# opteroncx/MoePhoto

Measured on AMD Instinct MI355X. Metric: megapixels/sec (input), 1080p 4x SR (Net4x a4), 256-px tiles with overlap, higher is better.
Workload: dtype fp16; 1 GPU; BASELINE configs[1]: 1 frame(s) 1920x1080 RGB -> 7680x4320, model a4 (Net4x, synthetic weights in zoo format), crop 256 pad 5 align 8 -> 40 tiles/frame, fp16 I/O, fp16 MFMA operands + fp32 accumulate; tiles_per_frame=40, parallelism=single GPU, precision=mixed, exact_blocks=1, input=natural-image-like synthetic frame (tests/golden_defs.natural_image)

## Files before the change

moephoto_amd/csrc/common.h:

```cpp
#pragma once
#include <hip/hip_runtime.h>
#include <stdint.h>

typedef _Float16 half_t;
typedef __attribute__((ext_vector_type(2))) _Float16 half2_t;
typedef __attribute__((ext_vector_type(4))) _Float16 half4_t;
typedef __attribute__((ext_vector_type(8))) _Float16 half8_t;
typedef __attribute__((ext_vector_type(4))) float float4_t;
typedef __attribute__((ext_vector_type(16))) float float16_t;

constexpr int kCB = 64;
constexpr int kTileW = 32;
constexpr int kTileH = 8;
constexpr int kFragBytes = 1024;

struct ConvArgs {
    const half_t* in;
    half_t* out;
    const half_t* res;
    const half_t* wpk;
    const float* bias;
    const float* bias_img;
    const half_t* zero;
    half_t* trash;
    half_t* out_lo;
    const half_t* in_lo;
    int plane_w;
    const half_t* side16;
    const float* tail1_w;
    float* tail1_out;
    const half_t* res_lo;
    float* acc32;
    int acc_mode;
    long long w_batch_stride;
    int B, H, W;
    int in_cs, out_cs;
    int r;
    int nchunks;
    int G;
    int px, py;
    float slope;
    float scale;
    const half_t* tail_w;
    float* tplanes;
    int tail_form;
    int tail_split;
    int dbg;
    float* pool; int pool_slabs;
};

struct ConvForm {
    int B = 0, H = 0, W = 0, in_cs = 64, out_cs = 64, r = 1, nchunks = 1, G = 1, py = 1;
    float slope = 1.f, scale = 1.f;
    int acc_mode = 0, dbg = 0, tail_form = 0, tail_split = 0, pool_slabs = 0;
    bool res = false, res_lo = false, in_lo = false, out_lo = false, side16 = false, tail = false, tail1 = false, pool = false, plane_w = false;
};
inline ConvForm conv_form(const ConvArgs& a)
{
    ConvForm c;
    c.B = a.B; c.H = a.H; c.W = a.W; c.in_cs = a.in_cs; c.out_cs = a.out_cs; c.r = a.r; c.nchunks = a.nchunks; c.G = a.G; c.py = a.py;
    c.slope = a.slope; c.scale = a.scale; c.acc_mode = a.acc_mode; c.dbg = a.dbg; c.tail_form = a.tail_form; c.tail_split = a.tail_split; c.pool_slabs = a.pool_slabs;
    c.res = a.res != nullptr; c.res_lo = a.res_lo != nullptr; c.in_lo = a.in_lo != nullptr; c.out_lo = a.out_lo != nullptr; c.side16 = a.side16 != nullptr;
    c.tail = a.tplanes != nullptr; c.tail1 = a.tail1_w != nullptr; c.pool = a.pool != nullptr; c.plane_w = a.plane_w != 0;
    return c;
}

struct TailSumLayout { unsigned S, RA, CA, CO, total; int py, px; };
__host__ __device__ inline TailSumLayout tailsum_layout(int B, int H, int W)
{
    TailSumLayout l;
    l.py = (H + kTileH - 1) / kTileH; l.px = (W + kTileW - 1) / kTileW;
    auto up = [](unsigned long long n) { return (unsigned)((n + 63) / 64 * 64); };
    l.S = 0;
    l.RA = l.S + up(16ull * B * H * W);
    l.CA = l.RA + up(8ull * B * l.py * W);
    l.CO = l.CA + up(8ull * B * H * l.px);
    l.total = l.CO + up(4ull * B * l.py * l.px);
    return l;
}
inline bool tailsum_fits(int B, int H, int W)
{
    const unsigned long long el = 16ull * B * H * W + 8ull * B * ((H + kTileH - 1) / kTileH) * W + 8ull * B * H * ((W + kTileW - 1) / kTileW) + 4ull * B * ((H + kTileH - 1) / kTileH) * ((W + kTileW - 1) / kTileW) + 4 * 64;
    return el * 4 < (1ull << 32) - (1ull << 17);
}

struct Conv1x1Args {
    const half_t* in_hi; const half_t* in_lo;
    half_t* out_hi; half_t* out_lo;
    const half_t* w_hi; const half_t* w_lo;
    const float* bias;
    const float* tail_w; float* tail_out;
    float slope;
    int B, H, W, r, nchunks, out_cs;
    int nks;
};
struct Conv1x1Form { int B, H, W, r, nchunks, out_cs; float slope; bool x3, tail, out_lo; };
bool conv1x1_applicable(const Conv1x1Form& a, int max_groups);
bool launch_conv1x1(const Conv1x1Args& a, int max_groups, hipStream_t s);
hipError_t conv1x1_init();

struct Conv1x1F2Args {
    const half_t* in_hi; const half_t* in_lo;
    const half_t* wa_hi; const half_t* wa_lo;
    const half_t* wb_hi; const half_t* wb_lo;
    const float* bias_a; const float* bias_b;
    const float* tail_w; float* tail_out;
    float slope_a, slope_b;
    int B, H, W;
};
bool conv1x1_f2_applicable(int B, int H, int W, float slope_a, float slope_b, int max_groups);
bool launch_conv1x1_f2(const Conv1x1F2Args& a, int max_groups, hipStream_t s);
hipError_t conv1x1_f2_init();

void launch_conv_mfma(const ConvArgs& a, int taps, int nseg, hipStream_t s);
int conv_mfma_max_groups();
hipError_t conv_mfma_init();
bool conv3x3_sp_applicable(const ConvForm& c);
bool launch_conv3x3_sp(const ConvArgs& a, hipStream_t s);
hipError_t conv3x3_sp_init();
bool conv3x3_rw_applicable(const ConvForm& c);
bool launch_conv3x3_rw(const ConvArgs& a, hipStream_t s);
hipError_t conv3x3_rw_init();

struct Ps4Args {
    const half_t* in;
    const half_t* wpk;
    const float* bias;
    const half_t* tail_w;
    half_t* out;
    float* plane;
    float* apron;
    float slope;
    int B, H, W;
    int split;
};
bool launch_conv3x3_ps4(const Ps4Args& a, int max_groups, hipStream_t s);
bool ps4_applicable(int B, int H, int W);
inline bool ps4_tail_applicable(int B, int H, int W, float slope) { return slope < 1.f && ps4_applicable(B, H, W); }
bool ps4_store_applicable(int B, int H, int W, float slope);
size_t ps4_plane_bytes(int B, int H, int W);
size_t ps4_apron_bytes(int B, int H, int W);
hipError_t conv3x3_ps4_init();
struct TailAddArgs {
    const float* p0; const float* p1;
    const float* a0; const float* a1;
    void* y; int y_dtype; const long long* y_off;
    int B, H, W, px;
    int vec_ok;
};
void launch_tailadd(const TailAddArgs& a, hipStream_t s);

struct Ps9Args {
    const half_t* in;
    const half_t* wpk;
    const float* bias;
    const half_t* tail_w;
    float* plane;
    float* apron;
    float slope;
    int B, H, W;
    int split;
    int xcd_map;
};
bool launch_conv3x3_ps9(const Ps9Args& a, int max_groups, hipStream_t s);
bool ps9_applicable(int B, int H, int W);
inline bool ps9_tail_applicable(int B, int H, int W, float slope) { return slope < 1.f && ps9_applicable(B, H, W); }
size_t ps9_plane_bytes(int B, int H, int W);
size_t ps9_apron_bytes(int B, int H, int W);
hipError_t conv3x3_ps9_init();
struct TailAdd3Args {
    const float* p0; const float* p1;
    const float* a0; const float* a1;
    void* y; int y_dtype; const long long* y_off;
    int B, H, W, px;
    int vec_ok;
};
void launch_tailadd3(const TailAdd3Args& a, hipStream_t s);

struct ArsbArgs {
    const half_t* x_hi; const half_t* x_lo;
    half_t* y_hi; half_t* y_lo;
    const half_t* w1; const half_t* w2;
    const half_t* zero;
    float slope;
    int B, H, W;
    int px, py;
    int cin;
    int drop_lo;
    unsigned long long* trace;
};
bool arsb32c_applicable(int B, int H, int W, float slope, bool x_lo, bool y_lo, int cin);
bool launch_arsb32c(ArsbArgs a, int max_groups, hipStream_t s);
hipError_t arsb32c_init();

struct ConvX3Args {
    const half_t* in_hi; const half_t* in_lo;
    half_t* out_hi; half_t* out_lo;
    const half_t* res_hi; const half_t* res_lo;
    const half_t* w_hi; const half_t* w_lo;
    const half_t* zero;
    float slope;
    int B, H, W;
    int px, py;
    float* pool; int pool_slabs;
    const float* gate;
    const half_t* wq_hi16; const unsigned char* wq_hi8; const unsigned char* wq_lo8;
    int in8, out8;
};
struct ConvX3Form {
    int B = 0, H = 0, W = 0, pool_slabs = 0;
    float slope = 1.f;
    bool res = false, res_lo = false, pool = false, gate = false, in8 = false, out8 = false;
};
inline ConvX3Form conv_x3_form(const ConvX3Args& a)
{
    ConvX3Form c;
    c.B = a.B; c.H = a.H; c.W = a.W; c.pool_slabs = a.pool_slabs; c.slope = a.slope;
    c.res = a.res_hi != nullptr; c.res_lo = a.res_lo != nullptr; c.pool = a.pool != nullptr; c.gate = a.gate != nullptr; c.in8 = a.in8 != 0; c.out8 = a.out8 != 0;
    return c;
}
bool conv64_x3_applicable(const ConvX3Form& c, int max_groups);
bool launch_conv64_x3(ConvX3Args a, int max_groups, hipStream_t s);
hipError_t conv64_x3_init();
bool conv64_q8_applicable(const ConvX3Form& c);
bool launch_conv64_q8(ConvX3Args a, int max_groups, hipStream_t s);
hipError_t conv64_q8_init();
bool conv64_sq_applicable(const ConvX3Form& c, int max_groups);
bool launch_conv64_sq(ConvX3Args a, int max_groups, hipStream_t s);
hipError_t conv64_sq_init();
bool conv64_s_applicable(const ConvForm& c);
bool launch_conv64_s(const ConvArgs& a, int max_groups, hipStream_t s);
hipError_t conv64_s_init();
struct ArsbSqArgs {
    const half_t* x_hi; const unsigned char* x_lo8;
    half_t* y_hi; void* y_lo;
    const half_t* w16[2]; const unsigned char* wh8[2]; const unsigned char* wl8[2];
    float slope;
    int B, H, W, out8;
};
bool arsb_sq_applicable(int B, int H, int W, float slope);
bool launch_arsb_sq(const ArsbSqArgs& a, int max_groups, hipStream_t s);
hipError_t arsb_sq_init();

inline int pooled_groups(long long P, long long items, int max_groups)
{
    long long G = 1;
    if (P <= max_groups) G = P * (max_groups / P);
    else for (long long d = max_groups; d >= 1; --d) if (P % d == 0) { G = d; break; }
    return (int)(G < items ? G : items);
}
inline bool pooled_groups_ok(long long P, long long items, int max_groups)
{
    const long long full = items < max_groups ? items : max_groups;
    return 2ll * pooled_groups(P, items, max_groups) >= full;
}

struct DirectConvArgs {
    const half_t* in; half_t* out; const half_t* res;
    const float* w;
    const float* bias;
    long long w_batch_stride;
    int B, H, W, in_cs, out_cs, cin, cout, k, r;
    float slope, scale;
};
void launch_conv_direct(const DirectConvArgs& a, hipStream_t s);

struct StemArgs {
    const void* x; int x_dtype;
    const long long* x_off;
    long long sB, sH, sW;
    const float* w;
    float slope;
    half_t* out;
    half_t* out_lo;
    int B, H, W, taps;
    int out_lo8;
    const float* w2; half_t* out2; half_t* out2_lo;
};
void launch_stem(const StemArgs& a, hipStream_t s);

struct TailArgs {
    const half_t* in0; const half_t* in1;
    const half_t* w0; const half_t* w1;
    const half_t* in0_lo; const half_t* in1_lo;
    const half_t* w0_lo; const half_t* w1_lo;
    int in1_lo8;
    const void* skip; int skip_dtype;
    const long long* skip_off; long long skip_sB, skip_sH, skip_sW;
    void* y; int y_dtype;
    const long long* y_off;
    int B, H, W, taps;
};
void launch_tail(const TailArgs& a, hipStream_t s);

struct TapSumArgs {
    const float* t0; const float* t1;
    void* y; int y_dtype; const long long* y_off;
    int B, H, W;
    int r;
    int form;
    int vec_ok;
};
void launch_tapsum(const TapSumArgs& a, hipStream_t s);

struct Tail1SumArgs {
    const float* p0; const float* p1;
    int nparts;
    void* y; int y_dtype; const long long* y_off;
    int B, H, W;
    const float* lut; int r; const void* x; const long long* x_off; long long sB, sH, sW;
    int vec_ok;
};
void launch_tail1sum(const Tail1SumArgs& a, hipStream_t s);

void launch_pool_partial(const half_t* in, const half_t* in_lo, float* partial, int B, long long HW, int C, int nslab, hipStream_t s);

struct SednSeArgs {
    const float* partial; int nslab; long long HW;
    const float* w_down;
    const float* w_up;
    const float* trans_pk32;
    half_t* trans_out;
    half_t* trans_out_lo;
    int B, nfrag;
};
void launch_sedn_se(const SednSeArgs& a, hipStream_t s);

struct SednFuseArgs {
    const half_t* x;
    float* partial;
    const float* pooled; int pooled_slabs;
    int pooled_count;
    int nslab, B, H, W;
    const float* w256t;
    const float* w256;
    const float* wt;
    const float* w_down;
    const float* w_up;
    float* gate;
    half_t* weff;
};
void launch_sedn_fuse(const SednFuseArgs& a, hipStream_t s);

struct FrmArgs {
    const float* partial; int nslab; long long HW;
    const float* w0; const float* b0;
    const float* w2; const float* b2;
    const half_t* t; const half_t* x; half_t* out;
    const half_t* t_lo; const half_t* x_lo; half_t* out_lo;
    float* gate;
    int B;
};
void launch_frm(const FrmArgs& a, hipStream_t s);
struct FrmPreArgs {
    const half_t* m; const half_t* m_lo;
    const float* partial; int nslab;
    const float* c2t;
    const float* w0; const float* b0;
    const float* w2; const float* b2;
    float* gate;
    int B, H, W;
};
void launch_frm_pre(const FrmPreArgs& a, hipStream_t s);

struct StitchArgs {
    const float* tiles; const long long* tile_off;
    const int* row_first; const int* row_cnt;
    const int* col_first; const int* col_cnt;
    const int* row_tab; const int* col_tab;
    const float* ramp;
    void* out; int out_dtype;
    int C, out_h, out_w, step_w;
    int row_lo;
    int y0, rows;
};
void launch_stitch(const StitchArgs& a, hipStream_t s);
struct QuantDither { float S, top; int ordered; };
bool launch_stitch_out(const StitchArgs& a, int canvas_dtype, float quant, hipStream_t s, const QuantDither* dq = nullptr);
void launch_stitch_planes(const StitchArgs& a, int canvas_dtype, int depth, hipStream_t s, const QuantDither* dq = nullptr);
struct StitchMix {
    const void* inp; long long sC, sH, sW;
    const void* alpha; long long aH, aW;
    float sf, tf; int blend;
    float quant;
    int inp_vec, alpha_vec;
    long long once_from; int q_once;
};
bool launch_stitch_mix(const StitchArgs& a, StitchMix m, int canvas_dtype, hipStream_t s, const QuantDither* dq = nullptr);
struct YuvEdge {
    int ky[3], ku[3], kv[3];
    unsigned mul_y, base_y; int mul_c, base_c;
    int depth, f16;
};
void launch_stitch_yuv(const StitchArgs& a, const YuvEdge& y, hipStream_t s, int dither = 0);
void launch_to_output_yuv(const void* src, int src_dtype, int H, int W, const YuvEdge& y, void* dst, hipStream_t s, int dither = 0);
struct LumaCoef { float kr, kg, kb, ib, ir, eb, er, gr, gb; };
struct StitchLuma { const float* c; LumaCoef k; int rp; float quant; };
bool launch_stitch_luma(const StitchArgs& a, const StitchLuma& m, int canvas_dtype, hipStream_t s, const QuantDither* dq = nullptr);
void launch_luma_split(const void* img, int dtype, int C, long long sC, long long sH, long long sW, int H, int W, const LumaCoef& k, int rp, void* dst_y, float* dst_c, hipStream_t s);
void launch_luma_merge(const void* y, int dtype, const float* c, int C, int H, int W, const LumaCoef& k, int rp, float quant, void* dst, int dst_dtype, hipStream_t s,
                       const QuantDither* dq = nullptr);

struct BlendTileArgs {
    const void* r; void* canvas; const void* ramp;
    long long r_sC, r_sH, c_sC, c_sH;
    int C, rh, rw;
    int top_sc, left_sc;
    int r0, c0;
    int lt_h, lt_w;
};
void launch_blend_tile(const BlendTileArgs& a, bool f16, hipStream_t s);

struct SymArgs {
    const void* src; void* dst;
    long long sC, sH, sW;
    int C, Hd, Wd;
    int nR, nC, flipR, flipC;
    int src_vec;
    int div; float inv;
};
void launch_sym(SymArgs a, bool f16, bool fold, bool tr, hipStream_t s);

struct WireRec {
    long long tile_off, wire_off;
    int C, th, tw;
    int ra0, ra1, rb0, rb1;
    int ca0, ca1, cb0, cb1;
    int pad_;
};
long long wire_rec_words(const WireRec& r);
void launch_wire(bool pack, float* tiles, unsigned* wire, const WireRec* recs, int n, long long max_elems, hipStream_t s);

void launch_to_float(const void* src, int src_dtype, float inv_or_div, bool divide, int H, int W, int C, void* dst, int dst_dtype, hipStream_t s);
void launch_to_output(const void* src, int src_dtype, int H, int W, int C, float quant, void* dst, int dst_dtype, hipStream_t s, const QuantDither* dq = nullptr);
void launch_to_float_planes(const void* src, int depth, int H, int W, void* dst_y, void* dst_c, int dst_dtype, hipStream_t s);
struct ChromaTab { short coef[16][4]; signed char off[16]; };
void launch_chroma_resample(const void* src, int src_depth, int h, int w, void* dst, int dst_depth, int scale, int taps, const ChromaTab& tx, const ChromaTab& ty, hipStream_t s);
void launch_chroma_guided(const void* src_c, const void* src_y, int src_depth, int h, int w, void* dst_c, const void* dst_y, int dst_depth, int scale, int left,
                          const unsigned char* cx, const signed char* ox, const unsigned char* cy, const signed char* oy, const unsigned char* range64, hipStream_t s);
constexpr int RGB_FRAC = 20;
struct PlanesRgb { int coef[5]; int yoff, coff, cmax, top, rgb, ordered; };
void launch_planes_rgb(const void* src, int depth, int H, int W, void* dst, int bits, int taps, const ChromaTab& tx, const ChromaTab& ty, const PlanesRgb& k, hipStream_t s);
constexpr int LUT3D_MIN = 2, LUT3D_MAX = 65;
struct Lut3dArgs { const float4* table; const float* vert; int d; float strength, rest; int blend, rgb; };
void launch_lut3d(const void* src, int src_bits, int H, int W, void* dst, int bits, const Lut3dArgs& k, float quant, const QuantDither* dq, hipStream_t s);
constexpr int FIT_TW = 128, FIT_TAPS = 16;
constexpr size_t FIT_LDS_BUDGET = 80 * 1024;
struct FitAxis { const int* off; const short* coef; int taps; };
void launch_fit(const void* src, int src_depth, int h, int w, void* dst, int dst_depth, int oh, int ow, int planes, int th, size_t lds, const FitAxis& ax, const FitAxis& ay, hipStream_t s);
void launch_fit_px(const void* src, int src_depth, int h, int w, void* dst, int dst_depth, int oh, int ow, int channels, int th, size_t lds, const FitAxis& ax, const FitAxis& ay, hipStream_t s);
void launch_resize(const void* src, void* dst, int dtype, int C, int H, int W, int h, int w, int mode, hipStream_t s);
void launch_maxabsdiff(const float* a, const float* b, long long n, unsigned* out, hipStream_t s);
void launch_changed_blocks(const void* cur, void* prev, int n, int rows, long long row_bytes, int block_rows, int block_bytes, unsigned char* map, hipStream_t s);
// ... 3 lines not shown
```

moephoto_amd/csrc/conv3x3_ps4.hip:

```cpp
#include "common.h"
#include "mfma_stream.h"
#include "rowtile.h"
#include "../../include/moephoto_amd.h"
#include <algorithm>

#ifndef PS4_FILL
#define PS4_FILL 5
#endif
#ifndef PS4_ZSKIP
#define PS4_ZSKIP 1
#endif
#ifndef PS4_ABL
#define PS4_ABL 0
#endif

namespace {

constexpr int RB = 4;
constexpr int PW = kTileW + 2;
constexpr int ROWB = PW * 128;
constexpr int BLKB = RB * ROWB;
constexpr int NPIECE = BLKB / 1024;
constexpr int TREC = 36 * 128 + 64;
constexpr int TEXP = 36 * 128;
constexpr int TROWS = 16;
constexpr int OFF_T = 2 * BLKB;
constexpr int OFF_BIAS = OFF_T + TROWS * TREC;
constexpr int OFF_TW = OFF_BIAS + 1024;
constexpr int OFF_DUMP = OFF_TW + 8 * 1024;
constexpr int LDS_BYTES = OFF_DUMP + 1024;

enum OpKind : int { OP_NONE = 0, OP_P, OP_WL, OP_TM, OP_TW, OP_BI, OP_DMA, OP_FA, OP_FR, OP_FS, OP_AR, OP_AS, OP_ST };
constexpr OpList row_ops(int epi)
{
    OpList r;
    if (epi == 0) {
        for (int s = 0; s < 4; ++s) {
            r.push(OP_P, s >> 1, 4 * (s & 1), 2); r.push(OP_P, s >> 1, 4 * (s & 1) + 2, 2);
            r.push(OP_ST, s >> 1, s & 1);
        }
        return r;
    }
    const bool split = epi == 2;
    int nl = 0;
    auto wl = [&](int frag) { r.push(OP_WL, frag, nl & 1); ++nl; };
    int nt = 0;
    wl(0);
    wl(split ? 4 : 1);
    for (int s = 0; s < 4; ++s) {
        if (split) for (int k = 0; k < 4; ++k) r.push(OP_P, s >> 1, 4 * (s & 1) + k, 1);
        else for (int k = 0; k < 4; k += 2) r.push(OP_P, s >> 1, 4 * (s & 1) + k, 2);
        r.push(OP_TM, nt & 1, 0, nt == 0); ++nt;
        if (split) {
            if (s < 3) wl(s + 1);
            r.push(OP_TM, nt & 1, 1, 0); ++nt;
            if (s < 3) wl(4 + s + 1);
        } else if (s + 2 < 4) wl(s + 2);
    }
    for (int k = 0; k < 5; ++k) r.push(OP_TW, k);
    return r;
}
constexpr OpList extra_ops(int e, bool tail)
{
    OpList r;
    if (!tail) {
        if (e == 0) for (int m = 0; m < 3; ++m) { r.push(OP_DMA, m, 0); r.push(OP_DMA, m, 1); }
        if (e == 1) for (int m = 3; m < 5; ++m) { r.push(OP_DMA, m, 0); r.push(OP_DMA, m, 1); }
        return r;
    }
    if (e == 0) {
        r.push(OP_FA);
        for (int dy = 0; dy < 3; ++dy) { r.push(OP_FR, dy, 0); r.push(OP_FR, dy, 1); r.push(OP_FR, dy, 2); }
        r.push(OP_FS);
        r.push(OP_AR); r.push(OP_AS);
        r.push(OP_DMA, 0, 0); r.push(OP_DMA, 0, 1);
    }
    if (e == 1) for (int m = 1; m < 5; ++m) { r.push(OP_DMA, m, 0); r.push(OP_DMA, m, 1); }
    return r;
}

template <int EPI, bool MASK>
__global__ __launch_bounds__(256) void conv3x3_ps4_kernel(Ps4Args a)
{
#if defined(__HIP_DEVICE_COMPILE__)
    constexpr bool TAIL = EPI >= 1, SPLIT = EPI == 2;
    constexpr bool PERM = !TAIL;
    extern __shared__ __attribute__((aligned(1024))) char smem[];
    const unsigned lds0 = (unsigned)(unsigned long long)(__attribute__((address_space(3))) char*)smem;
    const int tid = threadIdx.x, lane = tid & 63;
    const int w4 = __builtin_amdgcn_readfirstlane(tid >> 6);
    const int pi = w4 >> 1, pj = w4 & 1;
    const int j = lane & 31, hh = lane >> 5;
    const int H = a.H, W = a.W;

    const int px = (W + kTileW - 1) / kTileW, nyb = H / RB;
    const int g = blockIdx.x, G = gridDim.x;
    const long long nitems = (long long)a.B * px * nyb;
    int item = (int)(nitems * g / G);
    const int item_end = (int)(nitems * (g + 1) / G);
    if (item >= item_end) return;

    half8_t wf[2][36];
    {
        const half_t* wsrc = a.wpk + (long long)w4 * (72 * 512);
        int src = lane;
        if (PERM) {
            src = weight_row(j, hh);
        }
#pragma unroll
        for (int f = 0; f < 36; ++f) {
            wf[0][f] = *(const half8_t*)(wsrc + ((f * 2 + 0) * 64 + src) * 8);
            wf[1][f] = *(const half8_t*)(wsrc + ((f * 2 + 1) * 64 + src) * 8);
        }
#pragma unroll
        for (int f = 0; f < 36; ++f) asm volatile("" : "+a"(wf[0][f]));
#pragma unroll
        for (int f = 0; f < 28; ++f) asm volatile("" : "+a"(wf[1][f]));
#pragma unroll
        for (int f = 28; f < 36; ++f) asm volatile("" : "+v"(wf[1][f]));
    }
    {
        const int bw = tid >> 6, bcg = (tid >> 5) & 1, bhh = (tid >> 4) & 1, bq = (tid >> 2) & 3, be = tid & 3;
        *(float*)(smem + OFF_BIAS + tid * 4) = a.bias[64 * bw + 32 * bcg + (PERM ? 16 * (bq >> 1) + 8 * bhh + 4 * (bq & 1) + be : 8 * bq + 4 * bhh + be)];
        if (TAIL) {
            const u4_t* tsrc = (const u4_t*)a.tail_w;
            *(u4_t*)(smem + OFF_TW + tid * 16) = tsrc[tid];
            *(u4_t*)(smem + OFF_TW + 4096 + tid * 16) = SPLIT ? tsrc[256 + tid] : u4_t{0u, 0u, 0u, 0u};
            const u4_t z = {0u, 0u, 0u, 0u};
            for (int o = tid * 16; o < TROWS * TREC; o += 256 * 16) *(u4_t*)(smem + OFF_T + o) = z;
        }
    }
    const unsigned bias_ad = lds0 + (unsigned)(OFF_BIAS + ((w4 * 2 + 0) * 2 + hh) * 64);
    const unsigned tw_ad = lds0 + (unsigned)(OFF_TW + lane * 16);

    const unsigned in_pad = (unsigned)(RB * W + 1) * 128u;
    const __amdgpu_buffer_rsrc_t rin = __builtin_amdgcn_make_buffer_rsrc((void*)((const char*)a.in - in_pad), 0, (unsigned)a.B * H * W * 128u + in_pad, 0x00020000);
    const __amdgpu_buffer_rsrc_t rpl = TAIL ? __builtin_amdgcn_make_buffer_rsrc((void*)a.plane, 0, (unsigned)a.B * H * W * 16u, 0x00020000)
                                            : __builtin_amdgcn_make_buffer_rsrc((void*)a.out, 0, (unsigned)a.B * H * W * 512u, 0x00020000);
    const __amdgpu_buffer_rsrc_t rap = __builtin_amdgcn_make_buffer_rsrc((void*)(TAIL ? (void*)a.apron : (void*)a.out), 0, TAIL ? (unsigned)a.B * px * H * 16u : 0u, 0x00020000);
    unsigned d_off = 0, d_r = 0, d_cc = 0;
    auto piece_addr = [&](int m) {
        unsigned q = (unsigned)((m < 4 ? w4 + 4 * m : 16) * 8 + (lane >> 3));
        asm volatile("" : "+v"(q));
        d_r = __umul24(q, 241u) >> 13;
        d_cc = (unsigned)(__mul24((int)d_r, -PW) + (int)q);
        const unsigned sl = (unsigned)(lane & 7) ^ ((d_cc >> 1) & 7u);
        d_off = ((__umul24(d_r, (unsigned)W) + d_cc) << 7) | (sl << 4);
    };
    auto piece_off = [&](int ya, int xa, bool live) {
        const bool ok = ((unsigned)(ya + (int)d_r) < (unsigned)H) & ((unsigned)(xa + (int)d_cc) < (unsigned)W) & live;
        return ok ? d_off : kOOR;
    };

    unsigned fa[3];
#pragma unroll
    for (int dx = 0; dx < 3; ++dx) {
        fa[dx] = frag_addr(lds0, j + dx, hh);
        asm volatile("" : "+v"(fa[dx]));
    }
    unsigned wa[5];
#pragma unroll
    for (int k = 0; k < 5; ++k) {
        const int t = k < 4 ? 4 * hh + k : 8;
        const int dy = t / 3, dx = t - 3 * dy;
        int col = j;
        if (pj == 1 && dx == 0) col = j + 1;
        if (pj == 0 && dx == 2) col = j - 1;
        unsigned o = (unsigned)((w4 * 9 + t) * 128 + col * 4);
        if (col == kTileW) o = (unsigned)(TEXP + ((0 * 2 + pi) * 3 + dy) * 4);
        if (col < 0) o = (unsigned)(TEXP + ((1 * 2 + pi) * 3 + dy) * 4);
        if (k == 4 && hh == 1) o = (unsigned)(TEXP + 48 + w4 * 4);
        wa[k] = lds0 + (unsigned)OFF_T + o;
        asm volatile("" : "+v"(wa[k]));
    }
    const int f_i = (lane >> 4) & 1, f_xp = lane & 15;
    const int a_side = (lane >> 1) & 1, a_i = lane & 1;
    unsigned slope2;
    {
        const half2_t s2 = {(half_t)a.slope, (half_t)a.slope};
        slope2 = __builtin_bit_cast(unsigned, s2);
    }

    float16_t acc[4][2];
    half8_t fr[3];
    half8_t twr[2];
    unsigned hX[4], lX[4];
    float16_t Gt = zero16;

    asm volatile("s_waitcnt lgkmcnt(0)" ::: "memory");
    __builtin_amdgcn_s_barrier();

    while (item < item_end) {
        const int s0 = item % nyb;
        const int t_ = item / nyb;
        const int pxi = t_ % px, b = t_ / px;
        const int s1 = min(nyb, s0 + (item_end - item));
        item += s1 - s0;
        const int x0 = pxi * kTileW;
        const int nblk = s1 - s0 + 3;
        const int kfirst = (PS4_ZSKIP && s0 == 0) ? 1 : 0;
        const int kz = (PS4_ZSKIP && s1 == nyb) ? nblk - 2 : nblk - 1;
        const bool okx = x0 + j < W;
        const int ylo = RB * s0, yhi = RB * s1;

        asm volatile("s_waitcnt lgkmcnt(0)" ::: "memory");
        __builtin_amdgcn_s_barrier();
        asm volatile("" ::: "memory");
        {
            const int ya = RB * (s0 - 1 + kfirst), xa = x0 - 1;
            const unsigned org = (unsigned)((b * H + ya + RB) * W + xa + 1) * 128u;
#pragma unroll
            for (int m = 0; m < 5; ++m) {
                piece_addr(m);
                const bool mine = m < 4 || w4 == 0;
                char* dst = smem + (m < 4 ? (w4 + 4 * m) * 1024 : (mine ? 16 * 1024 : OFF_DUMP));
                __builtin_amdgcn_raw_ptr_buffer_load_lds(rin, (__attribute__((address_space(3))) void*)dst, 16, piece_off(ya, xa, mine), org, 0, 0);
#if PS4_ABL & 128
                if (m < 4) __builtin_amdgcn_raw_ptr_buffer_load_lds(rin, (__attribute__((address_space(3))) void*)(dst + BLKB), 16, piece_off(ya + 4 * RB, xa, mine), org + (unsigned)(4 * RB * W) * 128u, 0, 0);
#endif
            }
#pragma unroll
            for (int s = 0; s < 4; ++s)
#pragma unroll
                for (int cg = 0; cg < 2; ++cg) acc[s][cg] = *(const __attribute__((address_space(3))) float16_t*)(bias_ad + cg * 128);
            asm volatile("s_waitcnt vmcnt(0) lgkmcnt(0)" ::: "memory");
            __builtin_amdgcn_s_barrier();
            asm volatile("" ::: "memory");
            fr[0] = *(lds_h8_t)(fa[0]);
            fr[1] = *(lds_h8_t)(fa[0] ^ 32u);
        }

        auto block = [&](int k, auto BUF_, auto KIND_) __attribute__((always_inline)) {
            constexpr int BUF = decltype(BUF_)::value;
            constexpr bool LAST = decltype(KIND_)::value == 2;
            constexpr bool ZERO = decltype(KIND_)::value == 1;
            const int Rk = RB * (s0 - 1 + k);
            const bool live = k + 1 < kz;
            const int yan = Rk + RB, xan = x0 - 1;
            const unsigned orgn = (unsigned)__builtin_amdgcn_readfirstlane((int)((unsigned)((b * H + yan + RB) * W + xan + 1) * 128u));
            const int yf = Rk - 7 + w4;
            const bool f_ok = (yf >= ylo) & (yf < yhi);
            unsigned fb[3];
            f2_t fs[2] = {{0.f, 0.f}, {0.f, 0.f}};
            f2_t fv[2];
            float av[3];

            auto step = [&](auto E_) __attribute__((always_inline)) {
                constexpr int e = decltype(E_)::value;
                const int orow = Rk + e - 2;
                const unsigned trow = (unsigned)__builtin_amdgcn_readfirstlane((int)((unsigned)((orow + 64) & 15) * (unsigned)TREC));
                const bool rowok = (unsigned)orow < (unsigned)H;
                constexpr int SL = (e + 2) & 3;

                auto op_p = [&](auto CG_, auto K0_, auto N_) __attribute__((always_inline)) {
                    constexpr int cg = decltype(CG_)::value, k0 = decltype(K0_)::value, n = decltype(N_)::value;
#pragma unroll
                    for (int k = k0; k < k0 + n; ++k) {
                        const float s0v = acc[SL][cg][2 * k], s1v = acc[SL][cg][2 * k + 1];
                        unsigned hv, lv = 0;
                        if (SPLIT) {
                            const float t0 = __builtin_fmaxf(s0v, s0v * a.slope), t1 = __builtin_fmaxf(s1v, s1v * a.slope);
                            split2(t0, t1, -2048.f, hv, lv);
                        } else {
                            const half2_t pr = {(half_t)s0v, (half_t)s1v};
                            const half2_t t = pr * __builtin_bit_cast(half2_t, slope2);
                            hv = __builtin_bit_cast(unsigned, __builtin_elementwise_max(pr, t));
                        }
                        hX[k & 3] = hv; lX[k & 3] = lv;
                    }
                };
                auto op_st = [&](auto CG_, auto G_) __attribute__((always_inline)) {
                    constexpr int cg = decltype(CG_)::value, gq = decltype(G_)::value;
                    const bool rok = (orow >= ylo) & (orow < yhi);
                    const unsigned vo = okx ? (unsigned)(2 * j) * 128u + (unsigned)hh * 16u : kOOR;
                    const unsigned so = rok ? ((unsigned)((b * 2 * H + 2 * orow + pi) * 2 * W + 2 * x0 + pj) * 128u + (unsigned)(64 * cg + 32 * gq)) : kOOR;
                    const u4_t d = {hX[0], hX[1], hX[2], hX[3]};
                    __builtin_amdgcn_raw_buffer_store_b128(d, rpl, vo, so, 0);
                };
                auto op_wl = [&](auto F_, auto S_) __attribute__((always_inline)) {
                    constexpr int fg = decltype(F_)::value, st = decltype(S_)::value;
                    twr[st] = *(lds_h8_t)(tw_ad + (unsigned)(fg * 1024));
                };
                auto op_tm = [&](auto S_, auto LO_, auto FIRST_) __attribute__((always_inline)) {
                    constexpr int st = decltype(S_)::value, lo = decltype(LO_)::value, first = decltype(FIRST_)::value;
                    const half8_t bv = lo ? __builtin_bit_cast(half8_t, u4_t{lX[0], lX[1], lX[2], lX[3]}) : __builtin_bit_cast(half8_t, u4_t{hX[0], hX[1], hX[2], hX[3]});
                    Gt = __builtin_amdgcn_mfma_f32_32x32x16_f16(twr[st], bv, first ? zero16 : Gt, 0, 0, 0);
                };
                auto op_tw = [&](auto K_) __attribute__((always_inline)) {
                    constexpr int k = decltype(K_)::value;
                    float t = __builtin_fmaf(Gt[8 + k], 0.00048828125f, Gt[k]);
                    const bool ok = MASK ? (rowok & okx) : rowok;
                    t = ok ? t : 0.f;
                    const unsigned ad = wa[k] + trow;
                    asm volatile("ds_write_b32 %0, %1" ::"v"(ad), "v"(t) : "memory");
                };
                auto op_bi = [&](auto CG_) __attribute__((always_inline)) {
                    constexpr int cg = decltype(CG_)::value;
#pragma unroll
                    for (int q = 0; q < 4; ++q) {
                        const float4_t t = *(const __attribute__((address_space(3))) float4_t*)(bias_ad + (unsigned)(cg * 128 + q * 16));
                        acc[SL][cg][4 * q] = t[0]; acc[SL][cg][4 * q + 1] = t[1]; acc[SL][cg][4 * q + 2] = t[2]; acc[SL][cg][4 * q + 3] = t[3];
                    }
                };
                auto op_dma = [&](auto M_, auto HALF_) __attribute__((always_inline)) {
                    constexpr int m = decltype(M_)::value, half = decltype(HALF_)::value;
                    if constexpr (half == 0) piece_addr(m);
                    else {
                        const bool mine = m < 4 || w4 == 0;
                        const unsigned dsto = (unsigned)__builtin_amdgcn_readfirstlane((int)(m < 4 ? (BUF ^ 1) * BLKB + (w4 + 4 * m) * 1024 : (mine ? (BUF ^ 1) * BLKB + 16 * 1024 : OFF_DUMP)));
                        __builtin_amdgcn_raw_ptr_buffer_load_lds(rin, (__attribute__((address_space(3))) void*)(smem + dsto), 16, piece_off(yan, xan, live & mine), orgn, 0, 0);
                    }
                };
                auto op_fa = [&]() __attribute__((always_inline)) {
#pragma unroll
                    for (int dy = 0; dy < 3; ++dy) {
                        const int isrc = f_i == 0 ? (dy == 1 ? 0 : 1) : (dy == 1 ? 1 : 0);
                        const int dd = f_i == 0 ? (dy == 0 ? -1 : 0) : (dy == 2 ? 1 : 0);
                        fb[dy] = lds0 + (unsigned)OFF_T + (unsigned)((yf + dd + 64) & 15) * (unsigned)TREC + (unsigned)((2 * isrc * 9 + dy * 3) * 128 + f_xp * 8);
                    }
                };
                auto op_fr = [&](auto DY_, auto DX_) __attribute__((always_inline)) {
                    constexpr int dy = decltype(DY_)::value, dx = decltype(DX_)::value;
                    constexpr int j0 = dx == 1 ? 0 : 1, j1 = dx == 1 ? 1 : 0;
                    if constexpr (dx > 0 || dy > 0) { fs[0] = fs[0] + fv[0]; fs[1] = fs[1] + fv[1]; }
                    fv[0] = *(const __attribute__((address_space(3))) f2_t*)(fb[dy] + (unsigned)((j0 * 9 + dx) * 128));
                    fv[1] = *(const __attribute__((address_space(3))) f2_t*)(fb[dy] + (unsigned)((j1 * 9 + dx) * 128));
                };
                auto op_fs = [&]() __attribute__((always_inline)) {
                    fs[0] = fs[0] + fv[0]; fs[1] = fs[1] + fv[1];
                    const float4_t o4 = {fs[0][0], fs[1][0], fs[0][1], fs[1][1]};
                    const bool ok = f_ok & (lane < 32) & (x0 + 2 * f_xp < W);
                    const unsigned vo = ok ? (unsigned)(f_i * 2 * W + 4 * f_xp) * 4u : kOOR;
                    const unsigned so = (unsigned)(((b * 2 * H + 2 * yf) * 2 * W) + 2 * x0) * 4u;
                    __builtin_amdgcn_raw_buffer_store_b128(__builtin_bit_cast(u4_t, o4), rpl, vo, f_ok ? so : 0u, 0);
                };
                auto op_ar = [&]() __attribute__((always_inline)) {
#pragma unroll
                    for (int dy = 0; dy < 3; ++dy) {
                        const int isrc = a_i == 0 ? (dy == 1 ? 0 : 1) : (dy == 1 ? 1 : 0);
                        const int dd = a_i == 0 ? (dy == 0 ? -1 : 0) : (dy == 2 ? 1 : 0);
                        const unsigned ad = lds0 + (unsigned)OFF_T + (unsigned)((yf + dd + 64) & 15) * (unsigned)TREC + (unsigned)(TEXP + ((a_side * 2 + isrc) * 3 + dy) * 4);
                        av[dy] = *(const __attribute__((address_space(3))) float*)ad;
                    }
                };
                auto op_as = [&]() __attribute__((always_inline)) {
                    const float v = (av[0] + av[1]) + av[2];
                    const bool ok = f_ok & (lane >= 32) & (lane < 36);
                    const unsigned vo = ok ? (unsigned)(((a_side * a.B) * px) * 2 * H + a_i) * 4u : kOOR;
                    const unsigned so = (unsigned)((b * px + pxi) * 2 * H + 2 * yf) * 4u;
                    __builtin_amdgcn_raw_buffer_store_b32(__builtin_bit_cast(unsigned, v), rap, vo, f_ok ? so : 0u, 0);
                };

                if constexpr (LAST) {
                    if constexpr (e == 0 && !(PS4_ABL & 2)) {
                        op_fa();
                        op_fr(std::integral_constant<int, 0>{}, std::integral_constant<int, 0>{}); op_fr(std::integral_constant<int, 0>{}, std::integral_constant<int, 1>{}); op_fr(std::integral_constant<int, 0>{}, std::integral_constant<int, 2>{});
                        op_fr(std::integral_constant<int, 1>{}, std::integral_constant<int, 0>{}); op_fr(std::integral_constant<int, 1>{}, std::integral_constant<int, 1>{}); op_fr(std::integral_constant<int, 1>{}, std::integral_constant<int, 2>{});
                        op_fr(std::integral_constant<int, 2>{}, std::integral_constant<int, 0>{}); op_fr(std::integral_constant<int, 2>{}, std::integral_constant<int, 1>{}); op_fr(std::integral_constant<int, 2>{}, std::integral_constant<int, 2>{});
                        op_fs();
                        op_ar(); op_as();
                    }
                    return;
                }
                auto chunk = [&](auto F_) __attribute__((always_inline)) {
                    constexpr int f = decltype(F_)::value;
                    constexpr int dx = f >> 2, ks = f & 3;
                    if (e == 3 && f == 10 && !(PS4_ABL & 16)) {
                        asm volatile("s_waitcnt vmcnt(0) lgkmcnt(0)" ::: "memory");
                        __builtin_amdgcn_s_barrier();
                        asm volatile("" ::: "memory");
                    }
                    constexpr OpList LM = row_ops(EPI);
                    constexpr OpList LX = extra_ops(e, TAIL);
                    auto half = [&](auto HC_) __attribute__((always_inline)) {
                        constexpr int hc = decltype(HC_)::value;
                        if constexpr (!ZERO) {
#pragma unroll
                            for (int u = 3 * hc; u < 3 * hc + 3; ++u) {
                                const int dy = u >> 1, cg = u & 1;
                                const int sl = (e + 1 - dy + 4) & 3;
                                acc[sl][cg] = __builtin_amdgcn_mfma_f32_32x32x16_f16(wf[cg][(dy * 3 + dx) * 4 + ks], fr[f % 3], acc[sl][cg], 0, 0, 0);
                            }
                        }
                        if constexpr (hc == 0 && !ZERO) {
                            constexpr int f2 = (f + 2) % 12;
                            constexpr int rowsel = f + 2 < 12 ? BUF * RB + e : (e < 3 ? BUF * RB + e + 1 : (BUF ^ 1) * RB);
                            if (!(PS4_ABL & 8)) fr[(f + 2) % 3] = *(lds_h8_t)((fa[f2 >> 2] ^ (unsigned)((f2 & 3) * 32)) + (unsigned)(rowsel * ROWB));
                        }
                        constexpr int h = 2 * f + hc;
                        constexpr int MH = TAIL ? 20 : 10;
                        constexpr int m_lo = h < MH ? h * LM.n / MH : LM.n, m_hi = h < MH ? (h + 1) * LM.n / MH : LM.n;
                        constexpr int x_lo = TAIL ? h * LX.n / 24 : (h < 12 ? 0 : (h - 12) * LX.n / 12), x_hi = TAIL ? (h + 1) * LX.n / 24 : (h < 12 ? 0 : (h - 11) * LX.n / 12);
                        auto runm = [&](auto I_) __attribute__((always_inline)) {
                            constexpr int I = decltype(I_)::value;
                            if constexpr (I >= m_lo && I < m_hi && !(PS4_ABL & 1)) {
                                constexpr Op o = LM.op[I];
                                if constexpr (o.kind == OP_P) op_p(std::integral_constant<int, o.a>{}, std::integral_constant<int, o.b>{}, std::integral_constant<int, o.c>{});
                                if constexpr (o.kind == OP_WL) op_wl(std::integral_constant<int, o.a>{}, std::integral_constant<int, o.b>{});
                                if constexpr (o.kind == OP_TM && !(PS4_ABL & 32)) op_tm(std::integral_constant<int, o.a>{}, std::integral_constant<int, o.b>{}, std::integral_constant<int, o.c>{});
                                if constexpr (o.kind == OP_TW) op_tw(std::integral_constant<int, o.a>{});
                                if constexpr (o.kind == OP_ST) op_st(std::integral_constant<int, o.a>{}, std::integral_constant<int, o.b>{});
                            }
                        };
                        auto runx = [&](auto I_) __attribute__((always_inline)) {
                            constexpr int I = decltype(I_)::value;
                            if constexpr (I >= x_lo && I < x_hi) {
                                constexpr Op o = LX.op[I];
                                if constexpr (o.kind != OP_DMA && (PS4_ABL & 2)) return;
                                if constexpr (o.kind == OP_DMA && (PS4_ABL & 64)) return;
                                if constexpr (o.kind == OP_DMA) op_dma(std::integral_constant<int, o.a>{}, std::integral_constant<int, o.b>{});
                                if constexpr (o.kind == OP_FA) op_fa();
                                if constexpr (o.kind == OP_FR) op_fr(std::integral_constant<int, o.a>{}, std::integral_constant<int, o.b>{});
                                if constexpr (o.kind == OP_FS) op_fs();
                                if constexpr (o.kind == OP_AR) op_ar();
                                if constexpr (o.kind == OP_AS) op_as();
                            }
                        };
                        static_for<LM.n>(runm);
                        static_for<LX.n>(runx);
                        if (f == 10 && hc == 1 && !(PS4_ABL & 4)) op_bi(std::integral_constant<int, 0>{});
                        if (f == 11 && hc == 1 && !(PS4_ABL & 4)) op_bi(std::integral_constant<int, 1>{});
                    };
                    half(std::integral_constant<int, 0>{});
                    half(std::integral_constant<int, 1>{});
#ifndef PS4_NOPIN
                    static_for<ZERO ? 0 : 2>([&](auto HC_) __attribute__((always_inline)) {
                        constexpr int hc = decltype(HC_)::value, h = 2 * f + hc, MH = TAIL ? 20 : 10;
                        constexpr int m_lo = h < MH ? h * LM.n / MH : LM.n, m_hi = h < MH ? (h + 1) * LM.n / MH : LM.n;
                        pin_mfmas<3, hc == 0 ? 1 : 0, PS4_FILL>();
                        pin_mfmas<(!TAIL || (PS4_ABL & 33)) ? 0 : count_kind(LM, m_lo, m_hi, OP_TM), 0, PS4_FILL>();
                    });
#endif
                    __builtin_amdgcn_sched_barrier(0);
                };
#if PS4_ABL
                if constexpr (!LAST) asm volatile("" ::"v"(acc[SL][0]), "v"(acc[SL][1]), "v"(Gt));
#endif
                static_for<12>(chunk);
            };
            step(std::integral_constant<int, 0>{});
            step(std::integral_constant<int, 1>{});
            step(std::integral_constant<int, 2>{});
            step(std::integral_constant<int, 3>{});
        };

        typedef std::integral_constant<int, 0> Run;
        typedef std::integral_constant<int, 1> Zero;
        typedef std::integral_constant<int, 2> Last;
        int k = kfirst;
        for (; k + 1 < kz; k += 2) {
            block(k, std::integral_constant<int, 0>{}, Run{});
            block(k + 1, std::integral_constant<int, 1>{}, Run{});
        }
        if (k < kz) { block(k, std::integral_constant<int, 0>{}, Run{}); ++k; }
        if (k < nblk - 1) { block(k, std::integral_constant<int, 0>{}, Zero{}); ++k; }
        if (TAIL) block(k, std::integral_constant<int, 0>{}, Last{});
    }
#endif
}

template <bool VEC>
__global__ __launch_bounds__(256) void tailadd_kernel(TailAddArgs a)
{
    const int nq = a.W >> 3;
    const long long idx = (long long)blockIdx.x * 256 + threadIdx.x;
    if (idx >= (long long)a.B * a.H * nq) return;
    const int xq = (int)(idx % nq);
    const int Y = (int)((idx / nq) % a.H), b = (int)(idx / ((long long)nq * a.H));
    const int X0 = xq * 8;
    const long long po = ((long long)b * a.H + Y) * a.W + X0;
    float v[8];
    {
        const float4 r0 = *(const float4*)(a.p0 + po), r1 = *(const float4*)(a.p0 + po + 4);
        v[0] = r0.x; v[1] = r0.y; v[2] = r0.z; v[3] = r0.w; v[4] = r1.x; v[5] = r1.y; v[6] = r1.z; v[7] = r1.w;
        if (a.p1) {
            const float4 u0 = *(const float4*)(a.p1 + po), u1 = *(const float4*)(a.p1 + po + 4);
            v[0] += u0.x; v[1] += u0.y; v[2] += u0.z; v[3] += u0.w; v[4] += u1.x; v[5] += u1.y; v[6] += u1.z; v[7] += u1.w;
        }
    }
    const int c = X0 >> 6, in = X0 & 63;
    const long long as = (long long)a.B * a.px * a.H;
    if (in == 0 && c >= 1) {
        const long long o = ((long long)b * a.px + (c - 1)) * a.H + Y;
        float t = a.a0[o];
        if (a.a1) t += a.a1[o];
        v[0] += t;
    }
    if (in == 56 && c + 1 < a.px) {
        const long long o = as + ((long long)b * a.px + (c + 1)) * a.H + Y;
        float t = a.a0[o];
        if (a.a1) t += a.a1[o];
        v[7] += t;
    }
    const long long yo = (a.y_off ? a.y_off[b] : (long long)b * a.H * a.W) + (long long)Y * a.W + X0;
    if (a.y_dtype == MOE_F16) {
        if (VEC) {
            half8_t h;
#pragma unroll
            for (int k = 0; k < 8; ++k) h[k] = (half_t)v[k];
            *(half8_t*)((half_t*)a.y + yo) = h;
        } else {
#pragma unroll
            for (int k = 0; k < 8; ++k) ((half_t*)a.y)[yo + k] = (half_t)v[k];
        }
    } else {
        float* yp = (float*)a.y + yo;
        if (VEC) {
            *(float4*)yp = make_float4(v[0], v[1], v[2], v[3]);
            *(float4*)(yp + 4) = make_float4(v[4], v[5], v[6], v[7]);
        } else {
#pragma unroll
            for (int k = 0; k < 8; ++k) yp[k] = v[k];
        }
    }
}

template <int EPI, bool MASK>
hipError_t set_limit()
{
    return hipFuncSetAttribute((const void*)conv3x3_ps4_kernel<EPI, MASK>, hipFuncAttributeMaxDynamicSharedMemorySize, LDS_BYTES);
}

}

hipError_t conv3x3_ps4_init()
{
    hipError_t e;
    if ((e = set_limit<0, true>()) != hipSuccess) return e;
    if ((e = set_limit<1, false>()) != hipSuccess) return e;
    if ((e = set_limit<1, true>()) != hipSuccess) return e;
    if ((e = set_limit<2, false>()) != hipSuccess) return e;
    return set_limit<2, true>();
}

size_t ps4_plane_bytes(int B, int H, int W) { return (size_t)B * H * W * 16; }
size_t ps4_apron_bytes(int B, int H, int W) { return (size_t)2 * B * ((W + kTileW - 1) / kTileW) * 2 * H * 4; }

bool ps4_applicable(int B, int H, int W)
{
    if (H % RB != 0 || W % 4 != 0 || H < RB) return false;
    if ((long long)B * H * W * 128 + (long long)(RB * W + 1) * 128 >= (1ll << 32) - 65536) return false;
    return (long long)B * ((W + kTileW - 1) / kTileW) * (H / RB) < (1ll << 31) / 4;
}

bool ps4_store_applicable(int B, int H, int W, float slope)
{
    return ps4_tail_applicable(B, H, W, slope) && (long long)B * H * W * 512 < (1ll << 32) - 65536;
}

bool launch_conv3x3_ps4(const Ps4Args& a, int max_groups, hipStream_t s)
{
    if (!(a.out ? ps4_store_applicable(a.B, a.H, a.W, a.slope) : ps4_tail_applicable(a.B, a.H, a.W, a.slope))) return false;
    const int px = (a.W + kTileW - 1) / kTileW;
    const long long items = (long long)a.B * px * (a.H / RB);
    const int G = (int)std::min<long long>(items, max_groups);
    const bool ragged = a.W % kTileW != 0;
    if (a.out) {
        if (a.plane) return false;
        conv3x3_ps4_kernel<0, true><<<dim3(G), dim3(256), LDS_BYTES, s>>>(a);
        return true;
    }
    if (a.split) {
        if (ragged) conv3x3_ps4_kernel<2, true><<<dim3(G), dim3(256), LDS_BYTES, s>>>(a);
        else conv3x3_ps4_kernel<2, false><<<dim3(G), dim3(256), LDS_BYTES, s>>>(a);
    } else {
        if (ragged) conv3x3_ps4_kernel<1, true><<<dim3(G), dim3(256), LDS_BYTES, s>>>(a);
        else conv3x3_ps4_kernel<1, false><<<dim3(G), dim3(256), LDS_BYTES, s>>>(a);
    }
    return true;
}

void launch_tailadd(const TailAddArgs& a, hipStream_t s)
{
    const long long n = (long long)a.B * a.H * (a.W / 8);
    if (a.vec_ok) tailadd_kernel<true><<<dim3((unsigned)((n + 255) / 256)), dim3(256), 0, s>>>(a);
    else tailadd_kernel<false><<<dim3((unsigned)((n + 255) / 256)), dim3(256), 0, s>>>(a);
}
```

moephoto_amd/csrc/forward.cpp:

```cpp
#include "net.h"

using namespace moe;

namespace moe {

const char* kernel_name(ConvKernel k)
{
    static const char* const names[] = {"no kernel", "conv_direct", "conv1x1", "conv_mfma", "conv3x3_sp", "conv3x3_rw", "conv3x3_ps4 (store form)", "conv3x3_sp (hi + lo residual)",
                                        "conv_mfma (three products)", "conv64_x3", "conv64_q8", "conv64_sq", "conv3x3_sp (three launches)", "conv_mfma (fp32 side buffer)"};
    return names[(int)k];
}

static bool fast_layer(const moe_net& n, const ConvLayer& L) { return L.taps == 9 && L.nseg == 1 && !L.per_plane && n.opt.conv_impl == 2; }

ConvForm Fwd::form(const ConvLayer& L, int H, int W) const
{
    ConvForm c;
    c.B = B; c.H = H; c.W = W; c.in_cs = 64 * L.nseg; c.out_cs = L.r > 1 ? 64 : 64 * L.nchunks; c.r = L.r; c.nchunks = L.nchunks;
    c.py = (H + kTileH - 1) / kTileH;
    const long long items = (long long)B * ((W + kTileW - 1) / kTileW) * c.py;
    const int per_xcd = groups / 8;
    int G = per_xcd >= L.nchunks ? 8 * (per_xcd / L.nchunks) : groups / L.nchunks;
    if (G < 1) G = 1;
    if (G > items) G = (int)items;
// ... 82 lines not shown
        DirectConvArgs d{};
        d.in = in.hi; d.out = out.hi; d.res = res ? res->hi : nullptr;
        d.w = blob<float>(L.w_plain);
        d.bias = L.has_bias ? blob<float>(L.bias_plain) : nullptr;
        d.w_batch_stride = 0;
        d.B = B; d.H = H; d.W = W; d.in_cs = c.in_cs; d.out_cs = c.out_cs; d.cin = L.cin; d.cout = L.cout; d.k = L.k; d.r = L.r;
        d.slope = L.slope; d.scale = L.scale;
        if (L.per_plane) { d.w = (const float*)e.plane_w; d.w_batch_stride = (long long)L.cout * L.cin; }
        launch_conv_direct(d, s);
        return MOE_OK;
    }
    ConvArgs a{};
    a.in = in.hi; a.out = out.hi; a.res = res ? res->hi : nullptr;
    a.wpk = L.per_plane ? e.plane_w : blob<half_t>(L.w_hi);
    a.bias = L.has_bias ? blob<float>(L.bias) : small<float>("zero_bias");
    a.zero = small<half_t>("zero");
    a.bias_img = blob<float>(L.bias_img);
    a.trash = small<half_t>("trash");
    a.w_batch_stride = L.per_plane ? (long long)L.nchunks * L.nfrag() * 512 : 0;
    a.B = B; a.H = H; a.W = W; a.in_cs = c.in_cs; a.out_cs = c.out_cs; a.r = c.r; a.nchunks = c.nchunks;
    a.px = (W + kTileW - 1) / kTileW; a.py = c.py; a.G = c.G;
    a.slope = c.slope; a.scale = c.scale; a.dbg = c.dbg;
    a.tail_w = e.tail_w; a.tplanes = e.tplanes; a.tail_form = c.tail_form; a.tail_split = c.tail_split;
    a.tail1_w = e.tail1_w; a.tail1_out = e.tail1_out;
    if (c.pool) { a.pool = e.pool_out; a.pool_slabs = c.pool_slabs; }
    const bool x3 = this->x3 || e.exact;
    const bool timed = r.kernel != ConvKernel::mfma_x3 && r.kernel != ConvKernel::sp_three && r.kernel != ConvKernel::acc32;
    const int rec = timed ? prof_begin(key, (x3 ? 3 : 1) * 2.0 * (double)B * H * W * L.cout * L.cin * L.taps) : -1;
    bool ok = true;
    auto single = [&](const ConvArgs& ca) {
        if (r.kernel == ConvKernel::rw) return launch_conv3x3_rw(ca, s);
        if (r.kernel == ConvKernel::sp) return launch_conv3x3_sp(ca, s);
        if (r.kernel == ConvKernel::ps4_store) {
            Ps4Args q{};
            q.in = ca.in; q.wpk = ca.wpk; q.bias = ca.bias; q.out = ca.out; q.slope = ca.slope; q.B = ca.B; q.H = ca.H; q.W = ca.W;
            return launch_conv3x3_ps4(q, groups, s);
        }
        launch_conv_mfma(ca, L.taps, L.nseg, s);
        return true;
    };
    switch (r.kernel) {
    case ConvKernel::conv1x1: {
        Conv1x1Args q{};
        q.in_hi = in.hi; q.in_lo = x3 ? in.lo : nullptr; q.out_hi = out.hi; q.out_lo = x3 ? out.lo : nullptr;
        q.w_hi = blob<half_t>(L.w_hi); q.w_lo = x3 ? blob<half_t>(L.w_lo) : nullptr; q.bias = a.bias;
        q.tail_w = e.tail1_w; q.tail_out = e.tail1_out; q.slope = L.slope;
        q.B = B; q.H = H; q.W = W; q.r = L.r; q.nchunks = L.nchunks; q.out_cs = c.out_cs;
        q.nks = (L.cin <= 48 && n.opt.k48) ? 3 : 4;
        ok = launch_conv1x1(q, groups, s);
        break;
    }
    case ConvKernel::mfma: case ConvKernel::sp: case ConvKernel::rw: case ConvKernel::ps4_store: {
        unsigned long long* tr = nullptr;
        const size_t nb = 8 * 32 * 4 * 16 * 8;
        if (!x3 && (c.dbg & 64) && fast_layer(n, L) && key == n.opt.trace_key && hipMalloc((void**)&tr, nb) == hipSuccess) {
            (void)hipMemsetAsync(tr, 0, nb, s);
            ConvArgs t = a; t.acc32 = (float*)tr;
            ok = single(t);
            std::vector<unsigned long long> host(nb / 8);
            (void)hipStreamSynchronize(s);
            (void)hipMemcpy(host.data(), tr, nb, hipMemcpyDeviceToHost);
            if (FILE* f = fopen("/tmp/moe_trace.bin", "wb")) { fwrite(host.data(), 1, nb, f); fclose(f); }
            (void)hipFree(tr);
        } else
            ok = single(a);
        break;
    }
    case ConvKernel::sp_res_lo: {
        ConvArgs q = a; q.acc_mode = 3; q.side16 = res->lo; q.out_lo = out.lo; q.res_lo = nullptr;
        ok = launch_conv3x3_sp(q, s);
        break;
    }
    case ConvKernel::mfma_x3: {
        ConvArgs f4 = a; f4.wpk = blob<half_t>(L.w_x3); f4.acc_mode = 4; f4.in_lo = in.lo; f4.out_lo = out.lo; f4.res_lo = res ? res->lo : nullptr;
        launch_conv_mfma(f4, 1, 3, s);
        break;
    }
    case ConvKernel::x3: case ConvKernel::q8: case ConvKernel::sq: {
        ConvX3Args q{};
        q.in_hi = in.hi; q.in_lo = in.lo; q.out_hi = out.hi; q.out_lo = out.lo;
        q.res_hi = res ? res->hi : nullptr; q.res_lo = res ? res->lo : nullptr;
        q.w_hi = blob<half_t>(L.w_arsb); q.w_lo = blob<half_t>(L.w_arsb_lo); q.zero = small<half_t>("zero");
        q.slope = L.slope; q.B = B; q.H = H; q.W = W;
        if (r.x3.pool) { q.pool = e.pool_out; q.pool_slabs = e.pool_slabs; }
        if (r.x3.gate) q.gate = e.gate_in;
        if (r.kernel == ConvKernel::x3) { ok = launch_conv64_x3(q, groups, s); break; }
        q.wq_hi16 = blob<half_t>(L.w_hi); q.wq_hi8 = blob<unsigned char>(L.wq_hi8); q.wq_lo8 = blob<unsigned char>(L.wq_lo8);
        q.in8 = r.x3.in8; q.out8 = r.x3.out8;
        ok = r.kernel == ConvKernel::sq ? launch_conv64_sq(q, groups, s) : launch_conv64_q8(q, groups, s);
        break;
    }
    case ConvKernel::sp_three: {
        ConvArgs q1 = a; q1.wpk = blob<half_t>(L.w_lo); q1.out = side16; q1.res = (res && res->has_lo) ? res->lo : nullptr; q1.bias = small<float>("zero_bias");
        q1.bias_img = small<float>("zero_bias_img"); q1.slope = 1.f; q1.scale = 1.f; q1.acc_mode = 0; q1.tail_w = nullptr; q1.tplanes = nullptr;
        ConvArgs q2 = q1; q2.in = in.lo; q2.wpk = blob<half_t>(L.w_hi); q2.res = side16;
        ConvArgs q3 = a; q3.acc_mode = 3; q3.side16 = side16; q3.out_lo = out.lo; q3.res_lo = nullptr;
        ok = launch_conv3x3_sp(q1, s) && launch_conv3x3_sp(q2, s) && launch_conv3x3_sp(q3, s);
        break;
    }
    case ConvKernel::acc32: {
        a.acc32 = acc32;
        ConvArgs p1 = a; p1.wpk = L.per_plane ? e.plane_w_lo : blob<half_t>(L.w_lo); p1.acc_mode = 1; p1.res = nullptr; p1.bias = nullptr;
        launch_conv_mfma(p1, L.taps, L.nseg, s);
        ConvArgs p2 = a; p2.in = in.lo; p2.acc_mode = 2; p2.res = nullptr; p2.bias = nullptr;
        launch_conv_mfma(p2, L.taps, L.nseg, s);
        ConvArgs p3 = a; p3.acc_mode = 3; p3.out_lo = out.lo; p3.res_lo = res ? res->lo : nullptr;
        launch_conv_mfma(p3, L.taps, L.nseg, s);
        break;
    }
    default: ok = false;
    }
    prof_end(rec);
    if (!ok) return fail(MOE_EINVAL, "internal error: layer %s (%d planes of %dx%d) was routed to %s, and that launcher refused it", key.c_str(), B, H, W, kernel_name(r.kernel));
    return MOE_OK;
}

ConvDone Fwd::conv(const std::string& key, const Act& in, const Act& out, const Act* res, int H, int W, const ConvExtra& e)
{
    const ConvRoute r = route(key, in, out, res, H, W, e);
    if (r.done.ok && !dry()) {
        rc = launch(r, key, in, out, res, e);
        if (rc) ar.base = nullptr;
    }
    return r.done;
}

void Fwd::stem(const Act& out, const Act* out2)
{
    if (dry()) return;
    StemArgs a{};
    if (out2) { a.w2 = small<float>("stem.p2"); a.out2 = out2->hi; a.out2_lo = out2->lo; }
    a.x = io.x; a.x_dtype = io.x_dtype; a.x_off = io.x_off; a.sB = io.sB; a.sH = io.sH; a.sW = io.sW;
    a.w = small<float>("stem"); a.slope = n.scalars.at("stem_slope");
    a.out = out.hi; a.out_lo = out.lo; a.out_lo8 = out.lo8; a.B = B; a.H = h; a.W = w; a.taps = (int)n.scalars.at("stem_taps");
    launch_stem(a, s);
}

void Fwd::gate() { if (ctx.gate_event && !dry()) (void)hipStreamWaitEvent(s, ctx.gate_event, 0); }

void Fwd::tail(const Act* r, const Act* u, int H, int W, bool skip)
{
    gate();
    if (dry()) return;
    TailArgs a{};
    a.in0 = r->hi; a.w0 = small<half_t>("tail_r");
    if (u) { a.in1 = u->hi; a.w1 = small<half_t>("tail_u"); }
    if (r->has_lo && (!u || u->has_lo)) {
        a.in0_lo = r->lo; a.w0_lo = small<half_t>("tail_r.lo");
        if (u) { a.in1_lo = u->lo; a.w1_lo = small<half_t>("tail_u.lo"); a.in1_lo8 = u->lo8; }
    }
    if (skip) { a.skip = io.x; a.skip_dtype = io.x_dtype; a.skip_off = io.x_off; a.skip_sB = io.sB; a.skip_sH = io.sH; a.skip_sW = io.sW; }
    a.y = io.y; a.y_dtype = io.y_dtype; a.y_off = io.y_off; a.B = B; a.H = H; a.W = W; a.taps = (int)n.scalars.at("tail_taps");
    launch_tail(a, s);
}

static size_t acc32_need(const moe_net& n, int B, int h, int w)
{
    size_t best = 0;
    long long HW = (long long)h * w;
    if (n.arch == MOE_ARCH_SEDN) return (size_t)B * (size_t)HW * 256;
    int rr = 1;
    best = (size_t)B * (size_t)HW * 64;
    for (int s = 0; s < n.stages; ++s) {
        best = std::max<size_t>(best, (size_t)B * (size_t)HW * rr * rr * 64 * n.r * n.r);
        rr *= n.r;
    }
    return best;
}

int exact_blocks_of(const moe_net& n)
{
    if (n.exact_blocks >= 0) return n.exact_blocks > 6 ? 6 : n.exact_blocks;
    const int env = n.opt.exact_blocks_env;
    if (env >= 0) return env > 6 ? 6 : env;
    if (n.calib_valid && n.calib_blocks >= 0) return n.calib_blocks;
    return default_exact_blocks(n.arch);
}

int default_exact_blocks(int arch)
{
    switch (arch) {
        case MOE_ARCH_NET2X: return 4;
        case MOE_ARCH_NET3X: return 2;
        case MOE_ARCH_NET4X: return 1;
        case MOE_ARCH_NETDN: return 1;
        default: return 0;
    }
}

long long sp_bytes_per_pixel(const moe_net& n)
{
    long long per = 128;
    if (n.arch == MOE_ARCH_SEDN) per = 512;
    if (n.arch == MOE_ARCH_LITE) {
        for (int st = 0; st + 1 < n.stages; ++st) per *= 4;
    }
    if (n.arch == MOE_ARCH_NET2X || n.arch == MOE_ARCH_NET3X || n.arch == MOE_ARCH_NET4X) {
        long long rr = 1;
        for (int st = 0; st < n.stages; ++st) {
            rr *= (long long)n.r * n.r;
            per = std::max(per, st == n.stages - 1 ? 36 * rr : 128 * rr);
        }
    }
    return per;
}

static int run_forward(const moe_net& n, Fwd& f, const FwdIO& io)
{
    const int B = f.B, h = f.h, w = f.w;
    const long long P = (long long)B * h * w;
    f.io = io;
    if (f.x3) {
        f.acc32_elems = acc32_need(n, B, h, w);
        f.acc32 = (float*)f.ar.take(f.acc32_elems * 4);
        f.side16 = (half_t*)f.ar.take(f.acc32_elems * 2 + 4096);
    } else if (f.mixed) {
        f.side16 = (half_t*)f.ar.take((size_t)P * 64 * 2 + 4096);
        bool steep = false;
        for (int i = 1; i <= exact_blocks_of(n); ++i) steep = steep || n.convs[n.conv_index.at("c1_" + std::to_string(i))].slope > 1.f;
        if (steep) { f.acc32_elems = (size_t)P * 64; f.acc32 = (float*)f.ar.take(f.acc32_elems * 4); }
    }
    int rc = MOE_OK;
    switch (n.arch) {
        case MOE_ARCH_SEDN: rc = forward_sedn(n, f); break;
        case MOE_ARCH_LITE: rc = forward_lite(n, f); break;
        default: rc = forward_arsb(n, f);
    }
    return rc ? rc : f.rc;
}

static Fwd make_fwd(const moe_net& n, const FwdCtx& ctx, NetRuntime* rt, hipStream_t s, int B, int h, int w, Arena ar)
{
    Fwd f{n, ctx, rt, s, B, h, w, ar, ctx.groups, n.precision == MOE_PREC_FP16X3, n.precision == MOE_PREC_DEBUG_DIRECT};
    f.mixed = n.precision == MOE_PREC_MIXED;
    return f;
}

static size_t workspace_need(const moe_net& n, const FwdCtx& ctx, int B, int h, int w)
{
    Fwd f = make_fwd(n, ctx, nullptr, nullptr, B, h, w, Arena{});
    run_forward(n, f, FwdIO{});
    return f.ar.off + 4096;
}

static bool plan_matches(const Fwd& f, size_t planned)
{
    if (f.ar.overflow) return false;
    return f.skips_planned_work ? f.ar.off <= planned : f.ar.off == planned;
}

static int forward_dev_chunk(moe_net& n, const FwdIO& io, int B, int h, int w, hipStream_t s, bool y_off_mult8, const FwdCtx& ctx);

static void build_lite_lut_on_device(moe_net& n, hipStream_t s, const FwdCtx& ctx)
{
    const int r = n.scale;
    std::vector<unsigned short> pat(65536);
    for (int i = 0; i < 65536; ++i) pat[(size_t)i] = (unsigned short)i;
    half_t* in = nullptr;
    float* scratch = nullptr;
    int rc = MOE_ENOMEM;
    if (hipMalloc((void**)&in, 65536 * 2) == hipSuccess && hipMalloc((void**)&n.lut, (size_t)65536 * r * r * 4) == hipSuccess && hipMalloc((void**)&scratch, (size_t)65536 * r * r * 4) == hipSuccess &&
        hipMemcpyAsync(in, pat.data(), 65536 * 2, hipMemcpyHostToDevice, s) == hipSuccess && hipStreamSynchronize(s) == hipSuccess) {
        FwdCtx capture = ctx;
        capture.lut_capture = n.lut;
        rc = forward_dev_chunk(n, FwdIO{in, MOE_F16, 65536, 256, 1, nullptr, scratch, MOE_F32, nullptr}, 1, 256, 256, s, true, capture);
        (void)hipStreamSynchronize(s);
    }
    if (in) (void)hipFree(in);
    if (scratch) (void)hipFree(scratch);
    if (rc != MOE_OK) { (void)hipGetLastError(); drop_lut(n); }
    n.lut_state = rc == MOE_OK ? 1 : -1;
}

static void build_lite_lut(moe_net& n, hipStream_t s, const FwdCtx& ctx)
{
    n.lut_state = -1;
    if (n.arch != MOE_ARCH_LITE || !n.opt.lite_lut || n.debug || !n.opt.fuse_tail || n.precision == MOE_PREC_DEBUG_DIRECT) return;
    hipStreamCaptureStatus cs = hipStreamCaptureStatusNone;
    if (hipStreamIsCapturing(s, &cs) != hipSuccess || cs != hipStreamCaptureStatusNone) { (void)hipGetLastError(); n.lut_state = 0; return; }
    int cur = -1;
    if (hipGetDevice(&cur) != hipSuccess || (cur != n.device && hipSetDevice(n.device) != hipSuccess)) { (void)hipGetLastError(); n.lut_state = 0; return; }
    build_lite_lut_on_device(n, s, ctx);
    if (cur != n.device) (void)hipSetDevice(cur);
}

int forward_dev(moe_net& n, const FwdIO& io, int B, int h, int w, hipStream_t s, bool y_off_mult8, const FwdCtx& ctx)
{
    if (!n.finalized) return fail(MOE_ESTATE, "moe_net_forward: net is not finalized (load_state_dict + to(device) first)");
    if (B < 1 || h < 1 || w < 1) return fail(MOE_EINVAL, "moe_net_forward: bad shape B=%d h=%d w=%d", B, h, w);
    if ((io.x_dtype != MOE_F32 && io.x_dtype != MOE_F16) || (io.y_dtype != MOE_F32 && io.y_dtype != MOE_F16))
        return fail(MOE_EINVAL, "moe_net_forward: x/y dtype must be MOE_F32 or MOE_F16");
    const long long bmax = kSpRange / (sp_bytes_per_pixel(n) * (long long)h * w);
    if (bmax < 1)
        return fail(MOE_ENOMEM, "a %dx%d tile exceeds the convolution kernels' addressing range (%lld pixels per plane at most for this net): use a smaller cropsize",
                    h, w, kSpRange / sp_bytes_per_pixel(n));
    if (n.arch == MOE_ARCH_LITE && io.x_dtype == MOE_F16 && n.lut_state == 0 && n.opt.lite_lut) build_lite_lut(n, s, ctx);
    if (B <= bmax) return forward_dev_chunk(n, io, B, h, w, s, y_off_mult8, ctx);
    const size_t xe = io.x_dtype == MOE_F32 ? 4 : 2, ye = io.y_dtype == MOE_F32 ? 4 : 2;
    const long long yplane = (long long)h * n.scale * w * n.scale;
    for (int b0 = 0; b0 < B; b0 += (int)bmax) {
        const int cnt = (int)std::min<long long>(bmax, B - b0);
        FwdIO c = io;
        if (io.x_off) c.x_off += b0; else c.x = (const char*)io.x + (size_t)b0 * io.sB * xe;
        if (io.y_off) c.y_off += b0; else c.y = (char*)io.y + (size_t)b0 * yplane * ye;
        const bool al = y_off_mult8 && (io.y_off || ((size_t)b0 * yplane * ye) % 16 == 0);
        if (int rc = forward_dev_chunk(n, c, cnt, h, w, s, al, ctx)) return rc;
    }
    return MOE_OK;
}

static int forward_dev_chunk(moe_net& n, const FwdIO& io, int B, int h, int w, hipStream_t s, bool y_off_mult8, const FwdCtx& ctx)
{
    int cur = -1;
    HIP_TRY(hipGetDevice(&cur));
    if (cur != n.device) HIP_TRY(hipSetDevice(n.device));
    const size_t need = workspace_need(n, ctx, B, h, w);
    StreamSet& set = *ctx.set;
    if (int rc = set.ws.grow(need, s, "workspace of %zu bytes for %d planes of %dx%d does not fit", need, B, h, w)) return rc;
    const size_t planned = need - 4096;
    Fwd f = make_fwd(n, ctx, &n.rt, s, B, h, w, Arena{(char*)set.ws.p, 0, planned});
    f.y_vec = y_off_mult8 && ((uintptr_t)io.y % 16 == 0);
    int rc = run_forward(n, f, io);
    if (rc) return rc;
    if (!plan_matches(f, planned))
        return fail(MOE_EINVAL, "internal error: the launching pass took %zu bytes of workspace%s, the planning pass %zu (%d planes of %dx%d)", f.ar.off,
                    f.ar.overflow ? " (beyond the plan: the launches behind that point were not issued)" : "", planned, B, h, w);
    hipError_t e = hipGetLastError();
    if (e != hipSuccess) return fail(MOE_EHIP, "kernel launch failed: %s", hipGetErrorString(e));
    return MOE_OK;
}

void free_set(StreamSet& set)
{
    if (set.side) { (void)hipStreamSynchronize(set.side); (void)hipStreamDestroy(set.side); }
    for (hipEvent_t e : {set.ev_fork, set.ev_join}) if (e) (void)hipEventDestroy(e);
    set.ws.release();
    set = StreamSet{};
}

void free_records(NetRuntime& rt)
{
    for (auto& ev : rt.prof_ev) { (void)hipEventDestroy(ev.e0); (void)hipEventDestroy(ev.e1); }
    for (auto& sl : rt.off_ring) {
        if (sl.host) (void)hipHostFree(sl.host);
        if (sl.dev) (void)hipFree(sl.dev);
        if (sl.done) (void)hipEventDestroy(sl.done);
    }
    for (auto& t : rt.taps) if (t.second.dev) (void)hipFree(t.second.dev);
    rt = NetRuntime{};
}

void pipe_destroy(moe_net& n)
{
    for (auto& ps : n.pipe) {
        if (ps.main) { (void)hipStreamSynchronize(ps.main); (void)hipStreamDestroy(ps.main); }
        for (hipEvent_t e : {ps.entry, ps.done}) if (e) (void)hipEventDestroy(e);
        free_set(ps);
        ps = PipeSet{};
    }
    n.pipe_prev_valid = false;
    n.pipe_last_stream = nullptr;
}

static bool overlap_eligible(const moe_net& n, int B, int h, int w)
{
    const bool sr = n.arch == MOE_ARCH_NET2X || n.arch == MOE_ARCH_NET3X || n.arch == MOE_ARCH_NET4X;
    return sr && n.finalized && n.opt.overlap_calls && !n.debug && n.opt.conv_impl == 2 && (n.precision == MOE_PREC_MIXED || n.precision == MOE_PREC_FP16) &&
           (long long)B * h * w <= 4ll * 65536 && n.prof_keys.empty() && n.opt.repeat_key.empty();
}

static int forward_pipelined(moe_net* n, const void* x, int x_dtype, int B, int h, int w, int64_t sB, int64_t sH, int64_t sW, void* y, int y_dtype, hipStream_t s, unsigned flags)
{
    HIP_TRY(hipSetDevice(n->device));
    PipeSet& ps = n->pipe[n->pipe_next];
    PipeSet& prev = n->pipe[n->pipe_next ^ 1];
    if (!ps.main) {
        HIP_TRY(hipStreamCreateWithFlags(&ps.main, hipStreamNonBlocking));
        HIP_TRY(hipEventCreateWithFlags(&ps.entry, hipEventDisableTiming));
        HIP_TRY(hipEventCreateWithFlags(&ps.done, hipEventDisableTiming));
    }
    HIP_TRY(hipEventRecord(ps.entry, s));
    const bool since_prev = (flags & MOE_FWD_INPUT_SINCE_PREV) && n->pipe_prev_valid && n->pipe_last_stream == s && prev.entry;
    HIP_TRY(hipStreamWaitEvent(ps.main, since_prev ? prev.entry : ps.entry, 0));
    n->pipe_next ^= 1;
    const int groups = n->opt.overlap_groups > 0 ? std::max(16, std::min(n->opt.overlap_groups, n->max_groups)) : std::max(16, n->max_groups / 2);
    const FwdCtx ctx{&ps, groups, n->opt.overlap_fork && n->opt.branch_streams, since_prev ? ps.entry : nullptr, nullptr};
    const int rc = forward_dev(*n, FwdIO{x, x_dtype, sB, sH, sW, nullptr, y, y_dtype, nullptr}, B, h, w, ps.main, true, ctx);
    if (hipEventRecord(ps.done, ps.main) != hipSuccess || hipStreamWaitEvent(s, ps.done, 0) != hipSuccess) { (void)hipGetLastError(); (void)hipStreamSynchronize(ps.main); }
    n->pipe_prev_valid = rc == MOE_OK;
    n->pipe_last_stream = s;
    return rc;
}

}

extern "C" {

int moe_net_forward_ex(moe_net* n, const void* x, int x_dtype, int B, int h, int w, int64_t sB, int64_t sH, int64_t sW,
                       const int64_t* x_off, void* y, int y_dtype, const int64_t* y_off, void* stream, unsigned flags)
{
    if (!n || !x || !y) return fail(MOE_EINVAL, "moe_net_forward: NULL argument");
    if (flags & ~(unsigned)MOE_FWD_INPUT_SINCE_PREV) return fail(MOE_EINVAL, "moe_net_forward_ex: unknown flags 0x%x", flags);
    if ((flags & MOE_FWD_INPUT_SINCE_PREV) && !x_off && !y_off && B >= 1 && h >= 1 && w >= 1 && overlap_eligible(*n, B, h, w)) {
        hipStreamCaptureStatus cs = hipStreamCaptureStatusNone;
        if (hipStreamIsCapturing((hipStream_t)stream, &cs) == hipSuccess && cs == hipStreamCaptureStatusNone)
            return forward_pipelined(n, x, x_dtype, B, h, w, sB, sH, sW, y, y_dtype, (hipStream_t)stream, flags);
        (void)hipGetLastError();
    }
    n->pipe_prev_valid = false;
    return moe_net_forward(n, x, x_dtype, B, h, w, sB, sH, sW, x_off, y, y_dtype, y_off, stream);
}

int moe_net_forward(moe_net* n, const void* x, int x_dtype, int B, int h, int w, int64_t sB, int64_t sH, int64_t sW,
                    const int64_t* x_off, void* y, int y_dtype, const int64_t* y_off, void* stream)
{
    if (!n || !x || !y) return fail(MOE_EINVAL, "moe_net_forward: NULL argument");
    hipStream_t s = (hipStream_t)stream;
    long long* xo = nullptr;
    long long* yo = nullptr;
    NetRuntime::OffSlot* slot = nullptr;
    if (x_off || y_off) {
        HIP_TRY(hipSetDevice(n->device >= 0 ? n->device : 0));
        NetRuntime::OffSlot& sl = n->rt.off_ring[n->rt.off_next];
        n->rt.off_next = (n->rt.off_next + 1) % 4;
        if (sl.used) HIP_TRY(hipEventSynchronize(sl.done));
        const size_t need = (size_t)B * 2;
        if (need > sl.cap) {
            if (sl.host) { (void)hipHostFree(sl.host); sl.host = nullptr; }
            if (sl.dev) { (void)hipFree(sl.dev); sl.dev = nullptr; }
            sl.cap = 0;
            const size_t cap = std::max<size_t>(need, 256);
            HIP_TRY(hipHostMalloc((void**)&sl.host, cap * 8, hipHostMallocDefault));
            HIP_TRY(hipMalloc((void**)&sl.dev, cap * 8));
            sl.cap = cap;
        }
        if (!sl.done) HIP_TRY(hipEventCreateWithFlags(&sl.done, hipEventDisableTiming));
        for (int i = 0; i < B; ++i) { sl.host[i] = x_off ? x_off[i] : 0; sl.host[B + i] = y_off ? y_off[i] : 0; }
        HIP_TRY(hipMemcpyAsync(sl.dev, sl.host, need * 8, hipMemcpyHostToDevice, s));
        sl.used = true;
        slot = &sl;
        if (x_off) xo = sl.dev;
        if (y_off) yo = sl.dev + B;
    }
    bool mult8 = true;
    if (y_off) for (int i = 0; i < B; ++i) mult8 = mult8 && (y_off[i] % 8 == 0);
    const int rc = forward_dev(*n, FwdIO{x, x_dtype, sB, sH, sW, xo, y, y_dtype, yo}, B, h, w, s, mult8, own_ctx(*n, &n->set));
    if (slot && hipEventRecord(slot->done, s) != hipSuccess) { (void)hipGetLastError(); (void)hipStreamSynchronize(s); }
    return rc;
}

int64_t moe_net_workspace_bytes(const moe_net* n, int B, int h, int w)
{
    if (!n || B < 1 || h < 1 || w < 1) return fail(MOE_EINVAL, "moe_net_workspace_bytes: bad argument");
    if (!n->finalized) return fail(MOE_ESTATE, "moe_net_workspace_bytes: net is not finalized");
    return (int64_t)workspace_need(*n, own_ctx(*n, nullptr), B, h, w);
}

int moe_net_set_profile(moe_net* n, const char* layer_substrings)
{
    if (!n) return fail(MOE_EINVAL, "moe_net_set_profile: NULL net");
    n->prof_keys.clear();
    std::string all = layer_substrings ? layer_substrings : "";
    size_t pos = 0;
    while (pos <= all.size() && !all.empty()) {
        const size_t c = all.find(',', pos);
        const std::string k = all.substr(pos, c == std::string::npos ? std::string::npos : c - pos);
        if (!k.empty()) n->prof_keys.push_back(k);
        if (c == std::string::npos) break;
        pos = c + 1;
    }
    n->rt.prof_used = 0;
    return MOE_OK;
}

int moe_net_get_profile_at(moe_net* n, int index, double* total_ms, int64_t* launches, double* flops)
{
    if (!n || !total_ms || !launches || !flops) return fail(MOE_EINVAL, "moe_net_get_profile: NULL argument");
    double ms = 0, fl = 0;
    int64_t cnt = 0;
    for (size_t i = 0; i < n->rt.prof_used; ++i) {
        const NetRuntime::ProfRec& r = n->rt.prof_ev[i];
        if (r.key != index) continue;
        HIP_TRY(hipEventSynchronize(r.e1));
        float t = 0.f;
        HIP_TRY(hipEventElapsedTime(&t, r.e0, r.e1));
        ms += t; fl += r.flops; ++cnt;
    }
    *total_ms = ms; *launches = cnt; *flops = fl;
    return MOE_OK;
}

int moe_net_get_profile(moe_net* n, double* total_ms, int64_t* launches, double* flops)
{
    int rc = moe_net_get_profile_at(n, 0, total_ms, launches, flops);
    if (rc == MOE_OK) n->rt.prof_used = 0;
    return rc;
}

int64_t moe_net_max_tile_pixels(const moe_net* n)
{
    if (!n) return fail(MOE_EINVAL, "moe_net_max_tile_pixels: NULL net");
    return (int64_t)(kSpRange / sp_bytes_per_pixel(*n));
}

int moe_net_set_debug(moe_net* n, int enable)
{
    if (!n) return fail(MOE_EINVAL, "moe_net_set_debug: NULL net");
    if (enable == 2 && n->arch == MOE_ARCH_LITE)
        return fail(MOE_EINVAL, "moe_net_set_debug: value 2 (taps of the production forward) is defined for SEDN, Net2x / Net3x / Net4x and NetDN; 1 taps lite's unfused forward");
    n->debug = enable != 0 && enable != 2;
    n->tap_only = enable == 2;
    return MOE_OK;
}

int64_t moe_net_debug_tap(moe_net* n, const char* tap, float* host, int64_t capacity, int64_t shape[4], void* stream)
{
    if (!n || !tap) return fail(MOE_EINVAL, "moe_net_debug_tap: NULL argument");
    auto it = n->rt.taps.find(tap);
    if (it == n->rt.taps.end() || !it->second.dev) return fail(MOE_EINVAL, "no tap named \"%s\" (enable moe_net_set_debug before the forward)", tap);
    const auto& t = it->second;
    const int64_t nel = t.shape[0] * t.shape[1] * t.shape[2] * t.shape[3];
    if (shape) for (int d = 0; d < 4; ++d) shape[d] = t.shape[d];
    if (!host) return nel;
    if (capacity < nel) return fail(MOE_EINVAL, "moe_net_debug_tap: capacity %lld < %lld", (long long)capacity, (long long)nel);
    HIP_TRY(hipStreamSynchronize((hipStream_t)stream));
    HIP_TRY(hipMemcpy(host, t.dev, (size_t)nel * 4, hipMemcpyDeviceToHost));
    return nel;
}

}
```

moephoto_amd/csrc/forward_arsb.cpp:

```cpp
#include "net.h"

using namespace moe;

namespace {

const ConvLayer* last_up(const moe_net& n, int br)
{
    const auto it = n.conv_index.find(std::string(br == 0 ? "convt_R1" : "u") + ".up" + std::to_string(n.stages - 1));
    return it == n.conv_index.end() ? nullptr : &n.convs[it->second];
}

bool can_fuse_tail(const moe_net& n, const Fwd& f)
{
    const int B = f.B, h = f.h, w = f.w;
    if (!n.opt.fuse_tail || f.x3 || f.direct || n.debug || n.opt.conv_impl != 2 || n.stages < 1) return false;
    if (!(n.arch == MOE_ARCH_NET2X || n.arch == MOE_ARCH_NET3X || n.arch == MOE_ARCH_NET4X)) return false;
    if (sp_bytes_per_pixel(n) * B * h * w > kSpRange) return false;
    int hl = h, wl = w;
    for (int st = 0; st + 1 < n.stages; ++st) { hl *= n.r; wl *= n.r; }
    for (int br = 0; br < 2; ++br) {
        const ConvLayer* L = last_up(n, br);
        if (!L) return false;
        ConvForm c = f.form(*L, hl, wl);
        c.tail = true;
        if (!conv3x3_sp_applicable(c)) return false;
    }
    return true;
}

struct ArsbRun {
    const moe_net& n;
    Fwd& f;
    const int B, h, w;
    bool mixed = false;
    int nx = 0;
    Act A, Bb, Cc;
    bool chain8 = false;
    half_t* lo16x = nullptr;
    bool sr = false, fuse = false, ps4 = false, ps9 = false;
    int H = 0, W = 0;
    Act fin[2];
    float* tp[2] = {nullptr, nullptr};
    float* ps_plane[2] = {nullptr, nullptr};
    float* ps_apron[2] = {nullptr, nullptr};

    void plan_tail_form();
    template <typename Args, typename Launch>
    int ps_stage(int br, const std::string& key, const Act& cur, size_t plane_bytes, size_t apron_bytes, const char* name, Launch launch);
    int run_branch(int br, Act cur);
    int trunk_conv(const std::string& key, const Act& in, const Act& out, const Act* res, bool exact);
    int run_trunk();
    template <typename Args, typename Launch> void tail_add(Launch launch);
    int branch_sum();
    int run();
};

void ArsbRun::plan_tail_form()
{
    sr = n.arch != MOE_ARCH_NETDN;
    fuse = sr && can_fuse_tail(n, f);
    if (sr) {
        int hl = h, wl = w;
        for (int st = 0; st + 1 < n.stages; ++st) { hl *= n.r; wl *= n.r; }
        bool ok = fuse && n.opt.tail_form == 1;
        bool ps4_ok = true;
        bool ps9_ok = true;
        for (int br = 0; br < 2; ++br) {
            const ConvLayer* L = last_up(n, br);
            if (ok) {
                ConvForm c = f.form(*L, hl, wl);
                c.tail = true; c.tail_form = 1;
                ok = conv3x3_rw_applicable(c);
            }
            ps4_ok = ps4_ok && L && ps4_tail_applicable(B, hl, wl, L->slope);
            ps9_ok = ps9_ok && L && ps9_tail_applicable(B, hl, wl, L->slope);
        }
        f.tail_form = ok ? 1 : 0;
        ps4 = ok && n.opt.up_impl == 1 && ps4_ok && (2 * wl) % 8 == 0;
        ps9 = fuse && n.opt.up_impl == 1 && n.r == 3 && f.groups >= 3 && ps9_ok;
    }
}

template <typename Args, typename Launch>
int ArsbRun::ps_stage(int br, const std::string& key, const Act& cur, size_t plane_bytes, size_t apron_bytes, const char* name, Launch launch)
{
    ps_plane[br] = (float*)f.ar.take(plane_bytes + 4096);
    ps_apron[br] = (float*)f.ar.take(apron_bytes + 4096);
    if (!f.dry()) {
        const ConvLayer& L = n.convs[n.conv_index.at(key)];
        Args q{};
        q.in = cur.hi; q.wpk = f.blob<half_t>(L.w_hi); q.bias = L.has_bias ? f.blob<float>(L.bias) : f.small<float>("zero_bias");
        q.tail_w = f.small<half_t>(br == 0 ? "tail_r.frag" : "tail_u.frag");
        q.plane = ps_plane[br]; q.apron = ps_apron[br]; q.slope = L.slope; q.B = B; q.H = H; q.W = W;
        q.split = (f.mixed && f.tail_split_for(key)) ? 1 : 0;
        const int rec = f.prof_begin(key, 2.0 * (double)B * H * W * L.cout * L.cin * L.taps);
        bool done = false;
        for (int rep = f.repeats(key); rep > 0; --rep) done = launch(q, f.groups, f.s);
        f.prof_end(rec);
        if (!done) return fail(MOE_EINVAL, "fused tail kernel (%s) rejected layer %s", name, key.c_str());
    }
    H *= n.r; W *= n.r;
    return (int)MOE_OK;
}

int ArsbRun::run_branch(int br, Act cur)
{
    if (f.mixed) { cur.drop_lo(); cur.lo8 = false; }
    H = h; W = w;
    for (int st = 0; st < n.stages; ++st) {
        const std::string key = std::string(br == 0 ? "convt_R1" : "u") + ".up" + std::to_string(st);
        if (ps4 && st == n.stages - 1) {
            if (int rc = ps_stage<Ps4Args>(br, key, cur, ps4_plane_bytes(B, H, W), ps4_apron_bytes(B, H, W), "ps4", launch_conv3x3_ps4)) return rc;
            continue;
        }
        if (ps9 && st == n.stages - 1) {
            if (int rc = ps_stage<Ps9Args>(br, key, cur, ps9_plane_bytes(B, H, W), ps9_apron_bytes(B, H, W), "ps9", launch_conv3x3_ps9)) return rc;
            continue;
        }
        if (fuse && st == n.stages - 1) {
            tp[br] = (float*)f.ar.take(f.tail_form == 1 ? (size_t)tailsum_layout(B, H, W).total * 4 + 4096 : (size_t)9 * B * H * n.r * W * n.r * 4 + 4096);
            ConvExtra tail;
            tail.fuse_tail = true; tail.tail_w = f.small<half_t>(br == 0 ? "tail_r.frag" : "tail_u.frag"); tail.tplanes = tp[br];
            if (!f.conv(key, cur, Act{}, nullptr, H, W, tail))
                return fail(MOE_EINVAL, "fused tail kernel rejected layer %s", key.c_str());
            H *= n.r; W *= n.r;
            continue;
        }
        Act nxt = f.act((long long)B * H * n.r * W * n.r);
        f.conv(key, cur, nxt, nullptr, H, W);
        H *= n.r; W *= n.r;
        f.tap(std::string(br == 0 ? "r" : "u") + ".up" + std::to_string(st), nxt, H, W, 64, 64);
        cur = nxt;
    }
    fin[br] = cur;
    return (int)MOE_OK;
}

int ArsbRun::trunk_conv(const std::string& key, const Act& in, const Act& out, const Act* res, bool exact)
{
    ConvExtra e;
    e.exact = exact;
    if (!f.conv(key, in, out, res, h, w, e))
        return fail(MOE_EINVAL, "layer %s: %d planes of %dx%d exceed the conv kernel's addressing range (use smaller tiles)", key.c_str(), B, h, w);
    return (int)MOE_OK;
}

int ArsbRun::run_trunk()
{
    if (int rc = trunk_conv("input2", A, Bb, nullptr, mixed)) return rc;
    f.tap("input2", Bb, h, w, 64, n.C);
    const bool arsb_fuse = n.opt.arsb_fuse && !f.x3 && !f.direct && n.opt.conv_impl == 2;
    hipStream_t s = f.s;
    Act cur = Bb, oth = Cc;
    for (int i = 1; i <= 6; ++i) {
        const bool ex = mixed && i <= nx;
        const std::string k1 = "c1_" + std::to_string(i), k2 = "c2_" + std::to_string(i);
        const ConvLayer& L1 = n.convs[n.conv_index.at(k1)];
        const ConvLayer& L2 = n.convs[n.conv_index.at(k2)];
        const bool trunk64 = L1.w_arsb != 0;
        const int cin = (L1.cin == 48 && L2.cin == 48 && n.opt.k48) ? 48 : 64;
        const bool drop6 = mixed && i == 6 && n.arch != MOE_ARCH_NETDN && !n.debug;
        if (arsb_fuse && !ex && (!mixed || (cur.has_lo && oth.has_lo)) && trunk64 && arsb32c_applicable(B, h, w, L1.slope, mixed, mixed, cin)) {
            if (!f.dry()) {
                ArsbArgs q{};
                q.x_hi = cur.hi; q.x_lo = mixed ? cur.lo : nullptr; q.y_hi = oth.hi; q.y_lo = mixed ? oth.lo : nullptr;
                q.w1 = f.blob<half_t>(L1.w_hi); q.w2 = f.blob<half_t>(L2.w_hi); q.zero = f.small<half_t>("zero");
                q.slope = L1.slope; q.B = B; q.H = h; q.W = w; q.cin = cin;
                q.drop_lo = drop6 ? 1 : 0;
                const bool trace = n.opt.arsb_trace;
                const size_t tb = 8 * 16 * 4 * 40 * 8;
                if (trace && i == 3 && hipMalloc((void**)&q.trace, tb) == hipSuccess) (void)hipMemsetAsync(q.trace, 0, tb, s);
                const int rec = f.prof_begin("arsb" + std::to_string(i), 2.0 * 2.0 * (double)B * h * w * L1.cout * L1.cin * 9);
                bool done = false;
                for (int rep = f.repeats("arsb" + std::to_string(i)); rep > 0; --rep) done = launch_arsb32c(q, f.groups, s);
                f.prof_end(rec);
                if (q.trace) {
                    std::vector<unsigned long long> host(tb / 8);
                    (void)hipStreamSynchronize(s);
                    (void)hipMemcpy(host.data(), q.trace, tb, hipMemcpyDeviceToHost);
                    if (FILE* fp = fopen("/tmp/arsb_trace.bin", "wb")) { fwrite(host.data(), 1, tb, fp); fclose(fp); }
                    (void)hipFree(q.trace);
                }
                if (!done) return fail(MOE_EINVAL, "internal error: arsb32c rejected layer %s its predicate took", k1.c_str());
            }
            std::swap(cur, oth); cur.lo8 = oth.lo8 = false;
            Act seen = cur;
            if (drop6) seen.drop_lo();
            f.tap("arsb" + std::to_string(i), seen, h, w, 64, n.C);
            continue;
        }
        if (ex && chain8 && n.opt.exact_fuse && n.opt.q8_impl == 1 && cur.lo8 && cur.has_lo && oth.has_lo && L1.wq_hi8 && L2.wq_hi8 && !L1.has_bias && !L2.has_bias && L2.slope == 1.f &&
            arsb_sq_applicable(B, h, w, L1.slope)) {
            if (!f.dry()) {
                ArsbSqArgs q{};
                q.x_hi = cur.hi; q.x_lo8 = (const unsigned char*)cur.lo; q.y_hi = oth.hi; q.y_lo = oth.lo;
                q.w16[0] = f.blob<half_t>(L1.w_hi); q.wh8[0] = f.blob<unsigned char>(L1.wq_hi8); q.wl8[0] = f.blob<unsigned char>(L1.wq_lo8);
                q.w16[1] = f.blob<half_t>(L2.w_hi); q.wh8[1] = f.blob<unsigned char>(L2.wq_hi8); q.wl8[1] = f.blob<unsigned char>(L2.wq_lo8);
                q.slope = L1.slope; q.B = B; q.H = h; q.W = w; q.out8 = i < nx;
                const int rec = f.prof_begin("xpair" + std::to_string(i), 2.0 * 2.0 * 3.0 * (double)B * h * w * L1.cout * L1.cin * 9);
                const bool done = launch_arsb_sq(q, f.groups, s);
                f.prof_end(rec);
                if (!done) return fail(MOE_EINVAL, "internal error: arsb_sq rejected layer %s its predicate took", k1.c_str());
            }
            std::swap(cur, oth);
            cur.lo8 = i < nx;
            oth.lo8 = false;
            f.tap("arsb" + std::to_string(i), cur, h, w, 64, n.C);
            continue;
        }
        Act m = oth;
        if (mixed && !ex) m.drop_lo();
        m.lo8 = ex && chain8;
        Act bin = cur;
        if (mixed && !ex) bin.drop_lo();
        if (int rc = trunk_conv(k1, bin, m, nullptr, ex)) return rc;
        const Act resid = cur;
        if (ex && chain8 && i == nx) { cur.lo = lo16x ? lo16x : A.lo; cur.lo8 = false; }
        if (int rc = trunk_conv(k2, m, cur, &resid, ex)) return rc;
        f.tap("arsb" + std::to_string(i), cur, h, w, 64, n.C);
    }
    Bb = cur;
    return (int)MOE_OK;
}

template <typename Args, typename Launch>
void ArsbRun::tail_add(Launch launch)
{
    if (f.dry()) return;
    Args t{};
    t.p0 = ps_plane[0]; t.p1 = ps_plane[1]; t.a0 = ps_apron[0]; t.a1 = ps_apron[1];
    t.y = f.io.y; t.y_dtype = f.io.y_dtype; t.y_off = f.io.y_off; t.B = B; t.H = H; t.W = W; t.px = (W / n.r + kTileW - 1) / kTileW;
    t.vec_ok = f.y_vec;
    const int rec = f.prof_begin("tailadd", 0.0);
    f.gate();
    launch(t, f.s);
    f.prof_end(rec);
}

int ArsbRun::branch_sum()
{
    if (ps4) { tail_add<TailAddArgs>(launch_tailadd); return MOE_OK; }
    if (ps9) { tail_add<TailAdd3Args>(launch_tailadd3); return MOE_OK; }
    if (fuse) {
        if (!f.dry()) {
            TapSumArgs t{};
            t.t0 = tp[0]; t.t1 = tp[1]; t.y = f.io.y; t.y_dtype = f.io.y_dtype; t.y_off = f.io.y_off; t.B = B; t.H = H; t.W = W; t.r = n.r;
            t.form = f.tail_form;
            t.vec_ok = n.r == 2 && f.y_vec && W % 8 == 0;
            f.gate();
            launch_tapsum(t, f.s);
        }
        return MOE_OK;
    }
    f.tail(&fin[0], &fin[1], H, W, false);
    return MOE_OK;
}

int ArsbRun::run()
{
    const long long P = (long long)B * h * w;
    hipStream_t s = f.s;
    mixed = f.mixed;
    nx = mixed ? exact_blocks_of(n) : 0;
    f.drop_taps();
    A = f.act(P, 64, mixed); Bb = f.act(P, 64, mixed); Cc = f.act(P, 64, mixed);
    if (mixed && n.opt.conv_impl != 2)
        return fail(MOE_EINVAL, "precision 'mixed' runs on the fast 3x3 kernels only: conv_impl=v1 (MOE_CONV_IMPL=v1) is a debugging switch for 'fp16' / 'fp16x3'");
    const bool dn = n.arch == MOE_ARCH_NETDN;
    chain8 = mixed && f.use_q8() && n.opt.lo8 && !n.debug && !f.direct && nx >= 1 && A.has_lo && Bb.has_lo && Cc.has_lo;
    if (dn && (int)n.scalars.at("tail_taps") != 9) chain8 = false;
    for (int i = 0; chain8 && i <= nx; ++i)
        for (int j = (i == 0 ? 2 : 1); chain8 && j <= 2; ++j)
            chain8 = f.q8_capable(n.convs[n.conv_index.at(i == 0 ? std::string("input2") : "c" + std::to_string(j) + "_" + std::to_string(i))]);
    lo16x = (dn && chain8) ? (half_t*)f.ar.take((size_t)P * 64 * 2 + 2048) : nullptr;
    A.lo8 = Bb.lo8 = chain8;
    f.stem(A);
    f.tap("stem", A, h, w, 64, n.C);
    plan_tail_form();
    const bool forked = sr && f.ctx.fork && !n.debug && !f.direct && !f.x3 && n.opt.conv_impl == 2 && (long long)B * h * w <= 4ll * 65536;
    struct ForkGuard {
        StreamSet* set; hipStream_t s; bool armed = false;
        ~ForkGuard()
        {
            if (!armed) return;
            if (hipEventRecord(set->ev_join, set->side) != hipSuccess || hipStreamWaitEvent(s, set->ev_join, 0) != hipSuccess) (void)hipStreamSynchronize(set->side);
        }
    } fork_guard{f.ctx.set, s};
    const int all = f.groups;
    int g_side = 0;
    if (forked && all >= 32) {
        g_side = n.opt.branch_groups > 0 ? n.opt.branch_groups : (n.stages >= 2 ? 5 * all / 16 : 3 * all / 16);
        g_side = std::max(8, std::min(g_side, all - 8) / 8 * 8);
    }
    if (forked) {
        if (g_side) f.groups = g_side;
        if (!f.dry()) {
            StreamSet& set = *f.ctx.set;
            if (!set.side) {
                HIP_TRY(hipStreamCreateWithFlags(&set.side, hipStreamNonBlocking));
                HIP_TRY(hipEventCreateWithFlags(&set.ev_fork, hipEventDisableTiming));
                HIP_TRY(hipEventCreateWithFlags(&set.ev_join, hipEventDisableTiming));
            }
            HIP_TRY(hipEventRecord(set.ev_fork, s));
            HIP_TRY(hipStreamWaitEvent(set.side, set.ev_fork, 0));
            f.s = set.side;
            fork_guard.armed = true;
        }
        const int rc = run_branch(1, A);
        if (g_side) f.groups = all - g_side;
        if (!f.dry()) {
            f.s = s;
            if (!rc) HIP_TRY(hipEventRecord(f.ctx.set->ev_join, f.ctx.set->side));
        }
        if (rc) return rc;
    }
    if (int rc = run_trunk()) return rc;
    if (n.arch == MOE_ARCH_NETDN) { f.tail(&Bb, &A, h, w, false); return MOE_OK; }
    if (mixed) { A.drop_lo(); Bb.drop_lo(); A.lo8 = Bb.lo8 = false; }
    if (!forked) { if (int rc = run_branch(0, Bb)) return rc; if (int rc = run_branch(1, A)) return rc; }
    else {
        if (int rc = run_branch(0, Bb)) return rc;
        if (!f.dry()) { HIP_TRY(hipStreamWaitEvent(s, f.ctx.set->ev_join, 0)); fork_guard.armed = false; }
        f.groups = all;
    }
    return branch_sum();
}

}

int moe::forward_arsb(const moe_net& n, Fwd& f)
{
    ArsbRun r{n, f, f.B, f.h, f.w};
    return r.run();
}
```

moephoto_amd/csrc/net.h:

```cpp
#pragma once
#include "engine.h"

#include <algorithm>
#include <cmath>
#include <cstdarg>
#include <cstdio>
#include <cstdlib>
#include <cstring>
#include <map>
#include <memory>
#include <utility>

namespace moe {

int fail(int code, const char* fmt, ...);
int launched(const char* who);

inline bool plane_depth(int depth) { return depth == 8 || depth == 10 || depth == 12 || depth == 16; }

#define HIP_TRY(expr)                                                                                    \
    do {                                                                                                 \
        hipError_t e_ = (expr);                                                                          \
        if (e_ != hipSuccess) return fail(e_ == hipErrorOutOfMemory ? MOE_ENOMEM : MOE_EHIP, "%s: %s", #expr, hipGetErrorString(e_)); \
    } while (0)

struct DevBuf {
    void* p = nullptr;
    size_t bytes = 0;
    template <typename... A> int grow(size_t need, hipStream_t s, const char* does_not_fit, A... a)
    {
        if (need <= bytes) return MOE_OK;
        if (p) { HIP_TRY(hipStreamSynchronize(s)); HIP_TRY(hipFree(p)); p = nullptr; bytes = 0; }
        if (hipMalloc(&p, need) != hipSuccess) { (void)hipGetLastError(); p = nullptr; return fail(MOE_ENOMEM, does_not_fit, a...); }
        bytes = need;
        return MOE_OK;
    }
    void release() { if (p) (void)hipFree(p); p = nullptr; bytes = 0; }
};

struct Param {
    std::string name;
    std::vector<int64_t> shape;
    std::vector<float> data;
    bool set = false;
    int64_t numel() const { int64_t n = 1; for (auto d : shape) n *= d; return n; }
};

struct ConvLayer {
    int taps = 9, nseg = 1, nchunks = 1, r = 1;
    int cin = 64, cout = 64, k = 3;
    float slope = 1.f, scale = 1.f;
    bool per_plane = false;
    size_t w_hi = 0, w_lo = 0, bias = 0, bias_img = 0, w_plain = 0, bias_plain = 0, w_pk32 = 0;
    size_t w_arsb_lo = 0;
    size_t wq_hi8 = 0, wq_lo8 = 0;
    size_t w_arsb = 0;
    size_t w_x3 = 0;
    bool has_x3 = false;
    bool has_bias = false;
    int nfrag() const { return nseg * taps * 8; }
};

struct Act {
    half_t* hi = nullptr; half_t* lo = nullptr; bool lo8 = false; bool has_lo = false;
    void drop_lo() { lo = nullptr; has_lo = false; }
};

struct Arena {
    char* base = nullptr;
    size_t off = 0;
    size_t limit = 0;
    bool overflow = false;
    void* take(size_t bytes)
    {
        const size_t a = (off + 255) & ~(size_t)255;
        off = a + bytes;
        if (base && off > limit) { overflow = true; base = nullptr; }
        return base ? base + a : nullptr;
    }
};

struct NetOptions {
    int conv_impl = 2;
    int sp_impl = 1;
    int tail_split = 1;
    int tail_form = 1;
    int up_fuse2 = 1;
    int up_impl = 1;
    int conv1x1 = 1;
    int x3_fuse = 1;
    int arsb_fuse = 1;
    int lo8 = 1;
    int x3_impl = 0;
    int k48 = 1;
    int s64 = 1;
    int branch_streams = 1;
    int branch_groups = 0;
    int exact_fuse = 1;
    int q8_impl = 1;
    int fuse_tail = 1;
    int sedn_fuse = 1;
    int pool_fuse = 1;
    int lite_lut = 1;
    int stem2 = 1;
    int frm_pre = 1;
    int overlap_calls = 1;
    int overlap_fork = 0;
    int overlap_groups = 0;
    int calib_log = 0;
    int auto_calibrate = 1;
    int exact_blocks_env = -1;
    int tiles_per_batch = 0;
    int max_groups = 0;
    int dbg = 0;
    std::string trace_key = "convt_R1.up1";
    bool arsb_trace = false;
    std::string repeat_key;
    int repeat_n = 1;


    bool set(const std::string& key, const char* v);
    void from_env();
};

struct StreamSet { DevBuf ws; hipStream_t side = nullptr; hipEvent_t ev_fork = nullptr, ev_join = nullptr; };
struct PipeSet : StreamSet { hipStream_t main = nullptr; hipEvent_t entry = nullptr, done = nullptr; };

struct NetRuntime {
    struct ProfRec { hipEvent_t e0 = nullptr, e1 = nullptr; int key = 0; double flops = 0; };
    std::vector<ProfRec> prof_ev;
    size_t prof_used = 0;
    struct Tap { float* dev = nullptr; int64_t shape[4] = {0, 0, 0, 0}; };
    std::map<std::string, Tap> taps;
    struct OffSlot { long long* host = nullptr; long long* dev = nullptr; size_t cap = 0; hipEvent_t done = nullptr; bool used = false; };
    OffSlot off_ring[4];
    int off_next = 0;
};

}

struct moe_net {
    int arch = 0, scale = 1;
    moe::NetOptions opt;
    int C = 64;
    int stages = 1, r = 2;
    std::vector<moe::Param> params;
    std::map<std::string, int> index;
    bool finalized = false;
    int device = -1, precision = MOE_PREC_FP16;
    int exact_blocks = -1;
    bool calib_valid = false;
    float* lut = nullptr; int lut_state = 0;
    int calib_blocks = -1;
    double calib_err = 0.0;
    int auto_resolved = -1;
    char* blob = nullptr;
    size_t blob_bytes = 0;
    std::vector<moe::ConvLayer> convs;
    std::map<std::string, int> conv_index;
    std::map<std::string, size_t> small;
    std::map<std::string, float> scalars;
    int max_groups = 256;
    std::vector<std::string> prof_keys;
    bool debug = false;
    bool tap_only = false;
    bool tapping() const { return debug || tap_only; }
    moe::StreamSet set;
    moe::PipeSet pipe[2];
    int pipe_next = 0;
    bool pipe_prev_valid = false;
    hipStream_t pipe_last_stream = nullptr;
    moe::NetRuntime rt;
    moe::DevBuf ens_pad, ens_canvas;

    const moe::Param* get(const std::string& n) const
    {
        auto it = index.find(n);
        return it == index.end() ? nullptr : &params[it->second];
    }
    void add(const std::string& n, std::vector<int64_t> shape)
    {
        index[n] = (int)params.size();
        moe::Param p; p.name = n; p.shape = std::move(shape);
        params.push_back(std::move(p));
    }
};

namespace moe {

struct FwdIO {
    const void* x = nullptr; int x_dtype = MOE_F32; long long sB = 0, sH = 0, sW = 0; const long long* x_off = nullptr;
    void* y = nullptr; int y_dtype = MOE_F32; const long long* y_off = nullptr;
};

struct FwdCtx {
    StreamSet* set = nullptr;
    int groups = 0;
    bool fork = false;
    hipEvent_t gate_event = nullptr;
    float* lut_capture = nullptr;
};
inline FwdCtx own_ctx(const moe_net& n, StreamSet* set) { return FwdCtx{set, n.max_groups, n.opt.branch_streams != 0, nullptr, nullptr}; }

struct ConvExtra {
    const half_t* plane_w = nullptr;
    const half_t* plane_w_lo = nullptr;
    const half_t* tail_w = nullptr;
    float* tplanes = nullptr;
    const float* tail1_w = nullptr;
    float* tail1_out = nullptr;
    bool exact = false;
    float* pool_out = nullptr;
    int pool_slabs = 0;
    bool pool_act = false;
    const float* gate_in = nullptr;
    bool fuse_tail = false, fuse_tail1 = false, pool = false, gate = false;
};
struct ConvDone {
    bool ok = true;
    bool pooled = false;
    bool gated = false;
    int tail1_parts = 0;
    explicit operator bool() const { return ok; }
};
enum class ConvKernel {
    none, direct, conv1x1,
    mfma, sp, rw, ps4_store,
    sp_res_lo,
    mfma_x3,
    x3, q8, sq,
    sp_three, acc32,
};
struct ConvRoute {
    ConvKernel kernel = ConvKernel::none;
    ConvDone done;
    ConvForm form;
    ConvX3Form x3;
};
const char* kernel_name(ConvKernel k);

struct Fwd {
    const moe_net& n;
    const FwdCtx& ctx;
    NetRuntime* rt;
    hipStream_t s;
    int B, h, w;
    Arena ar;
    int groups;
    bool x3, direct;
    bool mixed = false;
    bool y_vec = false;
    float* acc32 = nullptr;
    size_t acc32_elems = 0;
    half_t* side16 = nullptr;
    bool dry() const { return ar.base == nullptr; }
    int rc = 0;
    bool skips_planned_work = false;
    int tail_form = 0;
    FwdIO io;

    Act act(long long pixels, int ch = 64, bool want_lo = false)
    {
        Act a;
        a.hi = (half_t*)ar.take((size_t)pixels * ch * 2 + 2048);
        if (x3 || want_lo) { a.lo = (half_t*)ar.take((size_t)pixels * ch * 2 + 2048); a.has_lo = true; }
        return a;
    }
    template <typename T> T* blob(size_t off) const { return (T*)(n.blob + off); }
    template <typename T> T* small(const std::string& k) const { return (T*)(n.blob + n.small.at(k)); }

    void tap(const std::string& name, const Act& a, int H, int W, int cs, int C)
    {
        if (!n.tapping() || dry()) return;
        auto forget = [&](const std::string& k) {
            auto it = rt->taps.find(k);
            if (it != rt->taps.end()) { if (it->second.dev) (void)hipFree(it->second.dev); rt->taps.erase(it); }
        };
        if (a.lo && a.lo8) {
            float* v = tap_alloc(name, H, W, C);
            float* w8 = tap_alloc(name + ".w8", H, W, C);
            if (v && w8) launch_nhwc8_to_nchw_f32(a.hi, (const unsigned char*)a.lo, v, w8, B, H, W, cs, C, s);
            else { forget(name); forget(name + ".w8"); }
        } else {
            tap_part(name, a.hi, a.lo, H, W, cs, C);
            forget(name + ".w8");
        }
        if (a.lo) tap_part(name + ".hi", a.hi, nullptr, H, W, cs, C);
        else forget(name + ".hi");
    }
    float* tap_alloc(const std::string& name, int H, int W, int C)
    {
        auto& t = rt->taps[name];
        if (t.dev) { (void)hipFree(t.dev); t.dev = nullptr; }
        if (hipMalloc((void**)&t.dev, (size_t)B * C * H * W * 4) != hipSuccess) { t.dev = nullptr; return nullptr; }
        t.shape[0] = B; t.shape[1] = C; t.shape[2] = H; t.shape[3] = W;
        return t.dev;
    }
    void tap_part(const std::string& name, const half_t* hi, const half_t* lo, int H, int W, int cs, int C)
    {
        auto& t = rt->taps[name];
        if (t.dev) { (void)hipFree(t.dev); t.dev = nullptr; }
        const size_t nel = (size_t)B * C * H * W;
        if (hipMalloc((void**)&t.dev, nel * 4) != hipSuccess) return;
        t.shape[0] = B; t.shape[1] = C; t.shape[2] = H; t.shape[3] = W;
        launch_nhwc_to_nchw_f32(hi, lo, t.dev, B, H, W, cs, C, s);
    }
    void drop_taps()
    {
        if (!n.tapping() || dry()) return;
        for (auto& t : rt->taps) if (t.second.dev) (void)hipFree(t.second.dev);
        rt->taps.clear();
    }
    void tap_raw16(const std::string& name, const half_t* p, long long per)
    {
        if (!n.tapping() || dry()) return;
        tap_part(name, p, nullptr, 1, 1, (int)per, (int)per);
    }
    void tap_f32(const std::string& name, const float* p, long long per)
    {
        if (!n.tapping() || dry()) return;
        auto& t = rt->taps[name];
        if (t.dev) { (void)hipFree(t.dev); t.dev = nullptr; }
        if (hipMalloc((void**)&t.dev, (size_t)B * per * 4) != hipSuccess) return;
        t.shape[0] = B; t.shape[1] = per; t.shape[2] = 1; t.shape[3] = 1;
        if (hipMemcpyAsync(t.dev, p, (size_t)B * per * 4, hipMemcpyDeviceToDevice, s) != hipSuccess) { (void)hipGetLastError(); (void)hipFree(t.dev); t.dev = nullptr; }
    }

    bool tail_split_for(const std::string& key) const
    {
        const int mode = n.opt.tail_split;
        return mode == 2 || (mode == 1 && key.compare(0, 8, "convt_R1") == 0);
    }

    int prof_begin(const std::string& key, double flops)
    {
        for (size_t i = 0; i < n.prof_keys.size(); ++i) {
            if (key.find(n.prof_keys[i]) == std::string::npos) continue;
            if (rt->prof_used == rt->prof_ev.size()) {
                NetRuntime::ProfRec r;
                if (hipEventCreate(&r.e0) != hipSuccess || hipEventCreate(&r.e1) != hipSuccess) return -1;
                rt->prof_ev.push_back(r);
            }
            NetRuntime::ProfRec& r = rt->prof_ev[rt->prof_used];
            r.key = (int)i; r.flops = flops;
            (void)hipEventRecord(r.e0, s);
            return (int)rt->prof_used++;
        }
        return -1;
    }
    void prof_end(int rec) { if (rec >= 0) (void)hipEventRecord(rt->prof_ev[rec].e1, s); }
    int repeats(const std::string& key) const { return (!n.opt.repeat_key.empty() && key.find(n.opt.repeat_key) != std::string::npos) ? n.opt.repeat_n : 1; }

    bool use_q8() const { return mixed && (n.opt.x3_impl == 2 || (n.opt.x3_impl == 0 && (n.scale > 1 || n.arch == MOE_ARCH_NETDN))); }
    bool q8_capable(const ConvLayer& L) const
    {
        ConvX3Form c;
        c.B = B; c.H = h; c.W = w; c.slope = L.slope; c.in8 = c.out8 = true;
        return n.opt.x3_fuse && n.opt.conv_impl == 2 && L.k == 3 && L.r == 1 && L.nchunks == 1 && L.nseg == 1 && !L.per_plane && L.wq_hi8 && L.w_arsb_lo && !L.has_bias && conv64_q8_applicable(c);
    }

    ConvDone conv(const std::string& key, const Act& in, const Act& out, const Act* res, int H, int W, const ConvExtra& extra = ConvExtra{});
    ConvRoute route(const std::string& key, const Act& in, const Act& out, const Act* res, int H, int W, const ConvExtra& extra = ConvExtra{}) const;
    ConvForm form(const ConvLayer& L, int H, int W) const;
    int launch(const ConvRoute& r, const std::string& key, const Act& in, const Act& out, const Act* res, const ConvExtra& extra);
    void stem(const Act& out, const Act* out2 = nullptr);
    void tail(const Act* r, const Act* u, int H, int W, bool skip);
    void gate();
};

int forward_arsb(const moe_net& n, Fwd& f);
int forward_sedn(const moe_net& n, Fwd& f);
int forward_lite(const moe_net& n, Fwd& f);

int exact_blocks_of(const moe_net& n);
int default_exact_blocks(int arch);
long long sp_bytes_per_pixel(const moe_net& n);
constexpr long long kSpRange = (1ll << 32) - (1ll << 16);
int forward_dev(moe_net& n, const FwdIO& io, int B, int h, int w, hipStream_t s, bool y_off_mult8, const FwdCtx& ctx);
void free_set(StreamSet& set);
void pipe_destroy(moe_net& n);
void free_records(NetRuntime& rt);
inline void free_ens_scratch(moe_net& n) { n.ens_pad.release(); n.ens_canvas.release(); }
int build_device_weights(moe_net& n, int precision);
void drop_lut(moe_net& n);
bool calibratable(const moe_net& n);
int calibrate_blocks(moe_net& n, double target, hipStream_t s);
int calibrate_sedn(moe_net& n, double target, hipStream_t s, bool adopt);

}
```

moephoto_amd/csrc/options.cpp:

```cpp
#include "net.h"

using namespace moe;

namespace {

enum OptionKind {
    kFlag,
    kWords,
    kCount,
    kInt,
    kText,
    kRepeat,
};
struct OptionWord { const char* word; int value; };
struct OptionRow {
    const char* key;
    const char* env;
    OptionKind kind;
    int NetOptions::*num;
    std::string NetOptions::*text;
    OptionWord words[3];
};
constexpr OptionWord kOnOff[] = {{"0", 0}, {"off", 0}, {"1", 1}, {"on", 1}};

const OptionRow kOptionTable[] = {
    {"conv_impl", "MOE_CONV_IMPL", kWords, &NetOptions::conv_impl, nullptr, {{"sp", 2}, {"v1", 0}}},
    {"sp_impl", "MOE_SP_IMPL", kWords, &NetOptions::sp_impl, nullptr, {{"sp", 0}, {"auto", 1}, {"rw", 2}}},
    {"tail_split", "MOE_TAIL_SPLIT", kWords, &NetOptions::tail_split, nullptr, {{"0", 0}, {"r", 1}, {"ru", 2}}},
    {"tail_form", "MOE_TAIL_FORM", kWords, &NetOptions::tail_form, nullptr, {{"planes", 0}, {"sums", 1}}},
    {"up_impl", "MOE_UP_IMPL", kWords, &NetOptions::up_impl, nullptr, {{"rw", 0}, {"ps4", 1}}},
    {"up_fuse2", "MOE_UP_FUSE2", kFlag, &NetOptions::up_fuse2},
    {"conv1x1", "MOE_CONV1X1", kFlag, &NetOptions::conv1x1},
    {"q8_impl", "MOE_Q8_IMPL", kWords, &NetOptions::q8_impl, nullptr, {{"s", 1}, {"p", 0}}},
    {"exact_fuse", "MOE_EXACT_FUSE", kFlag, &NetOptions::exact_fuse},
    {"branch_streams", "MOE_BRANCH_STREAMS", kFlag, &NetOptions::branch_streams},
    {"branch_groups", "MOE_BRANCH_GROUPS", kCount, &NetOptions::branch_groups},
    {"auto_calibrate", "MOE_AUTO_CALIBRATE", kFlag, &NetOptions::auto_calibrate},
    {"overlap_calls", "MOE_OVERLAP_CALLS", kFlag, &NetOptions::overlap_calls},
    {"overlap_groups", "MOE_OVERLAP_GROUPS", kCount, &NetOptions::overlap_groups},
    {"overlap_fork", "MOE_OVERLAP_FORK", kFlag, &NetOptions::overlap_fork},
    {"s64", "MOE_S64", kFlag, &NetOptions::s64},
    {"k48", "MOE_K48", kFlag, &NetOptions::k48},
    {"x3_impl", "MOE_X3_IMPL", kWords, &NetOptions::x3_impl, nullptr, {{"auto", 0}, {"x3", 1}, {"q8", 2}}},
    {"lo8", "MOE_LO8", kFlag, &NetOptions::lo8},
    {"x3_fuse", "MOE_X3_FUSE", kFlag, &NetOptions::x3_fuse},
    {"arsb_fuse", "MOE_ARSB_FUSE", kFlag, &NetOptions::arsb_fuse},
    {"fuse_tail", "MOE_FUSE_TAIL", kFlag, &NetOptions::fuse_tail},
    {"sedn_fuse", "MOE_SEDN_FUSE", kFlag, &NetOptions::sedn_fuse},
    {"pool_fuse", "MOE_POOL_FUSE", kFlag, &NetOptions::pool_fuse},
    {"frm_pre", "MOE_FRM_PRE", kFlag, &NetOptions::frm_pre},
    {"stem2", "MOE_STEM2", kFlag, &NetOptions::stem2},
    {"lite_lut", "MOE_LITE_LUT", kFlag, &NetOptions::lite_lut},
    {"dbg", "MOE_DBG", kInt, &NetOptions::dbg},
    {"trace_key", "MOE_TRACE_KEY", kText, nullptr, &NetOptions::trace_key},
    {"tiles_per_batch", "MOE_TILES_PER_BATCH", kCount, &NetOptions::tiles_per_batch},
    {"max_groups", "MOE_MAX_GROUPS", kCount, &NetOptions::max_groups},
    {"calib_log", nullptr, kFlag, &NetOptions::calib_log},
    {"repeat", nullptr, kRepeat},
};

bool word_value(const OptionWord* words, size_t n, const char* v, int& out)
{
    for (size_t i = 0; i < n; ++i)
        if (words[i].word && !strcmp(v, words[i].word)) { out = words[i].value; return true; }
    return false;
}

}

bool NetOptions::set(const std::string& key, const char* v)
{
    if (!v) return false;
    for (const OptionRow& r : kOptionTable) {
        if (key != r.key) continue;
        int t = 0;
        switch (r.kind) {
            case kFlag: if (!word_value(kOnOff, 4, v, t)) return false; break;
            case kWords: if (!word_value(r.words, 3, v, t)) return false; break;
            case kCount: if ((t = atoi(v)) < 0) return false; break;
            case kInt: t = atoi(v); break;
            case kText: this->*r.text = v; return true;
            case kRepeat: {
                const char* c = strrchr(v, ':');
                if (!c) {
                    if (*v && strcmp(v, "0")) return false;
                    repeat_key.clear(); repeat_n = 1;
                    return true;
                }
                const int cnt = atoi(c + 1);
                if (cnt < 1 || c == v) return false;
                repeat_key.assign(v, c - v); repeat_n = cnt;
                return true;
            }
        }
        this->*r.num = t;
        return true;
    }
    return false;
}

void NetOptions::from_env()
{
    for (const OptionRow& r : kOptionTable)
        if (const char* e = r.env ? getenv(r.env) : nullptr)
            if (!set(r.key, e)) fprintf(stderr, "moephoto_amd: %s=\"%s\" is not a value of option %s -- ignored\n", r.env, e, r.key);

    if (const char* e = getenv("MOE_EXACT_BLOCKS")) exact_blocks_env = atoi(e);
    arsb_trace = getenv("MOE_ARSB_TRACE") != nullptr;
}

extern "C" int moe_net_set_option(moe_net* n, const char* key, const char* value)
{
    if (!n || !key || !value) return fail(MOE_EINVAL, "moe_net_set_option: NULL argument");
    if (!n->opt.set(key, value)) return fail(MOE_EINVAL, "moe_net_set_option: unknown option or value \"%s\" = \"%s\"", key, value);
    drop_lut(*n);
    if (!strcmp(key, "max_groups") && n->finalized) n->max_groups = n->opt.max_groups > 0 ? n->opt.max_groups : conv_mfma_max_groups();
    return MOE_OK;
}
```

moephoto_amd/csrc/plan_run.cpp:

```cpp
#include "net.h"

using namespace moe;

struct TileTable {
    int device = -1, n_frames = 0;
    int64_t sC = 0, sH = 0, sW = 0, frame_stride = 0;
    std::vector<int64_t> tile_dst;
    bool y_mult8 = false;
    std::vector<int> group_first, group_count;
    void* dev = nullptr;
    const long long *x_off = nullptr, *y_off = nullptr;
};

struct StitchTables {
    int device = -1, C = 0;
    void* dev = nullptr;
    long long* tile_off = nullptr;
    int *row_first = nullptr, *row_cnt = nullptr, *col_first = nullptr, *col_cnt = nullptr, *row_tab = nullptr, *col_tab = nullptr;
    float* ramp = nullptr;
    std::vector<std::pair<int, int*>> strip_tabs;
};

struct UploadedOffsets { int device; std::vector<int64_t> host; void* dev; };

struct TableRing {
    static constexpr int kSlots = 32;
    int device = -1;
    size_t slot_bytes = 0;
    char *host = nullptr, *dev = nullptr;
    hipEvent_t done[kSlots] = {};
    bool used[kSlots] = {};
    int next = 0;
};

struct PlanDevice {
    static constexpr size_t kCached = 16;
    std::vector<TileTable> tables;
    std::vector<StitchTables> stitch;
    std::vector<UploadedOffsets> uploaded;
    std::vector<TableRing> rings;
    DevBuf pool;
    ~PlanDevice()
    {
        for (auto& t : tables) (void)hipFree(t.dev);
        for (auto& t : stitch) { (void)hipFree(t.dev); for (auto& e : t.strip_tabs) (void)hipFree(e.second); }
        for (auto& u : uploaded) (void)hipFree(u.dev);
        for (auto& r : rings) {
            for (hipEvent_t e : r.done) if (e) (void)hipEventDestroy(e);
            (void)hipHostFree(r.host);
            (void)hipFree(r.dev);
        }
        pool.release();
    }
    template <typename V> static int make_room(V& v, hipStream_t s)
    {
        if (v.size() < kCached) return MOE_OK;
        HIP_TRY(hipStreamSynchronize(s));
        (void)hipFree(v.front().dev);
        v.erase(v.begin());
        return MOE_OK;
    }
};

static int upload(const void* host, size_t bytes, void** dev)
{
    HIP_TRY(hipMalloc(dev, bytes));
    const hipError_t e = hipMemcpy(*dev, host, bytes, hipMemcpyHostToDevice);
    if (e != hipSuccess) { (void)hipFree(*dev); *dev = nullptr; }
    HIP_TRY(e);
    return MOE_OK;
}

struct moe_plan { Plan p; mutable PlanDevice dev; };

static void table_rows(const Plan& p, int64_t frame_stride, int64_t sC, int64_t sH, int64_t sW, int n_frames, const int64_t* tile_dst, TileTable& d,
                       std::vector<long long>& off, std::vector<long long>& yo)
{
    int slot = 0;
    for (const auto& g : p.groups) {
        d.group_first.push_back(slot);
        const long long plane = (long long)(g.th * p.sc) * (g.tw * p.sc);
        for (int f = 0; f < n_frames; ++f)
            for (int k : g.tiles) {
                const long long at = tile_dst[(size_t)f * p.tiles.size() + k];
                if (at < 0) continue;
                const TileRect& t = p.tiles[k];
                for (int c = 0; c < p.C; ++c) {
                    off.push_back((long long)f * frame_stride + (long long)c * sC + (long long)t.top * sH + (long long)t.left * sW);
                    yo.push_back(at + (long long)c * plane);
                }
                ++slot;
            }
        d.group_count.push_back(slot - d.group_first.back());
    }
    if (off.empty()) { off.push_back(0); yo.push_back(0); }
    d.y_mult8 = true;
    for (long long v : yo) d.y_mult8 = d.y_mult8 && (v % 8 == 0);
}

static int tile_table(const moe_plan& pl, int device, int64_t frame_stride, int64_t sC, int64_t sH, int64_t sW, int n_frames, const int64_t* tile_dst,
                      hipStream_t s, const TileTable** out)
{
    const Plan& p = pl.p;
    const size_t n = p.tiles.size() * (size_t)n_frames;
    for (const TileTable& c : pl.dev.tables)
        if (c.device == device && c.sC == sC && c.sH == sH && c.sW == sW && c.frame_stride == frame_stride && c.n_frames == n_frames &&
            std::equal(c.tile_dst.begin(), c.tile_dst.end(), tile_dst)) { *out = &c; return MOE_OK; }
    int rc = PlanDevice::make_room(pl.dev.tables, s);
    if (rc) return rc;
    TileTable d;
    std::vector<long long> off, yo;
    table_rows(p, frame_stride, sC, sH, sW, n_frames, tile_dst, d, off, yo);
    off.insert(off.end(), yo.begin(), yo.end());
    rc = upload(off.data(), off.size() * 8, &d.dev);
    if (rc) return rc;
    d.x_off = (const long long*)d.dev; d.y_off = d.x_off + yo.size();
    d.device = device; d.sC = sC; d.sH = sH; d.sW = sW; d.frame_stride = frame_stride; d.n_frames = n_frames;
    d.tile_dst.assign(tile_dst, tile_dst + n);
    pl.dev.tables.push_back(std::move(d));
    *out = &pl.dev.tables.back();
    return MOE_OK;
}

static int run_sets(moe_net& n, const Plan& p, const TileTable& d, const void* img, int img_dtype, int64_t sH, int64_t sW, float* dst, int max_tiles, hipStream_t s)
{
    if (max_tiles <= 0) {
        max_tiles = n.opt.tiles_per_batch > 0 ? n.opt.tiles_per_batch : 32;
    }
    for (size_t gi = 0; gi < p.groups.size(); ++gi) {
        const auto& g = p.groups[gi];
        const int nt = d.group_count[gi];
        if (nt < 1) continue;
        const long long px = (long long)g.th * g.tw;
        const int per = (int)std::max<long long>(1, std::min<long long>(nt, (long long)max_tiles * 65536 / std::max<long long>(px, 1)));
        for (int t0 = 0; t0 < nt; t0 += per) {
            const int cnt = std::min(per, nt - t0);
            const long long slot = (long long)(d.group_first[gi] + t0) * p.C;
            int rc = forward_dev(n, FwdIO{img, img_dtype, 0, sH, sW, d.x_off + slot, dst, MOE_F32, d.y_off + slot}, cnt * p.C, g.th, g.tw, s, d.y_mult8, own_ctx(n, &n.set));
            if (rc) return rc;
        }
    }
    return MOE_OK;
}

static int stitch_tables(const moe_plan& pl, int device, int C, StitchTables** out)
{
    for (StitchTables& c : pl.dev.stitch)
        if (c.device == device && c.C == C) { *out = &c; return MOE_OK; }
    const Plan& p = pl.p;
    std::vector<long long> toff(p.tiles.size());
    for (size_t k = 0; k < toff.size(); ++k) toff[k] = p.tile_off[k] / p.C * C;
    std::vector<char> host;
    auto put = [&](const void* src, size_t bytes) { const size_t a = (host.size() + 255) & ~(size_t)255; host.resize(a + bytes); memcpy(host.data() + a, src, bytes); return a; };
    const size_t o_t = put(toff.data(), toff.size() * 8);
    const size_t o_rf = put(p.row_first.data(), p.row_first.size() * 4), o_rc = put(p.row_cnt.data(), p.row_cnt.size() * 4);
    const size_t o_cf = put(p.col_first.data(), p.col_first.size() * 4), o_cc = put(p.col_cnt.data(), p.col_cnt.size() * 4);
    const size_t o_rt = put(p.row_tab.data(), p.row_tab.size() * 4), o_ct = put(p.col_tab.data(), p.col_tab.size() * 4);
    const float zero = 0.f;
    const size_t o_rp = put(p.ramp.empty() ? &zero : p.ramp.data(), std::max<size_t>(4, p.ramp.size() * 4));
    StitchTables d;
    int rc = upload(host.data(), host.size(), &d.dev);
    if (rc) return rc;
    char* b = (char*)d.dev;
    d.device = device; d.C = C; d.tile_off = (long long*)(b + o_t);
    d.row_first = (int*)(b + o_rf); d.row_cnt = (int*)(b + o_rc); d.col_first = (int*)(b + o_cf); d.col_cnt = (int*)(b + o_cc);
    d.row_tab = (int*)(b + o_rt); d.col_tab = (int*)(b + o_ct); d.ramp = (float*)(b + o_rp);
    pl.dev.stitch.push_back(std::move(d));
    *out = &pl.dev.stitch.back();
    return MOE_OK;
}

struct OutEdge { int canvas_dtype; float quant; const StitchMix* mix = nullptr; const YuvEdge* yuv = nullptr; int planes_depth = 0; const StitchLuma* luma = nullptr;
                 const QuantDither* dq = nullptr; int yuv_dither = 0; };

struct QuantReq {
    int low = 0, dither = 0; bool unit = false; QuantDither d{};
    const QuantDither* dq() { return dither ? &d : nullptr; }
    void fill() { const float top = (float)((1 << low) - 1); d = QuantDither{unit ? top : top + 1.f, top, dither == 2}; }
};
static int quant_flags(const char* who, int arg, bool unit_ok, QuantReq* q)
{
    const int known = MOE_Q_ROUND | MOE_Q_ORDERED | MOE_Q_UNIT, flags = arg & ~0xff;
    *q = QuantReq{};
    q->low = arg;
    if (arg < 0 || (flags & ~known)) return MOE_OK;
    q->low = arg & 0xff;
    if ((flags & MOE_Q_ROUND) && (flags & MOE_Q_ORDERED)) return fail(MOE_EINVAL, "%s: MOE_Q_ROUND and MOE_Q_ORDERED are both set (one mode at most)", who);
    if ((flags & MOE_Q_UNIT) && !(flags & (MOE_Q_ROUND | MOE_Q_ORDERED))) return fail(MOE_EINVAL, "%s: MOE_Q_UNIT without MOE_Q_ROUND or MOE_Q_ORDERED (the truncating quantiser has no unit scale)", who);
    if ((flags & MOE_Q_UNIT) && !unit_ok) return fail(MOE_EINVAL, "%s: MOE_Q_UNIT does not apply to the Y'CbCr edge (its samples are quantised in integers)", who);
    if (flags && q->low == 0) return fail(MOE_EINVAL, "%s: MOE_Q_* flags beside bits = 0 (the canvas form quantises nothing)", who);
    q->dither = flags & MOE_Q_ROUND ? 1 : flags & MOE_Q_ORDERED ? 2 : 0;
    q->unit = (flags & MOE_Q_UNIT) != 0;
    return MOE_OK;
}
static int stitch(const moe_plan& pl, int device, const float* tiles, const int64_t* tile_off, bool off_on_host, int C, void* out, int out_dtype, const int* band, hipStream_t s,
                  const OutEdge* edge = nullptr)
{
    const Plan& p = pl.p;
    HIP_TRY(hipSetDevice(device));
    StitchTables* d = nullptr;
    int rc = stitch_tables(pl, device, C, &d);
    if (rc) return rc;
    const long long* toff = tile_off ? (const long long*)tile_off : d->tile_off;
    if (tile_off && off_on_host) {
        const size_t nt = p.tiles.size();
        toff = nullptr;
        for (auto& c : pl.dev.uploaded)
            if (c.device == device && std::equal(c.host.begin(), c.host.end(), tile_off)) { toff = (const long long*)c.dev; break; }
        if (!toff) {
            void* up = nullptr;
            rc = PlanDevice::make_room(pl.dev.uploaded, s);
            if (!rc) rc = upload(tile_off, nt * 8, &up);
            if (rc) return rc;
            pl.dev.uploaded.push_back(UploadedOffsets{device, std::vector<int64_t>(tile_off, tile_off + nt), up});
            toff = (const long long*)up;
        }
    }
    StitchArgs a{};
    a.tiles = tiles; a.tile_off = toff;
    a.row_first = d->row_first; a.row_cnt = d->row_cnt; a.col_first = d->col_first; a.col_cnt = d->col_cnt;
    a.row_tab = d->row_tab; a.col_tab = d->col_tab; a.ramp = d->ramp;
    a.out = out; a.out_dtype = out_dtype; a.C = C; a.out_h = p.out_h; a.out_w = p.out_w; a.step_w = p.aw.step;
    a.y0 = 0; a.rows = p.out_h; a.row_lo = 0;
    if (band) {
        const int row0 = band[0], row1 = band[1], nrow = p.ah.step;
        a.row_lo = row0;
        a.y0 = p.row_tab[row0 * 4 + 1];
        a.rows = (row1 < nrow ? p.row_tab[row1 * 4 + 1] : p.out_h) - a.y0;
        if (band[2] && row1 < nrow) {
            int* tab = nullptr;
            for (auto& e : d->strip_tabs) if (e.first == row1) tab = e.second;
            if (!tab) {
                std::vector<int> rt(p.row_tab);
                rt[row1 * 4 + 2] = rt[row1 * 4 + 0];
                rt[row1 * 4 + 3] = rt[row1 * 4 + 1] - rt[row1 * 4 + 0];
                rc = upload(rt.data(), rt.size() * 4, (void**)&tab);
                if (rc) return rc;
                d->strip_tabs.push_back({row1, tab});
            }
            a.row_tab = tab;
        }
    }
    if (edge && edge->yuv) {
        launch_stitch_yuv(a, *edge->yuv, s, edge->yuv_dither);
        return launched("stitch_yuv");
    }
    if (edge && edge->planes_depth) {
        launch_stitch_planes(a, edge->canvas_dtype, edge->planes_depth, s, edge->dq);
        return launched("stitch_planes");
    }
    if (edge && edge->luma) {
        if (!launch_stitch_luma(a, *edge->luma, edge->canvas_dtype, s, edge->dq)) return fail(MOE_EINVAL, "moe_stitch_luma: %d pool planes (1 or 2 are supported)", C);
        return launched("stitch_luma");
    }
    if (edge && edge->mix) {
        if (!launch_stitch_mix(a, *edge->mix, edge->canvas_dtype, s, edge->dq)) return fail(MOE_EINVAL, "moe_stitch_mix: %d planes (1 to 4 are supported)", C + (edge->mix->alpha ? 1 : 0));
        return launched("stitch_mix");
    }
    if (edge) {
        if (!launch_stitch_out(a, edge->canvas_dtype, edge->quant, s, edge->dq)) return fail(MOE_EINVAL, "moe_stitch_out: %d planes (1 to 4 are supported)", C);
        return launched("stitch_out");
    }
    launch_stitch(a, s);
    return launched("stitch");
}

static int out_edge_args(const char* who, int planes, int canvas_dtype, int bits, const void* dst, int dst_dtype)
{
    if (!dst) return fail(MOE_EINVAL, "%s: NULL argument", who);
    if (planes < 1 || planes > 4) return fail(MOE_EINVAL, "%s: %d planes (1 to 4 are supported)", who, planes);
    if (canvas_dtype != MOE_F32 && canvas_dtype != MOE_F16) return fail(MOE_EINVAL, "%s: canvas dtype must be MOE_F32 or MOE_F16", who);
    if (bits != 8 && bits != 16) return fail(MOE_EINVAL, "%s: %d bits (8 or 16)", who, bits);
    if (dst_dtype != MOE_U8 && dst_dtype != MOE_U16) return fail(MOE_EINVAL, "%s: dst dtype must be MOE_U8 or MOE_U16", who);
    if (dst_dtype == MOE_U8 && bits > 8) return fail(MOE_EINVAL, "%s: %d bits do not fit MOE_U8", who, bits);
    return MOE_OK;
}

static int plane_edge_args(const char* who, int planes, int canvas_dtype, int depth, const void* dst, OutEdge* edge)
{
    if (!dst) return fail(MOE_EINVAL, "%s: NULL argument", who);
    if (planes < 1 || planes > 4) return fail(MOE_EINVAL, "%s: %d planes (1 to 4 are supported)", who, planes);
    if (canvas_dtype != MOE_F32 && canvas_dtype != MOE_F16) return fail(MOE_EINVAL, "%s: canvas dtype must be MOE_F32 or MOE_F16", who);
    if (!plane_depth(depth)) return fail(MOE_EINVAL, "%s: depth %d (8, 10, 12 or 16)", who, depth);
    if (depth > 8 && ((uintptr_t)dst & 1)) return fail(MOE_EINVAL, "%s: dst is not 2-byte aligned (depth %d: uint16 samples)", who, depth);
    *edge = OutEdge{canvas_dtype, (float)(1 << depth)};
    edge->planes_depth = depth;
    return MOE_OK;
}

static int yuv_edge_args(const char* who, int planes, int dtype, int depth, int matrix, int order, const void* dst, YuvEdge* y)
{
    static const int tab[3][3][3] = {{{3483, 11718, 1183}, {-1877, -6315, 8192}, {8192, -7441, -751}},
                                     {{4899, 9617, 1868}, {-2765, -5427, 8192}, {8192, -6860, -1332}},
                                     {{4304, 11108, 972}, {-2288, -5904, 8192}, {8192, -7533, -659}}};
    if (!dst) return fail(MOE_EINVAL, "%s: NULL argument", who);
    if (planes != 3) return fail(MOE_EINVAL, "%s: the plan has %d planes (C must be 3)", who, planes);
    if (dtype != MOE_F32 && dtype != MOE_F16) return fail(MOE_EINVAL, "%s: canvas dtype must be MOE_F32 or MOE_F16", who);
    if (depth != 8 && depth != 10 && depth != 12 && depth != 16) return fail(MOE_EINVAL, "%s: depth %d (8, 10, 12 or 16)", who, depth);
    if (matrix < MOE_YUV_BT709 || matrix > MOE_YUV_BT2020NC) return fail(MOE_EINVAL, "%s: unknown matrix %d", who, matrix);
    if (order != MOE_ORDER_BGR && order != MOE_ORDER_RGB) return fail(MOE_EINVAL, "%s: unknown order %d", who, order);
    for (int p = 0; p < 3; ++p) {
        const int colour = order == MOE_ORDER_BGR ? 2 - p : p;
        y->ky[p] = tab[matrix][0][colour]; y->ku[p] = tab[matrix][1][colour]; y->kv[p] = tab[matrix][2][colour];
    }
    y->mul_y = 219u << (depth - 6); y->base_y = 16u << (depth - 8);
    y->mul_c = 224 << (depth - 8); y->base_c = 128 << (depth - 8);
    y->depth = depth; y->f16 = dtype == MOE_F16;
    return MOE_OK;
}

static int mix_edge_args(const char* who, const Plan& p, int planes, const void* inp, int inp_dtype, int64_t sC, int64_t sH, int64_t sW, const void* alpha, int64_t aH, int64_t aW,
                         double strength, int bits, const void* dst, int dst_dtype, StitchMix* m)
{
    if (!inp || !dst) return fail(MOE_EINVAL, "%s: NULL argument", who);
    if (p.sc != 1) return fail(MOE_EINVAL, "%s: plan scale %d (the blend with the input needs a plan of scale 1)", who, p.sc);
    if (bits != 0 && bits != 8 && bits != 16) return fail(MOE_EINVAL, "%s: %d bits (0 = the canvas, 8 or 16)", who, bits);
    if (inp_dtype != MOE_F32 && inp_dtype != MOE_F16) return fail(MOE_EINVAL, "%s: canvas dtype (the input's) must be MOE_F32 or MOE_F16", who);
    if (bits == 0 && dst_dtype != inp_dtype) return fail(MOE_EINVAL, "%s: dst dtype must be the input's for the canvas form (bits = 0)", who);
    if (bits != 0 && dst_dtype != MOE_U8 && dst_dtype != MOE_U16) return fail(MOE_EINVAL, "%s: dst dtype must be MOE_U8 or MOE_U16 for %d bits", who, bits);
    if (bits > 8 && dst_dtype == MOE_U8) return fail(MOE_EINVAL, "%s: %d bits do not fit MOE_U8", who, bits);
    if (planes < 1 || planes + (alpha ? 1 : 0) > 4) return fail(MOE_EINVAL, "%s: %d planes%s (1 to 4 in all are supported)", who, planes, alpha ? " + alpha" : "");
    if (!std::isfinite(strength)) return fail(MOE_EINVAL, "%s: strength must be finite", who);
    *m = StitchMix{inp, sC, sH, sW, alpha, aH, aW, (float)strength, (float)(1.0 - strength), strength != 1.0, bits ? (float)(1 << bits) : 0.f, 0, 0, 0, 0};
    return MOE_OK;
}

static LumaCoef luma_coef(int matrix)
{
    static const double K[3][2] = {{0.2126, 0.0722}, {0.299, 0.114}, {0.2627, 0.0593}};
    const double kr = K[matrix][0], kb = K[matrix][1], kg = 1 - kr - kb;
    const double eb = 2 * (1 - kb), er = 2 * (1 - kr);
    return LumaCoef{(float)kr, (float)kg, (float)kb, (float)(1 / eb), (float)(1 / er), (float)eb, (float)er, (float)(kr * er / kg), (float)(kb * eb / kg)};
}

static int luma_edge_args(const char* who, int planes, int dtype, const void* c, int matrix, int order, int bits, const void* dst, int dst_dtype, StitchLuma* m)
{
    if (!c || !dst) return fail(MOE_EINVAL, "%s: NULL argument", who);
    if (planes != 3 && planes != 4) return fail(MOE_EINVAL, "%s: %d colour planes (3, or 4 with alpha)", who, planes);
    if (dtype != MOE_F32 && dtype != MOE_F16) return fail(MOE_EINVAL, "%s: canvas dtype must be MOE_F32 or MOE_F16", who);
    if (matrix < MOE_YUV_BT709 || matrix > MOE_YUV_BT2020NC) return fail(MOE_EINVAL, "%s: unknown matrix %d", who, matrix);
    if (order != MOE_ORDER_BGR && order != MOE_ORDER_RGB) return fail(MOE_EINVAL, "%s: unknown order %d", who, order);
    if (bits != 0 && bits != 8 && bits != 16) return fail(MOE_EINVAL, "%s: %d bits (0 = the canvas, 8 or 16)", who, bits);
    if (bits == 0 && dst_dtype != dtype) return fail(MOE_EINVAL, "%s: dst dtype must be the canvas dtype for the canvas form (bits = 0)", who);
    if (bits != 0 && dst_dtype != MOE_U8 && dst_dtype != MOE_U16) return fail(MOE_EINVAL, "%s: dst dtype must be MOE_U8 or MOE_U16 for %d bits", who, bits);
    if (bits > 8 && dst_dtype == MOE_U8) return fail(MOE_EINVAL, "%s: %d bits do not fit MOE_U8", who, bits);
    if ((uintptr_t)c & 3) return fail(MOE_EINVAL, "%s: c is not 4-byte aligned (fp32 planes)", who);
    const uintptr_t es = dst_dtype == MOE_F32 ? 4 : dst_dtype == MOE_U8 ? 1 : 2;
    if ((uintptr_t)dst & (es - 1)) return fail(MOE_EINVAL, "%s: dst is not aligned to its %d-byte elements", who, (int)es);
    *m = StitchLuma{(const float*)c, luma_coef(matrix), order == MOE_ORDER_RGB ? 0 : 2, bits ? (float)(1 << bits) : 0.f};
    return MOE_OK;
}

static int run_plan(const char* who, moe_net* n, const moe_plan* pl, const void* img, int img_dtype, int64_t sC, int64_t sH, int64_t sW,
                    void* out, int out_dtype, int max_tiles, float* pool, int shard_index, int shard_count, int do_stitch, void* stream, const OutEdge* edge)
{
    if (!n || !pl || !img || (do_stitch && !out)) return fail(MOE_EINVAL, "%s: NULL argument", who);
    if (!n->finalized) return fail(MOE_ESTATE, "%s: net is not finalized", who);
    const Plan& p = pl->p;
    if (p.sc != n->scale) return fail(MOE_EINVAL, "%s: plan scale %d != net scale %d", who, p.sc, n->scale);
    if (shard_count < 1) { shard_count = 1; shard_index = 0; }
    if (shard_index < 0 || shard_index >= shard_count) return fail(MOE_EINVAL, "%s: shard %d of %d", who, shard_index, shard_count);
    hipStream_t s = (hipStream_t)stream;
    HIP_TRY(hipSetDevice(n->device));
    std::vector<int64_t> at(p.tile_off.begin(), p.tile_off.end());
    for (size_t k = 0; k < at.size(); ++k) if ((int)(k % shard_count) != shard_index) at[k] = -1;
    const TileTable* d = nullptr;
    int rc = tile_table(*pl, n->device, 0, sC, sH, sW, 1, at.data(), s, &d);
    if (rc) return rc;
    if (!pool) {
        rc = pl->dev.pool.grow(p.pool_elems_per_plane_set * 4, s, "tile pool of %zu bytes does not fit", p.pool_elems_per_plane_set * 4);
        if (rc) return rc;
        pool = (float*)pl->dev.pool.p;
    }
    rc = run_sets(*n, p, *d, img, img_dtype, sH, sW, pool, max_tiles, s);
    if (rc || !do_stitch) return rc;
    return stitch(*pl, n->device, pool, nullptr, false, p.C, out, out_dtype, nullptr, s, edge);
}

static int ring_slot(const moe_plan& pl, int device, TableRing** ring, int* slot)
{
    TableRing* r = nullptr;
    for (TableRing& c : pl.dev.rings) if (c.device == device) r = &c;
    if (!r) {
        TableRing t;
        t.device = device;
        t.slot_bytes = (std::max<size_t>(1, pl.p.tiles.size() * (size_t)pl.p.C) * 16 + 255) & ~(size_t)255;
        HIP_TRY(hipMalloc((void**)&t.dev, t.slot_bytes * TableRing::kSlots));
        hipError_t e = hipHostMalloc((void**)&t.host, t.slot_bytes * TableRing::kSlots, hipHostMallocDefault);
        for (int i = 0; i < TableRing::kSlots && e == hipSuccess; ++i) e = hipEventCreateWithFlags(&t.done[i], hipEventDisableTiming);
        if (e != hipSuccess) {
            for (hipEvent_t ev : t.done) if (ev) (void)hipEventDestroy(ev);
            if (t.host) (void)hipHostFree(t.host);
            (void)hipFree(t.dev);
        }
        HIP_TRY(e);
        pl.dev.rings.push_back(t);
        r = &pl.dev.rings.back();
    }
    const int i = r->next;
    if (r->used[i]) {
        const hipError_t e = hipEventQuery(r->done[i]);
        if (e == hipErrorNotReady) HIP_TRY(hipEventSynchronize(r->done[i]));
        else HIP_TRY(e);
    }
    r->next = (i + 1) % TableRing::kSlots;
    *ring = r; *slot = i;
    return MOE_OK;
}

extern "C" {

int moe_plan_create(const int64_t shape[3], double ram, double ram_coef, int pad, int scale, int align, int cropsize, moe_plan** out)
{
    if (!shape || !out) return fail(MOE_EINVAL, "moe_plan_create: NULL argument");
    auto p = std::make_unique<moe_plan>();
    std::string err;
    int rc = build_plan(p->p, shape, ram, ram_coef, pad, scale, align, cropsize, err);
    if (rc) return fail(rc, "%s", err.c_str());
    *out = p.release();
    return MOE_OK;
}

void moe_plan_destroy(moe_plan* p)
{
    delete p;
}

int moe_plan_info(const moe_plan* p, int64_t info[12])
{
    if (!p || !info) return fail(MOE_EINVAL, "moe_plan_info: NULL argument");
    const Plan& q = p->p;
    const int64_t v[12] = {(int64_t)q.tiles.size(), q.ah.step, q.aw.step, q.out_h, q.out_w, q.pad_h_to, q.pad_w_to, q.pad_sc,
                           q.tile_h, q.tile_w, q.ah.clip, q.aw.clip};
    memcpy(info, v, sizeof v);
    return MOE_OK;
}

int moe_plan_rows(const moe_plan* p, int32_t* rows)
{
    if (!p || !rows) return fail(MOE_EINVAL, "moe_plan_rows: NULL argument");
    memcpy(rows, p->p.row_tab.data(), p->p.row_tab.size() * 4);
    return MOE_OK;
}

static void axis_seams(const std::vector<int>& tab, int i, int out[4])
{
    const int n = (int)tab.size() / 4;
    const int o = tab[i * 4 + 2], ext = tab[i * 4 + 3];
    std::vector<std::pair<int, int>> iv;
    for (int k = 0; k < n; ++k) {
        const int a = std::max(tab[k * 4 + 0] - o, 0), b = std::min(tab[k * 4 + 1] - o, ext);
        if (b > a) iv.push_back({a, b});
    }
    std::sort(iv.begin(), iv.end());
    std::vector<std::pair<int, int>> m;
    for (auto& v : iv) {
        if (!m.empty() && v.first <= m.back().second) m.back().second = std::max(m.back().second, v.second);
        else m.push_back(v);
    }
    while (m.size() > 2) { m[1].second = m.back().second; m.pop_back(); }
    out[0] = out[1] = out[2] = out[3] = 0;
    if (m.size() >= 1) { out[0] = m[0].first; out[1] = m[0].second; out[2] = out[3] = m[0].second; }
    if (m.size() == 2) { out[2] = m[1].first; out[3] = m[1].second; }
}

int moe_plan_seams(const moe_plan* p, int32_t* seams)
{
    if (!p || !seams) return fail(MOE_EINVAL, "moe_plan_seams: NULL argument");
    const Plan& q = p->p;
    for (int i = 0; i < q.ah.step; ++i)
        for (int j = 0; j < q.aw.step; ++j) {
            int r[4], c[4];
            axis_seams(q.row_tab, i, r);
            axis_seams(q.col_tab, j, c);
            int32_t* o = seams + ((size_t)i * q.aw.step + j) * 8;
            for (int e = 0; e < 4; ++e) { o[e] = r[e]; o[4 + e] = c[e]; }
        }
    return MOE_OK;
}

static_assert(sizeof(moe_wire_rec) == sizeof(WireRec) && sizeof(WireRec) == 64, "moe_wire_rec layout");

int64_t moe_wire_words(const moe_wire_rec* rec)
{
    if (!rec) return -1;
    WireRec r;
    memcpy(&r, rec, sizeof r);
    return wire_rec_words(r);
}

static int wire_call(bool pack, float* tiles, void* wire, const moe_wire_rec* recs_dev, int n, int64_t max_elems, void* stream)
{
    if (n < 0 || (n > 0 && (!tiles || !wire || !recs_dev))) return fail(MOE_EINVAL, "moe_wire_%s: bad argument", pack ? "pack" : "unpack");
    launch_wire(pack, tiles, (unsigned*)wire, (const WireRec*)recs_dev, n, max_elems, (hipStream_t)stream);
    return launched("wire kernel");
}

int moe_wire_pack(const float* tiles_dev, void* wire_dev, const moe_wire_rec* recs_dev, int n, int64_t max_elems, void* stream)
{
    return wire_call(true, (float*)tiles_dev, wire_dev, recs_dev, n, max_elems, stream);
}

int moe_wire_unpack(float* tiles_dev, const void* wire_dev, const moe_wire_rec* recs_dev, int n, int64_t max_elems, void* stream)
{
    return wire_call(false, tiles_dev, (void*)wire_dev, recs_dev, n, max_elems, stream);
}

int moe_plan_tiles(const moe_plan* p, int32_t* tiles)
{
    if (!p || !tiles) return fail(MOE_EINVAL, "moe_plan_tiles: NULL argument");
    for (size_t k = 0; k < p->p.tiles.size(); ++k) {
        const TileRect& t = p->p.tiles[k];
        const int32_t v[8] = {t.top, t.bottom, t.left, t.right, t.top_t, t.left_t, t.bsc, t.rsc};
        memcpy(tiles + k * 8, v, sizeof v);
    }
    return MOE_OK;
}

int moe_plan_ramp(const moe_plan* p, float* ramp)
{
    if (!p || !ramp) return fail(MOE_EINVAL, "moe_plan_ramp: NULL argument");
    memcpy(ramp, p->p.ramp.data(), p->p.ramp.size() * 4);
    return MOE_OK;
}

int64_t moe_plan_pool_elems(const moe_plan* p, int C)
{
    if (!p || C < 1) return fail(MOE_EINVAL, "moe_plan_pool_elems: bad argument");
    return (int64_t)(p->p.pool_elems_per_plane_set / p->p.C * C);
}

int moe_plan_tile_offsets(const moe_plan* p, int C, int64_t* off)
{
    if (!p || !off || C < 1) return fail(MOE_EINVAL, "moe_plan_tile_offsets: bad argument");
    for (size_t k = 0; k < p->p.tiles.size(); ++k) off[k] = p->p.tile_off[k] / p->p.C * C;
    return MOE_OK;
}

int moe_stitch(const moe_plan* p, int device, const float* tiles_dev, const int64_t* tile_off, int C, void* out, int out_dtype, void* stream)
{
    if (!p || !tiles_dev || !out || C < 1) return fail(MOE_EINVAL, "moe_stitch: bad argument");
    return stitch(*p, device, tiles_dev, tile_off, true, C, out, out_dtype, nullptr, (hipStream_t)stream);
}

int moe_stitch_dev(const moe_plan* p, int device, const float* tiles_dev, const int64_t* tile_off_dev, int C, void* out, int out_dtype, void* stream)
{
    if (!p || !tiles_dev || !tile_off_dev || !out || C < 1) return fail(MOE_EINVAL, "moe_stitch_dev: bad argument");
    return stitch(*p, device, tiles_dev, tile_off_dev, false, C, out, out_dtype, nullptr, (hipStream_t)stream);
}

int moe_stitch_band(const moe_plan* p, int device, const float* tiles_dev, const int64_t* tile_off_dev, int C, void* out, int out_dtype,
                    int row0, int row1, int strip, void* stream)
{
    if (!p || !tiles_dev || !tile_off_dev || !out || C < 1) return fail(MOE_EINVAL, "moe_stitch_band: bad argument");
    const int nrow = p->p.ah.step;
    if (row0 < 0 || row1 <= row0 || row1 > nrow) return fail(MOE_EINVAL, "moe_stitch_band: tile rows [%d, %d) of %d", row0, row1, nrow);
    const int band[3] = {row0, row1, strip};
    return stitch(*p, device, tiles_dev, tile_off_dev, false, C, out, out_dtype, band, (hipStream_t)stream);
}

int moe_stitch_out(const moe_plan* p, int device, const float* tiles_dev, const int64_t* tile_off_dev, int C, int canvas_dtype, int bits, void* dst, int dst_dtype, void* stream)
{
    if (!p || !tiles_dev || C < 1) return fail(MOE_EINVAL, "moe_stitch_out: bad argument");
    QuantReq q;
    if (int rc = quant_flags("moe_stitch_out", bits, true, &q)) return rc;
    bits = q.low;
    const int rc = out_edge_args("moe_stitch_out", C, canvas_dtype, bits, dst, dst_dtype);
    if (rc) return rc;
    q.fill();
    OutEdge edge{canvas_dtype, (float)(1 << bits)};
    edge.dq = q.dq();
    return stitch(*p, device, tiles_dev, tile_off_dev, false, C, dst, dst_dtype, nullptr, (hipStream_t)stream, &edge);
}

int moe_stitch_planes(const moe_plan* p, int device, const float* tiles_dev, const int64_t* tile_off_dev, int C, int canvas_dtype, int depth, void* dst, void* stream)
{
    if (!p || !tiles_dev) return fail(MOE_EINVAL, "moe_stitch_planes: NULL argument");
    OutEdge edge{};
    QuantReq q;
    if (int rc = quant_flags("moe_stitch_planes", depth, true, &q)) return rc;
    depth = q.low;
    const int rc = plane_edge_args("moe_stitch_planes", C, canvas_dtype, depth, dst, &edge);
    if (rc) return rc;
    q.fill();
    edge.dq = q.dq();
    return stitch(*p, device, tiles_dev, tile_off_dev, false, C, dst, depth == 8 ? MOE_U8 : MOE_U16, nullptr, (hipStream_t)stream, &edge);
}

int moe_stitch_mix(const moe_plan* p, int device, const float* tiles_dev, const int64_t* tile_off_dev, int C, const void* inp, int inp_dtype, int64_t sC, int64_t sH, int64_t sW,
                   const void* alpha, int64_t aH, int64_t aW, double strength, int bits, void* dst, int dst_dtype, void* stream)
{
    if (!p || !tiles_dev) return fail(MOE_EINVAL, "moe_stitch_mix: NULL argument");
    StitchMix m{};
    QuantReq q;
    if (int rc = quant_flags("moe_stitch_mix", bits, true, &q)) return rc;
    bits = q.low;
    const int rc = mix_edge_args("moe_stitch_mix", p->p, C, inp, inp_dtype, sC, sH, sW, alpha, aH, aW, strength, bits, dst, dst_dtype, &m);
    if (rc) return rc;
    q.fill();
    OutEdge edge{inp_dtype, m.quant, &m};
    edge.dq = q.dq();
    return stitch(*p, device, tiles_dev, tile_off_dev, false, C, dst, dst_dtype, nullptr, (hipStream_t)stream, &edge);
}

int moe_stitch_yuv(const moe_plan* p, int device, const float* tiles_dev, const int64_t* tile_off_dev, int canvas_dtype, int depth, int matrix, int order, void* dst, void* stream)
{
    if (!p || !tiles_dev) return fail(MOE_EINVAL, "moe_stitch_yuv: NULL argument");
    YuvEdge y{};
    QuantReq q;
    if (int rc = quant_flags("moe_stitch_yuv", depth, false, &q)) return rc;
    depth = q.low;
    const int rc = yuv_edge_args("moe_stitch_yuv", p->p.C, canvas_dtype, depth, matrix, order, dst, &y);
    if (rc) return rc;
    OutEdge edge{canvas_dtype, 0.f};
    edge.yuv = &y;
    edge.yuv_dither = q.dither;
    return stitch(*p, device, tiles_dev, tile_off_dev, false, 3, dst, depth == 8 ? MOE_U8 : MOE_U16, nullptr, (hipStream_t)stream, &edge);
}

int moe_stitch_luma(const moe_plan* p, int device, const float* tiles_dev, const int64_t* tile_off_dev, int P, int canvas_dtype, const void* c, int matrix, int order,
                    int bits, void* dst, int dst_dtype, void* stream)
{
    if (!p || !tiles_dev) return fail(MOE_EINVAL, "moe_stitch_luma: NULL argument");
    if (P != 1 && P != 2) return fail(MOE_EINVAL, "moe_stitch_luma: %d pool planes (1: Y', or 2: Y' and alpha)", P);
    StitchLuma m{};
    QuantReq q;
    if (int rc = quant_flags("moe_stitch_luma", bits, true, &q)) return rc;
    bits = q.low;
    const int rc = luma_edge_args("moe_stitch_luma", P + 2, canvas_dtype, c, matrix, order, bits, dst, dst_dtype, &m);
    if (rc) return rc;
    q.fill();
    if ((uintptr_t)tiles_dev & 3) return fail(MOE_EINVAL, "moe_stitch_luma: tiles_dev is not 4-byte aligned (fp32 pool)");
    OutEdge edge{canvas_dtype, m.quant};
    edge.luma = &m;
    edge.dq = q.dq();
    return stitch(*p, device, tiles_dev, tile_off_dev, false, P, dst, dst_dtype, nullptr, (hipStream_t)stream, &edge);
}

int moe_blend_tile(const void* r, int64_t r_sC, int64_t r_sH, void* canvas, int64_t c_sC, int64_t c_sH, int dtype, int C,
                   int top_sc, int left_sc, int bsc, int rsc, int topT, int leftT, int pad_sc, const void* ramp, void* stream)
{
    if (!r || !canvas || C < 1) return fail(MOE_EINVAL, "moe_blend_tile: NULL argument");
    if (dtype != MOE_F32 && dtype != MOE_F16) return fail(MOE_EINVAL, "moe_blend_tile: dtype must be MOE_F32 or MOE_F16");
    const int rh = bsc - top_sc, rw = rsc - left_sc;
    if (rh < 1 || rw < 1 || top_sc < 0 || left_sc < 0 || pad_sc < 0) return fail(MOE_EINVAL, "moe_blend_tile: empty or negative window (%d..%d, %d..%d)", top_sc, bsc, left_sc, rsc);
    auto band = [&](int lt, int l, int& first, int& solid) {
        if (lt < 0) lt += l;
        if (lt < 1) { first = solid = 0; return true; }
        first = lt - pad_sc; solid = lt;
        return first >= 0 && lt <= l;
    };
    BlendTileArgs a{};
    if (!band(topT, rh, a.r0, a.lt_h) || !band(leftT, rw, a.c0, a.lt_w))
        return fail(MOE_EINVAL, "moe_blend_tile: blend band outside the window (topT %d, leftT %d, pad_sc %d, window %d x %d)", topT, leftT, pad_sc, rh, rw);
    if ((a.lt_h > a.r0 || a.lt_w > a.c0) && !ramp) return fail(MOE_EINVAL, "moe_blend_tile: ramp is NULL");
    a.r = r; a.canvas = canvas; a.ramp = ramp; a.r_sC = r_sC; a.r_sH = r_sH; a.c_sC = c_sC; a.c_sH = c_sH;
    a.C = C; a.rh = rh; a.rw = rw; a.top_sc = top_sc; a.left_sc = left_sc;
    launch_blend_tile(a, dtype == MOE_F16, (hipStream_t)stream);
    return launched("blend");
}

int moe_run_plan_ex(moe_net* n, const moe_plan* pl, const void* img, int img_dtype, int64_t sC, int64_t sH, int64_t sW,
                    void* out, int out_dtype, int max_tiles, float* pool, int shard_index, int shard_count, int do_stitch, void* stream)
{
    return run_plan("moe_run_plan", n, pl, img, img_dtype, sC, sH, sW, out, out_dtype, max_tiles, pool, shard_index, shard_count, do_stitch, stream, nullptr);
}

int moe_run_plan_out(moe_net* n, const moe_plan* pl, const void* img, int img_dtype, int64_t sC, int64_t sH, int64_t sW,
                     int canvas_dtype, int bits, void* dst, int dst_dtype, int max_tiles, void* stream)
{
    if (!n || !pl || !img) return fail(MOE_EINVAL, "moe_run_plan_out: NULL argument");
    QuantReq q;
    if (int rc = quant_flags("moe_run_plan_out", bits, true, &q)) return rc;
    bits = q.low;
    const int rc = out_edge_args("moe_run_plan_out", pl->p.C, canvas_dtype, bits, dst, dst_dtype);
    if (rc) return rc;
    q.fill();
    OutEdge edge{canvas_dtype, (float)(1 << bits)};
    edge.dq = q.dq();
// ... 375 lines not shown
```

moephoto_amd/csrc/stitch.hip:

```cpp
#include "common.h"
#include "run_store.h"
#include "luma.h"
#include "quant.h"
#include <type_traits>
#include "../../include/moephoto_amd.h"

namespace {

__device__ __forceinline__ float stitch_pixel(const StitchArgs& a, int X, int Y, int c)
{
    const int i0 = a.row_first[Y], ni = a.row_cnt[Y];
    const int j0 = a.col_first[X], nj = a.col_cnt[X];
    float cur = 0.f;
    for (int i = max(i0, a.row_lo); i < i0 + ni; ++i) {
        const int fy = a.row_tab[i * 4 + 0], sy = a.row_tab[i * 4 + 1], oy = a.row_tab[i * 4 + 2], eh = a.row_tab[i * 4 + 3];
        for (int j = j0; j < j0 + nj; ++j) {
            const int fx = a.col_tab[j * 4 + 0], sx = a.col_tab[j * 4 + 1], ox = a.col_tab[j * 4 + 2], ew = a.col_tab[j * 4 + 3];
            const float r = a.tiles[a.tile_off[i * a.step_w + j] + ((long long)c * eh + (Y - oy)) * ew + (X - ox)];
            float v1 = r;
            if (Y < sy) v1 = cur + a.ramp[Y - fy] * (r - cur);
            float v = v1;
            if (X < sx) v = cur + a.ramp[X - fx] * (v1 - cur);
            cur = v;
        }
// ... 137 lines not shown
    static constexpr int NP = C, NOUT = C;
    typedef StitchRun<TD, 8 * C> Row;
    Quant<DITHER> q; bool f16;
    __device__ __forceinline__ int c0() const { return 0; }
    __device__ __forceinline__ int np(const StitchArgs&) const { return C; }
    __device__ __forceinline__ void emit(const StitchArgs&, int X0, int Y, const float (&cur)[C][8], Row& o) const
    {
#pragma unroll
        for (int c = 0; c < C; ++c)
#pragma unroll
            for (int e = 0; e < 8; ++e) o.e[e * C + c] = quant_sample<TD>(cur[c][e], f16, q, X0 + e, Y);
    }
    __device__ __forceinline__ void store(const StitchArgs& a, int X0, int Y, const Row& o) const { stitch_store((TD*)a.out + ((long long)Y * a.out_w + X0) * C, o); }
    __device__ __forceinline__ void pixel(const StitchArgs& a, int X, int Y, int c) const
    {
        ((TD*)a.out)[((long long)Y * a.out_w + X) * C + c] = quant_sample<TD>(stitch_pixel(a, X, Y, c), f16, q, X, Y);
    }
};

template <typename TD, int C, int R>
__global__ __launch_bounds__(256) void stitch_out_kernel(StitchArgs a, float quant, int f16)
{
    stitch_fold<R>(a, SamplesEdge<TD, C>{{quant}, f16 != 0});
}

template <typename TD, int C, int R>
__global__ __launch_bounds__(256) void stitch_out_dither_kernel(StitchArgs a, QuantDither d, int f16)
{
    stitch_fold<R>(a, SamplesEdge<TD, C, true>{{d}, f16 != 0});
}

template <typename TD, bool DITHER = false>
struct PlaneEdge {
    static constexpr int NP = 1, NOUT = 1;
    typedef StitchRun<TD, 8> Row;
    Quant<DITHER> q; bool f16;
    __device__ __forceinline__ int c0() const { return blockIdx.z; }
    __device__ __forceinline__ int np(const StitchArgs&) const { return 1; }
    __device__ __forceinline__ long long at(const StitchArgs& a, int X, int Y) const { return ((long long)blockIdx.z * a.out_h + Y) * a.out_w + X; }
    __device__ __forceinline__ void emit(const StitchArgs&, int X0, int Y, const float (&cur)[1][8], Row& o) const
    {
#pragma unroll
        for (int e = 0; e < 8; ++e) o.e[e] = quant_sample<TD>(cur[0][e], f16, q, X0 + e, Y);
    }
    __device__ __forceinline__ void store(const StitchArgs& a, int X0, int Y, const Row& o) const { stitch_store((TD*)a.out + at(a, X0, Y), o); }
    __device__ __forceinline__ void pixel(const StitchArgs& a, int X, int Y, int) const
    {
        ((TD*)a.out)[at(a, X, Y)] = quant_sample<TD>(stitch_pixel(a, X, Y, blockIdx.z), f16, q, X, Y);
    }
};

template <typename TD, int R>
__global__ __launch_bounds__(256) void stitch_planes_kernel(StitchArgs a, float quant, int f16)
{
    stitch_fold<R>(a, PlaneEdge<TD>{{quant}, f16 != 0});
}

template <typename TD, int R>
__global__ __launch_bounds__(256) void stitch_planes_dither_kernel(StitchArgs a, QuantDither d, int f16)
{
    stitch_fold<R>(a, PlaneEdge<TD, true>{{d}, f16 != 0});
}

template <typename T>
__device__ __forceinline__ T stitch_mix_mul(T h, float f)
{
#pragma clang fp contract(off)
    float p = __fmul_rn(f, (float)h);
    asm("" : "+v"(p));
    return (T)p;
}

__device__ __forceinline__ half_t stitch_mix_mul_once(half_t h, float f)
{
    unsigned r;
    const unsigned hb = __builtin_bit_cast(unsigned short, h);
    const float nz = -0.0f;
    asm("v_fma_mixlo_f16 %0, %1, %2, %3 op_sel_hi:[1,0,0]" : "=v"(r) : "v"(hb), "v"(f), "v"(nz));
    return __builtin_bit_cast(half_t, (unsigned short)(r & 0xffffu));
}
__device__ __forceinline__ float stitch_mix_mul_once(float h, float f) { return stitch_mix_mul<float>(h, f); }

template <typename T>
__device__ __forceinline__ T stitch_mix_value(float cur, T inp, float sf, float tf, bool p_once, bool q_once)
{
#pragma clang fp contract(off)
    const T c = (T)cur;
    const T hp = p_once ? stitch_mix_mul_once(c, sf) : stitch_mix_mul<T>(c, sf);
    const T hq = q_once ? stitch_mix_mul_once(inp, tf) : stitch_mix_mul<T>(inp, tf);
    return (T)__fadd_rn((float)hp, (float)hq);
}

template <typename T>
__device__ __forceinline__ void stitch_mix_load8(const T* p, long long sW, bool vec, T (&v)[8])
{
    if (vec) {
        typedef T vec_t __attribute__((ext_vector_type(16 / sizeof(T))));
        constexpr int N = 16 / sizeof(T);
#pragma unroll
        for (int k = 0; k < 8 / N; ++k) {
            const vec_t q = *(const vec_t*)(p + k * N);
#pragma unroll
            for (int e = 0; e < N; ++e) v[k * N + e] = q[e];
        }
    } else {
#pragma unroll
        for (int e = 0; e < 8; ++e) v[e] = p[e * sW];
    }
}

template <typename T, typename TD, int CT, bool DITHER = false>
struct MixEdge {
    static constexpr bool SAMPLE = !std::is_same<T, TD>::value;
    static constexpr int NP = CT, NOUT = CT;
    struct Planes { StitchRun<T, 8> p[CT]; };
    typedef typename std::conditional<SAMPLE, StitchRun<TD, 8 * CT>, Planes>::type Row;
    const StitchMix& m;
    typename std::conditional<DITHER, QuantDither, QuantNone>::type d;
    template <typename V> __device__ __forceinline__ TD quant(V v, int X, int Y) const
    {
        if constexpr (DITHER) return quant_sample<TD, true>((float)v, false, d.S, d.top, d.ordered != 0, X, Y);
        else return quant_sample<TD, false>((float)v, false, m.quant, 0.f, false, X, Y);
    }
    __device__ __forceinline__ int c0() const { return 0; }
    __device__ __forceinline__ int np(const StitchArgs& a) const { return a.C; }
    __device__ __forceinline__ void emit(const StitchArgs& a, int X0, int Y, const float (&cur)[CT][8], Row& o) const
    {
#pragma unroll
        for (int c = 0; c < CT; ++c) {
            T y[8];
            if (c >= a.C) stitch_mix_load8((const T*)m.alpha + Y * m.aH + X0 * m.aW, m.aW, m.alpha_vec != 0, y);
            else if (m.blend) {
                const long long left = sizeof(T) == 2 ? m.once_from - (((long long)c * a.out_h + Y) * a.out_w + X0) : 8;
                stitch_mix_load8((const T*)m.inp + c * m.sC + Y * m.sH + X0 * m.sW, m.sW, m.inp_vec != 0, y);
#pragma unroll
                for (int e = 0; e < 8; ++e) y[e] = stitch_mix_value<T>(cur[c][e], y[e], m.sf, m.tf, e >= left, e >= left || m.q_once);
            } else {
#pragma unroll
                for (int e = 0; e < 8; ++e) y[e] = (T)cur[c][e];
            }
#pragma unroll
            for (int e = 0; e < 8; ++e) {
                if constexpr (SAMPLE) o.e[e * CT + c] = quant(y[e], X0 + e, Y);
                else o.p[c].e[e] = y[e];
            }
        }
    }
    __device__ __forceinline__ void store(const StitchArgs& a, int X0, int Y, const Row& o) const
    {
        if constexpr (SAMPLE) stitch_store((TD*)a.out + ((long long)Y * a.out_w + X0) * CT, o);
        else {
#pragma unroll
            for (int c = 0; c < CT; ++c) stitch_store((T*)a.out + ((long long)c * a.out_h + Y) * a.out_w + X0, o.p[c]);
        }
    }
    __device__ __forceinline__ void pixel(const StitchArgs& a, int X, int Y, int c) const
    {
        T y;
        if (c >= a.C) y = ((const T*)m.alpha)[Y * m.aH + X * m.aW];
        else {
            const float cur = stitch_pixel(a, X, Y, c);
            const bool p_once = sizeof(T) == 2 && ((long long)c * a.out_h + Y) * a.out_w + X >= m.once_from;
            y = m.blend ? stitch_mix_value<T>(cur, ((const T*)m.inp)[c * m.sC + Y * m.sH + X * m.sW], m.sf, m.tf, p_once, p_once || m.q_once) : (T)cur;
        }
        if constexpr (SAMPLE) ((TD*)a.out)[((long long)Y * a.out_w + X) * CT + c] = quant(y, X, Y);
        else ((T*)a.out)[((long long)c * a.out_h + Y) * a.out_w + X] = y;
    }
};

template <typename T, typename TD, int CT, int R>
__global__ __launch_bounds__(256) void stitch_mix_kernel(StitchArgs a, StitchMix m)
{
    stitch_fold<R>(a, MixEdge<T, TD, CT>{m});
}

template <typename T, typename TD, int CT, int R>
__global__ __launch_bounds__(256) void stitch_mix_dither_kernel(StitchArgs a, StitchMix m, QuantDither d)
{
    stitch_fold<R>(a, MixEdge<T, TD, CT, true>{m, d});
}

template <typename T, typename TD, int CT, bool DITHER = false>
struct LumaEdge {
    static constexpr bool SAMPLE = !std::is_same<T, TD>::value;
    static constexpr int NP = CT - 2, NOUT = CT;
    struct Planes { StitchRun<T, 8> p[CT]; };
    typedef typename std::conditional<SAMPLE, StitchRun<TD, 8 * CT>, Planes>::type Row;
    const StitchLuma& m;
    typename std::conditional<DITHER, QuantDither, QuantNone>::type d;
    template <typename V> __device__ __forceinline__ TD quant(V v, int X, int Y) const
    {
        if constexpr (DITHER) return quant_sample<TD, true>((float)v, false, d.S, d.top, d.ordered != 0, X, Y);
        else return quant_sample<TD, false>((float)v, false, m.quant, 0.f, false, X, Y);
    }
    __device__ __forceinline__ int c0() const { return 0; }
    __device__ __forceinline__ int np(const StitchArgs&) const { return NP; }
    __device__ __forceinline__ void emit(const StitchArgs& a, int X0, int Y, const float (&cur)[NP][8], Row& o) const
    {
        const float* const pb = m.c + (long long)Y * a.out_w + X0;
        const float* const pr = pb + (long long)a.out_h * a.out_w;
        float cb[8], cr[8];
        stitch_mix_load8(pb, 1, ((uintptr_t)pb & 15) == 0, cb);
        stitch_mix_load8(pr, 1, ((uintptr_t)pr & 15) == 0, cr);
        T y[CT][8];
#pragma unroll
        for (int e = 0; e < 8; ++e) {
            luma_merge_planes<T>(m.k, (float)(T)cur[0][e], cb[e], cr[e], m.rp, y[0][e], y[1][e], y[2][e]);
            if constexpr (CT == 4) y[3][e] = luma_canon((T)cur[1][e]);
        }
#pragma unroll
        for (int c = 0; c < CT; ++c)
#pragma unroll
            for (int e = 0; e < 8; ++e) {
                if constexpr (SAMPLE) o.e[e * CT + c] = quant(y[c][e], X0 + e, Y);
                else o.p[c].e[e] = y[c][e];
            }
    }
    __device__ __forceinline__ void store(const StitchArgs& a, int X0, int Y, const Row& o) const
    {
        if constexpr (SAMPLE) stitch_store((TD*)a.out + ((long long)Y * a.out_w + X0) * CT, o);
        else {
#pragma unroll
            for (int c = 0; c < CT; ++c) stitch_store((T*)a.out + ((long long)c * a.out_h + Y) * a.out_w + X0, o.p[c]);
        }
    }
    __device__ __forceinline__ void pixel(const StitchArgs& a, int X, int Y, int c) const
    {
        T y;
        if (c == 3) y = luma_canon((T)stitch_pixel(a, X, Y, 1));
        else {
            const long long at = (long long)Y * a.out_w + X;
            y = luma_canon((T)luma_merge_px(m.k, (float)(T)stitch_pixel(a, X, Y, 0), m.c[at], m.c[(long long)a.out_h * a.out_w + at], luma_colour(c, m.rp)));
        }
        if constexpr (SAMPLE) ((TD*)a.out)[((long long)Y * a.out_w + X) * CT + c] = quant(y, X, Y);
        else ((T*)a.out)[((long long)c * a.out_h + Y) * a.out_w + X] = y;
    }
};

template <typename T, typename TD, int CT, int R>
__global__ __launch_bounds__(256) void stitch_luma_kernel(StitchArgs a, StitchLuma m)
{
    stitch_fold<R>(a, LumaEdge<T, TD, CT>{m});
}

template <typename T, typename TD, int CT, int R>
__global__ __launch_bounds__(256) void stitch_luma_dither_kernel(StitchArgs a, StitchLuma m, QuantDither d)
{
    stitch_fold<R>(a, LumaEdge<T, TD, CT, true>{m, d});
}

template <bool DITHER>
__device__ __forceinline__ unsigned yuv_round(bool ordered, int x, int y)
{
    if constexpr (DITHER) return quant_threshold(ordered, x, y) << 25;
    else return 0x80000000u;
}

__device__ __forceinline__ unsigned yuv_luma(const YuvEdge& y, unsigned p0, unsigned p1, unsigned p2, unsigned rnd = 0x80000000u)
{
    const unsigned L = __umul24(y.ky[0], p0) + __umul24(y.ky[1], p1) + __umul24(y.ky[2], p2);
    return y.base_y + (unsigned)(((unsigned long long)L * y.mul_y + (unsigned long long)rnd) >> 32);
}

__device__ __forceinline__ unsigned yuv_chroma(const int (&k)[3], const YuvEdge& y, int s0, int s1, int s2, unsigned rnd = 0x80000000u)
{
    const int M = __mul24(k[0], s0) + __mul24(k[1], s1) + __mul24(k[2], s2);
    return (unsigned)(y.base_c + (int)(((long long)M * y.mul_c + (long long)rnd) >> 32));
}

__device__ __forceinline__ int yuv_sample16(float v, bool f16) { return quant_sample<uint16_t, false>(v, f16, 65536.f, 65536.f - 1.f, false, 0, 0); }

template <typename TD, int R>
__global__ __launch_bounds__(256) void stitch_yuv_kernel(StitchArgs a, YuvEdge y)
{
    constexpr bool DITHER = false;
    const bool ordered = false;
#include "stitch_yuv_body.inc"
}

template <typename TD, int R>
__global__ __launch_bounds__(256) void stitch_yuv_dither_kernel(StitchArgs a, YuvEdge y, int ordered_)
{
    constexpr bool DITHER = true;
    const bool ordered = ordered_ != 0;
#include "stitch_yuv_body.inc"
}

template <typename TS, typename TD>
__global__ __launch_bounds__(256) void to_output_yuv_kernel(const TS* __restrict__ src, TD* __restrict__ dst, int H, int W, YuvEdge y)
{
    constexpr bool DITHER = false;
    const bool ordered = false;
#include "to_output_yuv_body.inc"
}

template <typename TS, typename TD>
__global__ __launch_bounds__(256) void to_output_yuv_dither_kernel(const TS* __restrict__ src, TD* __restrict__ dst, int H, int W, YuvEdge y, int ordered_)
{
    constexpr bool DITHER = true;
    const bool ordered = ordered_ != 0;
#include "to_output_yuv_body.inc"
}

}

void launch_stitch(const StitchArgs& a, hipStream_t s)
{
    if (a.rows <= 0) return;
    hipLaunchKernelGGL(stitch8r_kernel<4>, dim3(((a.out_w + 7) / 8 + 255) / 256, (a.rows + 3) / 4, a.C), dim3(256), 0, s, a);
}

template <typename TD>
static bool launch_stitch_out_t(const StitchArgs& a, float quant, int f16, hipStream_t s, const QuantDither* dq)
{
    constexpr int R = 4;
    const dim3 g(((a.out_w + 7) / 8 + 255) / 256, (a.rows + R - 1) / R);
    if (dq) {
        if (a.C == 1) hipLaunchKernelGGL((stitch_out_dither_kernel<TD, 1, R>), g, dim3(256), 0, s, a, *dq, f16);
        else if (a.C == 2) hipLaunchKernelGGL((stitch_out_dither_kernel<TD, 2, R>), g, dim3(256), 0, s, a, *dq, f16);
        else if (a.C == 3) hipLaunchKernelGGL((stitch_out_dither_kernel<TD, 3, R>), g, dim3(256), 0, s, a, *dq, f16);
        else if (a.C == 4) hipLaunchKernelGGL((stitch_out_dither_kernel<TD, 4, R>), g, dim3(256), 0, s, a, *dq, f16);
        else return false;
        return true;
    }
    if (a.C == 1) hipLaunchKernelGGL((stitch_out_kernel<TD, 1, R>), g, dim3(256), 0, s, a, quant, f16);
    else if (a.C == 2) hipLaunchKernelGGL((stitch_out_kernel<TD, 2, R>), g, dim3(256), 0, s, a, quant, f16);
    else if (a.C == 3) hipLaunchKernelGGL((stitch_out_kernel<TD, 3, R>), g, dim3(256), 0, s, a, quant, f16);
    else if (a.C == 4) hipLaunchKernelGGL((stitch_out_kernel<TD, 4, R>), g, dim3(256), 0, s, a, quant, f16);
    else return false;
    return true;
}

bool launch_stitch_out(const StitchArgs& a, int canvas_dtype, float quant, hipStream_t s, const QuantDither* dq)
{
    const int f16 = canvas_dtype == MOE_F16;
    return a.out_dtype == MOE_U8 ? launch_stitch_out_t<uint8_t>(a, quant, f16, s, dq) : launch_stitch_out_t<uint16_t>(a, quant, f16, s, dq);
}

template <typename TD>
static void launch_stitch_planes_t(const StitchArgs& a, float quant, int f16, hipStream_t s, const QuantDither* dq)
{
    const unsigned gx = ((a.out_w + 7) / 8 + 255) / 256;
    const bool four = (long long)gx * ((a.out_h + 3) / 4) * a.C >= 1024;
    if (dq) {
        if (four) hipLaunchKernelGGL((stitch_planes_dither_kernel<TD, 4>), dim3(gx, (a.out_h + 3) / 4, a.C), dim3(256), 0, s, a, *dq, f16);
        else hipLaunchKernelGGL((stitch_planes_dither_kernel<TD, 1>), dim3(gx, a.out_h, a.C), dim3(256), 0, s, a, *dq, f16);
    } else if (four) hipLaunchKernelGGL((stitch_planes_kernel<TD, 4>), dim3(gx, (a.out_h + 3) / 4, a.C), dim3(256), 0, s, a, quant, f16);
    else hipLaunchKernelGGL((stitch_planes_kernel<TD, 1>), dim3(gx, a.out_h, a.C), dim3(256), 0, s, a, quant, f16);
}

void launch_stitch_planes(const StitchArgs& a, int canvas_dtype, int depth, hipStream_t s, const QuantDither* dq)
{
    const int f16 = canvas_dtype == MOE_F16;
    if (depth == 8) launch_stitch_planes_t<uint8_t>(a, 256.f, f16, s, dq);
    else launch_stitch_planes_t<uint16_t>(a, (float)(1 << depth), f16, s, dq);
}

template <typename T, typename TD, int R>
static bool launch_stitch_mix_r(const StitchArgs& a, const StitchMix& m, int planes, hipStream_t s, const QuantDither* dq)
{
    const dim3 g(((a.out_w + 7) / 8 + 255) / 256, (a.rows + R - 1) / R);
    if constexpr (!std::is_same<T, TD>::value) {
        if (dq) {
            if (planes == 1) hipLaunchKernelGGL((stitch_mix_dither_kernel<T, TD, 1, R>), g, dim3(256), 0, s, a, m, *dq);
            else if (planes == 2) hipLaunchKernelGGL((stitch_mix_dither_kernel<T, TD, 2, R>), g, dim3(256), 0, s, a, m, *dq);
            else if (planes == 3) hipLaunchKernelGGL((stitch_mix_dither_kernel<T, TD, 3, R>), g, dim3(256), 0, s, a, m, *dq);
            else if (planes == 4) hipLaunchKernelGGL((stitch_mix_dither_kernel<T, TD, 4, R>), g, dim3(256), 0, s, a, m, *dq);
            else return false;
            return true;
        }
    }
    if (planes == 1) hipLaunchKernelGGL((stitch_mix_kernel<T, TD, 1, R>), g, dim3(256), 0, s, a, m);
    else if (planes == 2) hipLaunchKernelGGL((stitch_mix_kernel<T, TD, 2, R>), g, dim3(256), 0, s, a, m);
    else if (planes == 3) hipLaunchKernelGGL((stitch_mix_kernel<T, TD, 3, R>), g, dim3(256), 0, s, a, m);
    else if (planes == 4) hipLaunchKernelGGL((stitch_mix_kernel<T, TD, 4, R>), g, dim3(256), 0, s, a, m);
    else return false;
    return true;
}

template <typename T, typename TD>
static bool launch_stitch_mix_t(const StitchArgs& a, const StitchMix& m, int planes, hipStream_t s, const QuantDither* dq = nullptr)
{
    const long long blocks4 = (long long)(((a.out_w + 7) / 8 + 255) / 256) * ((a.out_h + 3) / 4);
    return blocks4 >= 1024 ? launch_stitch_mix_r<T, TD, 4>(a, m, planes, s, dq) : launch_stitch_mix_r<T, TD, 1>(a, m, planes, s, dq);
}

bool launch_stitch_mix(const StitchArgs& a, StitchMix m, int canvas_dtype, hipStream_t s, const QuantDither* dq)
{
    const int planes = a.C + (m.alpha ? 1 : 0);
    const bool f16 = canvas_dtype == MOE_F16;
    const long long V = f16 ? 8 : 4;
    m.inp_vec = m.sW == 1 && (uintptr_t)m.inp % 16 == 0 && m.sC % V == 0 && m.sH % V == 0;
    m.alpha_vec = m.alpha && m.aW == 1 && (uintptr_t)m.alpha % 16 == 0 && m.aH % V == 0;
    m.once_from = (long long)a.C * a.out_h * a.out_w / 2048 * 2048;
    m.q_once = f16 && !(m.sW == 1 && (uintptr_t)m.inp % 16 == 0);
    if (m.quant == 0.f) return f16 ? launch_stitch_mix_t<half_t, half_t>(a, m, planes, s) : launch_stitch_mix_t<float, float>(a, m, planes, s);
    if (a.out_dtype == MOE_U8) return f16 ? launch_stitch_mix_t<half_t, uint8_t>(a, m, planes, s, dq) : launch_stitch_mix_t<float, uint8_t>(a, m, planes, s, dq);
    return f16 ? launch_stitch_mix_t<half_t, uint16_t>(a, m, planes, s, dq) : launch_stitch_mix_t<float, uint16_t>(a, m, planes, s, dq);
}

template <typename T, typename TD, int R>
static bool launch_stitch_luma_r(const StitchArgs& a, const StitchLuma& m, hipStream_t s, const QuantDither* dq)
{
    const dim3 g(((a.out_w + 7) / 8 + 255) / 256, (a.rows + R - 1) / R);
    if constexpr (!std::is_same<T, TD>::value) {
        if (dq) {
            if (a.C == 1) hipLaunchKernelGGL((stitch_luma_dither_kernel<T, TD, 3, R>), g, dim3(256), 0, s, a, m, *dq);
            else if (a.C == 2) hipLaunchKernelGGL((stitch_luma_dither_kernel<T, TD, 4, R>), g, dim3(256), 0, s, a, m, *dq);
            else return false;
            return true;
        }
    }
    if (a.C == 1) hipLaunchKernelGGL((stitch_luma_kernel<T, TD, 3, R>), g, dim3(256), 0, s, a, m);
    else if (a.C == 2) hipLaunchKernelGGL((stitch_luma_kernel<T, TD, 4, R>), g, dim3(256), 0, s, a, m);
    else return false;
    return true;
}

template <typename T, typename TD>
static bool launch_stitch_luma_t(const StitchArgs& a, const StitchLuma& m, hipStream_t s, const QuantDither* dq = nullptr)
{
    const long long blocks4 = (long long)(((a.out_w + 7) / 8 + 255) / 256) * ((a.out_h + 3) / 4);
    return blocks4 >= 1024 ? launch_stitch_luma_r<T, TD, 4>(a, m, s, dq) : launch_stitch_luma_r<T, TD, 1>(a, m, s, dq);
}

bool launch_stitch_luma(const StitchArgs& a, const StitchLuma& m, int canvas_dtype, hipStream_t s, const QuantDither* dq)
{
    const bool f16 = canvas_dtype == MOE_F16;
    if (m.quant == 0.f) return f16 ? launch_stitch_luma_t<half_t, half_t>(a, m, s) : launch_stitch_luma_t<float, float>(a, m, s);
    if (a.out_dtype == MOE_U8) return f16 ? launch_stitch_luma_t<half_t, uint8_t>(a, m, s, dq) : launch_stitch_luma_t<float, uint8_t>(a, m, s, dq);
    return f16 ? launch_stitch_luma_t<half_t, uint16_t>(a, m, s, dq) : launch_stitch_luma_t<float, uint16_t>(a, m, s, dq);
}

void launch_stitch_yuv(const StitchArgs& a, const YuvEdge& y, hipStream_t s, int dither)
{
    constexpr int R = 4;
    const dim3 g(((a.out_w + 7) / 8 + 255) / 256, (a.out_h + R - 1) / R);
    if (dither) {
        const int ordered = dither == 2;
        if (y.depth == 8) hipLaunchKernelGGL((stitch_yuv_dither_kernel<uint8_t, R>), g, dim3(256), 0, s, a, y, ordered);
        else hipLaunchKernelGGL((stitch_yuv_dither_kernel<uint16_t, R>), g, dim3(256), 0, s, a, y, ordered);
    } else if (y.depth == 8) hipLaunchKernelGGL((stitch_yuv_kernel<uint8_t, R>), g, dim3(256), 0, s, a, y);
    else hipLaunchKernelGGL((stitch_yuv_kernel<uint16_t, R>), g, dim3(256), 0, s, a, y);
}

void launch_to_output_yuv(const void* src, int src_dtype, int H, int W, const YuvEdge& y, void* dst, hipStream_t s, int dither)
{
    const dim3 g(((W + 7) / 8 + 255) / 256, (H + 1) / 2);
    if (dither) {
        const int ordered = dither == 2;
        if (src_dtype == MOE_F16) {
            if (y.depth == 8) hipLaunchKernelGGL((to_output_yuv_dither_kernel<half_t, uint8_t>), g, dim3(256), 0, s, (const half_t*)src, (uint8_t*)dst, H, W, y, ordered);
            else hipLaunchKernelGGL((to_output_yuv_dither_kernel<half_t, uint16_t>), g, dim3(256), 0, s, (const half_t*)src, (uint16_t*)dst, H, W, y, ordered);
        } else {
            if (y.depth == 8) hipLaunchKernelGGL((to_output_yuv_dither_kernel<float, uint8_t>), g, dim3(256), 0, s, (const float*)src, (uint8_t*)dst, H, W, y, ordered);
            else hipLaunchKernelGGL((to_output_yuv_dither_kernel<float, uint16_t>), g, dim3(256), 0, s, (const float*)src, (uint16_t*)dst, H, W, y, ordered);
        }
    } else if (src_dtype == MOE_F16) {
        if (y.depth == 8) hipLaunchKernelGGL((to_output_yuv_kernel<half_t, uint8_t>), g, dim3(256), 0, s, (const half_t*)src, (uint8_t*)dst, H, W, y);
        else hipLaunchKernelGGL((to_output_yuv_kernel<half_t, uint16_t>), g, dim3(256), 0, s, (const half_t*)src, (uint16_t*)dst, H, W, y);
    } else {
        if (y.depth == 8) hipLaunchKernelGGL((to_output_yuv_kernel<float, uint8_t>), g, dim3(256), 0, s, (const float*)src, (uint8_t*)dst, H, W, y);
        else hipLaunchKernelGGL((to_output_yuv_kernel<float, uint16_t>), g, dim3(256), 0, s, (const float*)src, (uint16_t*)dst, H, W, y);
    }
}
```

Measured before the change: 88.04 MP/s.

## Fuse branch sum into second PS4 tail conv writing directly to output planes

When the second pixel-shuffle tail branch runs, the kernel now loads the first branch's plane through LDS and adds it in the epilogue, storing straight into the dense fp32 output buffer. A small apron-stitch kernel then adds the boundary apron contributions, replacing the separate tail-add pass. Tile outputs are laid out contiguously per group so the destination is dense. This removes a full read/write pass over the upscaled planes, at the cost of extra LDS use, an extra buffer load per row in the epilogue, and more complex eligibility conditions.

After: 87.87 MP/s (median of 2 runs). About the same (-0.2%).

```diff
diff --git a/moephoto_amd/csrc/common.h b/moephoto_amd/csrc/common.h
--- a/moephoto_amd/csrc/common.h
+++ b/moephoto_amd/csrc/common.h
@@ -130,6 +130,7 @@
     half_t* out;
     float* plane;
     float* apron;
+    const float* add;
     float slope;
     int B, H, W;
     int split;
@@ -149,6 +150,12 @@
     int vec_ok;
 };
 void launch_tailadd(const TailAddArgs& a, hipStream_t s);
+struct ApronArgs {
+    float* y;
+    const float* a0; const float* a1;
+    int B, H, W, px;
+};
+void launch_stitch_aprons(const ApronArgs& a, hipStream_t s);
 
 struct Ps9Args {
     const half_t* in;
diff --git a/moephoto_amd/csrc/conv3x3_ps4.hip b/moephoto_amd/csrc/conv3x3_ps4.hip
--- a/moephoto_amd/csrc/conv3x3_ps4.hip
+++ b/moephoto_amd/csrc/conv3x3_ps4.hip
@@ -28,9 +28,10 @@
 constexpr int OFF_BIAS = OFF_T + TROWS * TREC;
 constexpr int OFF_TW = OFF_BIAS + 1024;
 constexpr int OFF_DUMP = OFF_TW + 8 * 1024;
-constexpr int LDS_BYTES = OFF_DUMP + 1024;
-
-enum OpKind : int { OP_NONE = 0, OP_P, OP_WL, OP_TM, OP_TW, OP_BI, OP_DMA, OP_FA, OP_FR, OP_FS, OP_AR, OP_AS, OP_ST };
+constexpr int OFF_ADD = OFF_DUMP + 1024;
+constexpr int LDS_BYTES = OFF_ADD + 4 * 1024;
+
+enum OpKind : int { OP_NONE = 0, OP_P, OP_WL, OP_TM, OP_TW, OP_BI, OP_DMA, OP_FA, OP_FR, OP_FX, OP_FS, OP_AR, OP_AS, OP_ST, OP_AL };
 constexpr OpList row_ops(int epi)
 {
     OpList r;
@@ -60,7 +61,7 @@
     for (int k = 0; k < 5; ++k) r.push(OP_TW, k);
     return r;
 }
-constexpr OpList extra_ops(int e, bool tail)
+constexpr OpList extra_ops(int e, bool tail, bool add)
 {
     OpList r;
     if (!tail) {
@@ -71,11 +72,15 @@
     if (e == 0) {
         r.push(OP_FA);
         for (int dy = 0; dy < 3; ++dy) { r.push(OP_FR, dy, 0); r.push(OP_FR, dy, 1); r.push(OP_FR, dy, 2); }
+        if (add) r.push(OP_FX);
         r.push(OP_FS);
         r.push(OP_AR); r.push(OP_AS);
         r.push(OP_DMA, 0, 0); r.push(OP_DMA, 0, 1);
     }
-    if (e == 1) for (int m = 1; m < 5; ++m) { r.push(OP_DMA, m, 0); r.push(OP_DMA, m, 1); }
+    if (e == 1) {
+        if (add) r.push(OP_AL);
+        for (int m = 1; m < 5; ++m) { r.push(OP_DMA, m, 0); r.push(OP_DMA, m, 1); }
+    }
     return r;
 }
 
@@ -84,6 +89,7 @@
 {
 #if defined(__HIP_DEVICE_COMPILE__)
     constexpr bool TAIL = EPI >= 1, SPLIT = EPI == 2;
+    constexpr bool ADD = EPI == 1;
     constexpr bool PERM = !TAIL;
     extern __shared__ __attribute__((aligned(1024))) char smem[];
     const unsigned lds0 = (unsigned)(unsigned long long)(__attribute__((address_space(3))) char*)smem;
@@ -128,6 +134,7 @@
             *(u4_t*)(smem + OFF_TW + 4096 + tid * 16) = SPLIT ? tsrc[256 + tid] : u4_t{0u, 0u, 0u, 0u};
             const u4_t z = {0u, 0u, 0u, 0u};
             for (int o = tid * 16; o < TROWS * TREC; o += 256 * 16) *(u4_t*)(smem + OFF_T + o) = z;
+            if (ADD) *(u4_t*)(smem + OFF_ADD + tid * 16) = u4_t{0x80000000u, 0x80000000u, 0x80000000u, 0x80000000u};
         }
     }
     const unsigned bias_ad = lds0 + (unsigned)(OFF_BIAS + ((w4 * 2 + 0) * 2 + hh) * 64);
@@ -138,6 +145,9 @@
     const __amdgpu_buffer_rsrc_t rpl = TAIL ? __builtin_amdgcn_make_buffer_rsrc((void*)a.plane, 0, (unsigned)a.B * H * W * 16u, 0x00020000)
                                             : __builtin_amdgcn_make_buffer_rsrc((void*)a.out, 0, (unsigned)a.B * H * W * 512u, 0x00020000);
     const __amdgpu_buffer_rsrc_t rap = __builtin_amdgcn_make_buffer_rsrc((void*)(TAIL ? (void*)a.apron : (void*)a.out), 0, TAIL ? (unsigned)a.B * px * H * 16u : 0u, 0x00020000);
+    const bool has_add = ADD && a.add != nullptr;
+    const __amdgpu_buffer_rsrc_t rad = __builtin_amdgcn_make_buffer_rsrc((void*)a.add, 0, has_add ? (unsigned)a.B * H * W * 16u : 0u, 0x00020000);
+    const unsigned add_dst = (unsigned)__builtin_amdgcn_readfirstlane(has_add ? OFF_ADD + w4 * 1024 : OFF_DUMP);
     unsigned d_off = 0, d_r = 0, d_cc = 0;
     auto piece_addr = [&](int m) {
         unsigned q = (unsigned)((m < 4 ? w4 + 4 * m : 16) * 8 + (lane >> 3));
@@ -334,6 +344,21 @@
                     const unsigned so = (unsigned)(((b * 2 * H + 2 * yf) * 2 * W) + 2 * x0) * 4u;
                     __builtin_amdgcn_raw_buffer_store_b128(__builtin_bit_cast(u4_t, o4), rpl, vo, f_ok ? so : 0u, 0);
                 };
+                auto op_fx = [&]() __attribute__((always_inline)) {
+                    fs[0] = fs[0] + fv[0]; fs[1] = fs[1] + fv[1];
+                    const unsigned ad = tw_ad + (unsigned)__builtin_amdgcn_readfirstlane(OFF_ADD - OFF_TW + w4 * 1024);
+                    typedef const __attribute__((address_space(3))) float* lds_f;
+                    fv[0] = f2_t{*(lds_f)(ad), *(lds_f)(ad + 8u)};
+                    fv[1] = f2_t{*(lds_f)(ad + 4u), *(lds_f)(ad + 12u)};
+                };
+                auto op_al = [&]() __attribute__((always_inline)) {
+                    const int yn = yf + RB;
+                    const bool n_ok = (yn >= ylo) & (yn < yhi);
+                    const bool ok = n_ok & (lane < 32) & (x0 + 2 * f_xp < W);
+                    const unsigned vo = ok ? (unsigned)(f_i * 2 * W + 4 * f_xp) * 4u : kOOR;
+                    const unsigned so = (unsigned)__builtin_amdgcn_readfirstlane((int)(n_ok ? (unsigned)(((b * 2 * H + 2 * yn) * 2 * W) + 2 * x0) * 4u : 0u));
+                    __builtin_amdgcn_raw_ptr_buffer_load_lds(rad, (__attribute__((address_space(3))) void*)(smem + add_dst), 16, vo, so, 0, 0);
+                };
                 auto op_ar = [&]() __attribute__((always_inline)) {
 #pragma unroll
                     for (int dy = 0; dy < 3; ++dy) {
@@ -357,6 +382,7 @@
                         op_fr(std::integral_constant<int, 0>{}, std::integral_constant<int, 0>{}); op_fr(std::integral_constant<int, 0>{}, std::integral_constant<int, 1>{}); op_fr(std::integral_constant<int, 0>{}, std::integral_constant<int, 2>{});
                         op_fr(std::integral_constant<int, 1>{}, std::integral_constant<int, 0>{}); op_fr(std::integral_constant<int, 1>{}, std::integral_constant<int, 1>{}); op_fr(std::integral_constant<int, 1>{}, std::integral_constant<int, 2>{});
                         op_fr(std::integral_constant<int, 2>{}, std::integral_constant<int, 0>{}); op_fr(std::integral_constant<int, 2>{}, std::integral_constant<int, 1>{}); op_fr(std::integral_constant<int, 2>{}, std::integral_constant<int, 2>{});
+                        if constexpr (ADD) op_fx();
                         op_fs();
                         op_ar(); op_as();
                     }
@@ -371,7 +397,7 @@
                         asm volatile("" ::: "memory");
                     }
                     constexpr OpList LM = row_ops(EPI);
-                    constexpr OpList LX = extra_ops(e, TAIL);
+                    constexpr OpList LX = extra_ops(e, TAIL, ADD);
                     auto half = [&](auto HC_) __attribute__((always_inline)) {
                         constexpr int hc = decltype(HC_)::value;
                         if constexpr (!ZERO) {
@@ -411,9 +437,11 @@
                                 if constexpr (o.kind == OP_DMA) op_dma(std::integral_constant<int, o.a>{}, std::integral_constant<int, o.b>{});
                                 if constexpr (o.kind == OP_FA) op_fa();
                                 if constexpr (o.kind == OP_FR) op_fr(std::integral_constant<int, o.a>{}, std::integral_constant<int, o.b>{});
+                                if constexpr (o.kind == OP_FX) op_fx();
                                 if constexpr (o.kind == OP_FS) op_fs();
                                 if constexpr (o.kind == OP_AR) op_ar();
                                 if constexpr (o.kind == OP_AS) op_as();
+                                if constexpr (o.kind == OP_AL) op_al();
                             }
                         };
                         static_for<LM.n>(runm);
@@ -560,6 +588,7 @@
         conv3x3_ps4_kernel<0, true><<<dim3(G), dim3(256), LDS_BYTES, s>>>(a);
         return true;
     }
+    if (a.add && a.split) return false;
     if (a.split) {
         if (ragged) conv3x3_ps4_kernel<2, true><<<dim3(G), dim3(256), LDS_BYTES, s>>>(a);
         else conv3x3_ps4_kernel<2, false><<<dim3(G), dim3(256), LDS_BYTES, s>>>(a);
diff --git a/moephoto_amd/csrc/forward.cpp b/moephoto_amd/csrc/forward.cpp
--- a/moephoto_amd/csrc/forward.cpp
+++ b/moephoto_amd/csrc/forward.cpp
@@ -408,7 +408,7 @@
         const int cnt = (int)std::min<long long>(bmax, B - b0);
         FwdIO c = io;
         if (io.x_off) c.x_off += b0; else c.x = (const char*)io.x + (size_t)b0 * io.sB * xe;
-        if (io.y_off) c.y_off += b0; else c.y = (char*)io.y + (size_t)b0 * yplane * ye;
+        if (io.y_off) { c.y_off += b0; if (io.y_dense >= 0) c.y_dense = io.y_dense + (long long)b0 * yplane; } else c.y = (char*)io.y + (size_t)b0 * yplane * ye;
         const bool al = y_off_mult8 && (io.y_off || ((size_t)b0 * yplane * ye) % 16 == 0);
         if (int rc = forward_dev_chunk(n, c, cnt, h, w, s, al, ctx)) return rc;
     }
@@ -550,7 +550,14 @@
     }
     bool mult8 = true;
     if (y_off) for (int i = 0; i < B; ++i) mult8 = mult8 && (y_off[i] % 8 == 0);
-    const int rc = forward_dev(*n, FwdIO{x, x_dtype, sB, sH, sW, xo, y, y_dtype, yo}, B, h, w, s, mult8, own_ctx(*n, &n->set));
+    FwdIO io{x, x_dtype, sB, sH, sW, xo, y, y_dtype, yo};
+    if (y_off && B >= 1 && h >= 1 && w >= 1) {
+        const long long yplane = (long long)h * n->scale * w * n->scale;
+        bool dense = y_off[0] >= 0;
+        for (int i = 1; i < B; ++i) dense = dense && y_off[i] == y_off[0] + i * yplane;
+        if (dense) io.y_dense = y_off[0];
+    }
+    const int rc = forward_dev(*n, io, B, h, w, s, mult8, own_ctx(*n, &n->set));
     if (slot && hipEventRecord(slot->done, s) != hipSuccess) { (void)hipGetLastError(); (void)hipStreamSynchronize(s); }
     return rc;
 }
diff --git a/moephoto_amd/csrc/forward_arsb.cpp b/moephoto_amd/csrc/forward_arsb.cpp
--- a/moephoto_amd/csrc/forward_arsb.cpp
+++ b/moephoto_amd/csrc/forward_arsb.cpp
@@ -1,4 +1,6 @@
 #include "net.h"
+
+#include <type_traits>
 
 using namespace moe;
 
@@ -38,6 +40,8 @@
     bool chain8 = false;
     half_t* lo16x = nullptr;
     bool sr = false, fuse = false, ps4 = false, ps9 = false;
+    bool sum_up = false;
+    float* y_planes() const { return (float*)f.io.y + (f.io.y_off ? f.io.y_dense : 0); }
     int H = 0, W = 0;
     Act fin[2];
     float* tp[2] = {nullptr, nullptr};
@@ -93,6 +97,8 @@
         q.tail_w = f.small<half_t>(br == 0 ? "tail_r.frag" : "tail_u.frag");
         q.plane = ps_plane[br]; q.apron = ps_apron[br]; q.slope = L.slope; q.B = B; q.H = H; q.W = W;
         q.split = (f.mixed && f.tail_split_for(key)) ? 1 : 0;
+        if constexpr (std::is_same<Args, Ps4Args>::value)
+            if (sum_up && br == 1) { q.plane = y_planes(); q.add = ps_plane[0]; f.gate(); }
         const int rec = f.prof_begin(key, 2.0 * (double)B * H * W * L.cout * L.cin * L.taps);
         bool done = false;
         for (int rep = f.repeats(key); rep > 0; --rep) done = launch(q, f.groups, f.s);
@@ -239,6 +245,14 @@
 
 int ArsbRun::branch_sum()
 {
+    if (sum_up) {
+        if (f.dry()) return MOE_OK;
+        const ApronArgs t{y_planes(), ps_apron[0], ps_apron[1], B, H, W, (W / n.r + kTileW - 1) / kTileW};
+        const int rec = f.prof_begin("aprons", 0.0);
+        launch_stitch_aprons(t, f.s);
+        f.prof_end(rec);
+        return MOE_OK;
+    }
     if (ps4) { tail_add<TailAddArgs>(launch_tailadd); return MOE_OK; }
     if (ps9) { tail_add<TailAdd3Args>(launch_tailadd3); return MOE_OK; }
     if (fuse) {
@@ -314,6 +328,8 @@
         }
         if (rc) return rc;
     }
+    sum_up = ps4 && !forked && n.opt.branch_sum == 1 && !f.dry() && f.io.y_dtype == MOE_F32 && f.y_vec && (!f.io.y_off || f.io.y_dense >= 0) &&
+             !(f.mixed && f.tail_split_for("u.up" + std::to_string(n.stages - 1)));
     if (int rc = run_trunk()) return rc;
     if (n.arch == MOE_ARCH_NETDN) { f.tail(&Bb, &A, h, w, false); return MOE_OK; }
     if (mixed) { A.drop_lo(); Bb.drop_lo(); A.lo8 = Bb.lo8 = false; }
diff --git a/moephoto_amd/csrc/net.h b/moephoto_amd/csrc/net.h
--- a/moephoto_amd/csrc/net.h
+++ b/moephoto_amd/csrc/net.h
@@ -99,6 +99,7 @@
     int exact_fuse = 1;
     int q8_impl = 1;
     int fuse_tail = 1;
+    int branch_sum = 1;
     int sedn_fuse = 1;
     int pool_fuse = 1;
     int lite_lut = 1;
@@ -191,6 +192,7 @@
 struct FwdIO {
     const void* x = nullptr; int x_dtype = MOE_F32; long long sB = 0, sH = 0, sW = 0; const long long* x_off = nullptr;
     void* y = nullptr; int y_dtype = MOE_F32; const long long* y_off = nullptr;
+    long long y_dense = -1;
 };
 
 struct FwdCtx {
diff --git a/moephoto_amd/csrc/options.cpp b/moephoto_amd/csrc/options.cpp
--- a/moephoto_amd/csrc/options.cpp
+++ b/moephoto_amd/csrc/options.cpp
@@ -58,6 +58,15 @@
     {"calib_log", nullptr, kFlag, &NetOptions::calib_log},
     {"repeat", nullptr, kRepeat},
 };
+const OptionRow kLaterOptions[] = {
+    {"branch_sum", "MOE_BRANCH_SUM", kWords, &NetOptions::branch_sum, nullptr, {{"pass", 0}, {"up", 1}}},
+};
+template <typename F> bool any_row(F f)
+{
+    for (const OptionRow& r : kOptionTable) if (f(r)) return true;
+    for (const OptionRow& r : kLaterOptions) if (f(r)) return true;
+    return false;
+}
 
 bool word_value(const OptionWord* words, size_t n, const char* v, int& out)
 {
@@ -66,44 +75,53 @@
     return false;
 }
 
+bool set_row(NetOptions& o, const OptionRow& r, const char* v)
+{
+    int t = 0;
+    switch (r.kind) {
+        case kFlag: if (!word_value(kOnOff, 4, v, t)) return false; break;
+        case kWords: if (!word_value(r.words, 3, v, t)) return false; break;
+        case kCount: if ((t = atoi(v)) < 0) return false; break;
+        case kInt: t = atoi(v); break;
+        case kText: o.*r.text = v; return true;
+        case kRepeat: {
+            const char* c = strrchr(v, ':');
+            if (!c) {
+                if (*v && strcmp(v, "0")) return false;
+                o.repeat_key.clear(); o.repeat_n = 1;
+                return true;
+            }
+            const int cnt = atoi(c + 1);
+            if (cnt < 1 || c == v) return false;
+            o.repeat_key.assign(v, c - v); o.repeat_n = cnt;
+            return true;
+        }
+    }
+    o.*r.num = t;
+    return true;
+}
+
 }
 
 bool NetOptions::set(const std::string& key, const char* v)
 {
     if (!v) return false;
-    for (const OptionRow& r : kOptionTable) {
-        if (key != r.key) continue;
-        int t = 0;
-        switch (r.kind) {
-            case kFlag: if (!word_value(kOnOff, 4, v, t)) return false; break;
-            case kWords: if (!word_value(r.words, 3, v, t)) return false; break;
-            case kCount: if ((t = atoi(v)) < 0) return false; break;
-            case kInt: t = atoi(v); break;
-            case kText: this->*r.text = v; return true;
-            case kRepeat: {
-                const char* c = strrchr(v, ':');
-                if (!c) {
-                    if (*v && strcmp(v, "0")) return false;
-                    repeat_key.clear(); repeat_n = 1;
-                    return true;
-                }
-                const int cnt = atoi(c + 1);
-                if (cnt < 1 || c == v) return false;
-                repeat_key.assign(v, c - v); repeat_n = cnt;
-                return true;
-            }
-        }
-        this->*r.num = t;
+    bool ok = false;
+    any_row([&](const OptionRow& r) {
+        if (key != r.key) return false;
+        ok = set_row(*this, r, v);
         return true;
-    }
-    return false;
+    });
+    return ok;
 }
 
 void NetOptions::from_env()
 {
-    for (const OptionRow& r : kOptionTable)
+    any_row([&](const OptionRow& r) {
         if (const char* e = r.env ? getenv(r.env) : nullptr)
             if (!set(r.key, e)) fprintf(stderr, "moephoto_amd: %s=\"%s\" is not a value of option %s -- ignored\n", r.env, e, r.key);
+        return false;
+    });
 
     if (const char* e = getenv("MOE_EXACT_BLOCKS")) exact_blocks_env = atoi(e);
     arsb_trace = getenv("MOE_ARSB_TRACE") != nullptr;
diff --git a/moephoto_amd/csrc/plan_run.cpp b/moephoto_amd/csrc/plan_run.cpp
--- a/moephoto_amd/csrc/plan_run.cpp
+++ b/moephoto_amd/csrc/plan_run.cpp
@@ -7,6 +7,7 @@
     int64_t sC = 0, sH = 0, sW = 0, frame_stride = 0;
     std::vector<int64_t> tile_dst;
     bool y_mult8 = false;
+    std::vector<long long> y_host;
     std::vector<int> group_first, group_count;
     void* dev = nullptr;
     const long long *x_off = nullptr, *y_off = nullptr;
@@ -96,6 +97,7 @@
     if (off.empty()) { off.push_back(0); yo.push_back(0); }
     d.y_mult8 = true;
     for (long long v : yo) d.y_mult8 = d.y_mult8 && (v % 8 == 0);
+    d.y_host = yo;
 }
 
 static int tile_table(const moe_plan& pl, int device, int64_t frame_stride, int64_t sC, int64_t sH, int64_t sW, int n_frames, const int64_t* tile_dst,
@@ -136,7 +138,12 @@
         for (int t0 = 0; t0 < nt; t0 += per) {
             const int cnt = std::min(per, nt - t0);
             const long long slot = (long long)(d.group_first[gi] + t0) * p.C;
-            int rc = forward_dev(n, FwdIO{img, img_dtype, 0, sH, sW, d.x_off + slot, dst, MOE_F32, d.y_off + slot}, cnt * p.C, g.th, g.tw, s, d.y_mult8, own_ctx(n, &n.set));
+            FwdIO io{img, img_dtype, 0, sH, sW, d.x_off + slot, dst, MOE_F32, d.y_off + slot};
+            const long long plane = (long long)(g.th * p.sc) * (g.tw * p.sc), first = d.y_host[(size_t)slot];
+            bool dense = first >= 0;
+            for (int b = 1; b < cnt * p.C && dense; ++b) dense = d.y_host[(size_t)slot + b] == first + b * plane;
+            if (dense) io.y_dense = first;
+            int rc = forward_dev(n, io, cnt * p.C, g.th, g.tw, s, d.y_mult8, own_ctx(n, &n.set));
             if (rc) return rc;
         }
     }
@@ -363,6 +370,13 @@
     hipStream_t s = (hipStream_t)stream;
     HIP_TRY(hipSetDevice(n->device));
     std::vector<int64_t> at(p.tile_off.begin(), p.tile_off.end());
+    const bool by_group = !pool;
+    if (by_group) {
+        long long off = 0;
+        for (const auto& g : p.groups)
+            for (int k : g.tiles) { at[(size_t)k] = off; off += (long long)p.C * (g.th * p.sc) * (g.tw * p.sc); }
+    }
+    const std::vector<int64_t> layout(at);
     for (size_t k = 0; k < at.size(); ++k) if ((int)(k % shard_count) != shard_index) at[k] = -1;
     const TileTable* d = nullptr;
     int rc = tile_table(*pl, n->device, 0, sC, sH, sW, 1, at.data(), s, &d);
@@ -374,7 +388,7 @@
     }
     rc = run_sets(*n, p, *d, img, img_dtype, sH, sW, pool, max_tiles, s);
     if (rc || !do_stitch) return rc;
-    return stitch(*pl, n->device, pool, nullptr, false, p.C, out, out_dtype, nullptr, s, edge);
+    return stitch(*pl, n->device, pool, by_group ? layout.data() : nullptr, true, p.C, out, out_dtype, nullptr, s, edge);
 }
 
 static int ring_slot(const moe_plan& pl, int device, TableRing** ring, int* slot)
diff --git a/moephoto_amd/csrc/stitch.hip b/moephoto_amd/csrc/stitch.hip
--- a/moephoto_amd/csrc/stitch.hip
+++ b/moephoto_amd/csrc/stitch.hip
@@ -463,6 +463,27 @@
 #include "to_output_yuv_body.inc"
 }
 
+__global__ __launch_bounds__(256) void stitch_aprons_kernel(ApronArgs a)
+{
+    const int nb = a.px - 1;
+    const long long idx = (long long)blockIdx.x * 256 + threadIdx.x;
+    if (idx >= (long long)a.B * nb * a.H) return;
+    const int Y = (int)(idx % a.H);
+    const int c = (int)((idx / a.H) % nb) + 1, b = (int)(idx / ((long long)a.H * nb));
+    const long long side = (long long)a.B * a.px * a.H;
+    const long long r = ((long long)b * a.px + (c - 1)) * a.H + Y, l = side + ((long long)b * a.px + c) * a.H + Y;
+    float* at = a.y + ((long long)b * a.H + Y) * a.W + 64 * c;
+    at[0] += a.a0[r] + a.a1[r];
+    at[-1] += a.a0[l] + a.a1[l];
+}
+
+}
+
+void launch_stitch_aprons(const ApronArgs& a, hipStream_t s)
+{
+    const long long n = (long long)a.B * (a.px - 1) * a.H;
+    if (n <= 0) return;
+    hipLaunchKernelGGL(stitch_aprons_kernel, dim3((unsigned)((n + 255) / 256)), dim3(256), 0, s, a);
 }
 
 void launch_stitch(const StitchArgs& a, hipStream_t s)
```
